# codeonwort/Software-Raytracing

Measured on AMD Instinct MI355X. Metric: Mrays/sec (primary+secondary) + frame time, Cornell Box 1080p 64spp, higher is better.
Workload: dtype f32

## Files before the change

### include/raylib_amd.h

```cpp
#ifndef RAYLIB_AMD_H
#define RAYLIB_AMD_H

#include "raylib_types.h"

#ifdef __cplusplus
extern "C" {
#endif

typedef struct RaylibAMDStats {
	uint64_t rays;
	uint64_t nodesVisited;
	uint64_t trisTested;
	uint64_t shadedHits;
	uint64_t texFetches;
	uint64_t cameraSamples;
	uint64_t pixels;
	double   kernelMs;
	double   traceKernelMs;
	double   wallMs;
	uint32_t traceLaunches;
	uint32_t numNodes;
	uint32_t numTriangles;
	uint32_t bvhDepth;
	uint64_t waveTrips;
// ... 203 lines not shown
typedef struct RaylibAMDLightmapParams {
	int32_t width, height;
	int32_t triFirst, triCount;
	int32_t dilate;
	float   time;
	RaylibAMDGatherParams gather;
} RaylibAMDLightmapParams;
RAYLIB_API int64_t RaylibAMD_LightmapPoints(SceneHandle scene, const RaylibAMDLightmapParams* params, const float* uv, RaylibAMDGatherPoint* outPoints, uint32_t* outTexel,
        int64_t capacity);
RAYLIB_API int64_t RaylibAMD_LightmapPointsHost(SceneHandle scene, const RaylibAMDLightmapParams* params, const float* uv, RaylibAMDGatherPoint* outPoints, uint32_t* outTexel,
        int64_t capacity);
RAYLIB_API int32_t RaylibAMD_BakeLightmap(SceneHandle scene, const RaylibAMDLightmapParams* params, const float* uv, float* out, uint8_t* outCoverage);
RAYLIB_API int32_t RaylibAMD_BakeLightmapDevice(SceneHandle scene, const RaylibAMDLightmapParams* params, const float* uv, float* out, uint8_t* outCoverage, void* stream);
RAYLIB_API int32_t RaylibAMD_BakeLightmapAdaptive(SceneHandle scene, const RaylibAMDLightmapParams* params, const RaylibAMDGatherAdaptiveParams* adaptive, const float* uv,
        float* out, uint8_t* outCoverage, uint32_t* outSamples);
RAYLIB_API int32_t RaylibAMD_BakeLightmapAdaptiveDevice(SceneHandle scene, const RaylibAMDLightmapParams* params, const RaylibAMDGatherAdaptiveParams* adaptive,
        const float* uv, float* out, uint8_t* outCoverage, uint32_t* outSamples, void* stream);

typedef struct RaylibAMDLightmapFilterParams {
	int32_t iterations;
	float   sigmaColor;
	float   sigmaNormal;
	float   sigmaPosition;
} RaylibAMDLightmapFilterParams;
RAYLIB_API int32_t RaylibAMD_BakeLightmapFiltered(SceneHandle scene, const RaylibAMDLightmapParams* params, const RaylibAMDLightmapFilterParams* filter, const float* uv,
        float* out, uint8_t* outCoverage);
RAYLIB_API int32_t RaylibAMD_BakeLightmapFilteredDevice(SceneHandle scene, const RaylibAMDLightmapParams* params, const RaylibAMDLightmapFilterParams* filter, const float* uv,
        float* out, uint8_t* outCoverage, void* stream);
RAYLIB_API int32_t RaylibAMD_FilterLightmap(SceneHandle scene, const RaylibAMDLightmapParams* params, const RaylibAMDLightmapFilterParams* filter, const float* uv,
        const float* in, float* out, uint8_t* outCoverage);
RAYLIB_API int32_t RaylibAMD_FilterLightmapDevice(SceneHandle scene, const RaylibAMDLightmapParams* params, const RaylibAMDLightmapFilterParams* filter, const float* uv,
        const float* in, float* out, uint8_t* outCoverage, void* stream);
RAYLIB_API int32_t RaylibAMD_FilterLightmapHost(int32_t width, int32_t height, int32_t kind, const RaylibAMDLightmapFilterParams* filter, const RaylibAMDGatherPoint* points,
        const uint32_t* texel, int64_t count, const float* values, float* outValues);

typedef uintptr_t MaterialHandle;
RAYLIB_API MaterialHandle RaylibAMD_CreateMaterial(int32_t type, const float albedo[3], float roughness, float metallic,
	const float emissive[3], float ior, const float transmission[3], float fuzziness);
RAYLIB_API int32_t RaylibAMD_DestroyMaterial(MaterialHandle material);
RAYLIB_API SceneElementHandle RaylibAMD_CreateSphere(float cx, float cy, float cz, float radius, MaterialHandle material);
RAYLIB_API SceneElementHandle RaylibAMD_CreateCube(const float minBounds[3], const float maxBounds[3], float timeStartMove,
	const float velocity[3], MaterialHandle material);
RAYLIB_API SceneElementHandle RaylibAMD_CreateTriangle(const float v0[3], const float v1[3], const float v2[3],
	const float n0[3], const float n1[3], const float n2[3], const float uv[6], MaterialHandle material);
RAYLIB_API int32_t RaylibAMD_DestroySceneElement(SceneElementHandle element);

RAYLIB_API int32_t RaylibAMD_EvalScatter(SceneHandle scene, int32_t material, const float* records, int32_t n, uint64_t seed, float* out);
RAYLIB_API int32_t RaylibAMD_EvalCameraRays(CameraHandle camera, const float* uv, int32_t n, uint64_t seed, float* out);
RAYLIB_API int32_t RaylibAMD_EvalTexture(SceneHandle scene, int32_t texture, int32_t bSRGB, const float* uv, int32_t n, float* out);
RAYLIB_API int32_t RaylibAMD_EvalDeviceMath(int32_t fn, const float* x, const float* y, int32_t n, float* out);

RAYLIB_API int32_t RaylibAMD_CullCells(CameraHandle camera, const float* bounds, const float* sunIlluminance, const float* sunDirection,
                                       int32_t width, int32_t height, uint8_t* outEmpty, float* outConstant);

RAYLIB_API int32_t RaylibAMD_VerifyExactMath(int32_t which, uint64_t* outMismatches, uint64_t* outFirstBits);
RAYLIB_API int32_t RaylibAMD_VerifyLazyRefl(uint32_t n, uint64_t seed, uint64_t* outEvents, uint64_t* outUnsafe, uint64_t* outGuardFailed);
RAYLIB_API int32_t RaylibAMD_VerifyLazyPdf(uint32_t n, uint64_t seed, uint64_t* outEvents, uint64_t* outWrong, uint64_t* outRefused);
RAYLIB_API int32_t RaylibAMD_VerifySamplerRanged(int32_t mode, uint64_t* outMismatches, uint64_t* outFirstBits, uint32_t* outInterval, uint64_t* outOutside);

RAYLIB_API int32_t RaylibAMD_SceneMoveTriangles(SceneHandle scene, int32_t first, int32_t count, const float* positions, const float* normals);
RAYLIB_API int32_t RaylibAMD_SceneMoveTrianglesDevice(SceneHandle scene, int32_t first, int32_t count, const float* positions, const float* normals, void* stream);
RAYLIB_API int32_t RaylibAMD_SceneRebuild(SceneHandle scene);
RAYLIB_API int32_t RaylibAMD_SceneCheckTrees(SceneHandle scene, uint32_t* outFailedTree);
RAYLIB_API int32_t RaylibAMD_SceneCompareTrees(SceneHandle scene, uint32_t* outDiffMask);

RAYLIB_API int32_t RaylibAMD_SceneNumTriangles(SceneHandle scene);
RAYLIB_API int32_t RaylibAMD_SceneNumMaterials(SceneHandle scene);
RAYLIB_API int32_t RaylibAMD_SceneNumTextures(SceneHandle scene);
RAYLIB_API void    RaylibAMD_SceneExportTriangles(SceneHandle scene, void* outTriangles);
RAYLIB_API void    RaylibAMD_SceneExportMaterials(SceneHandle scene, void* outMaterials);
RAYLIB_API int32_t RaylibAMD_SceneExportTriOrder(SceneHandle scene, uint32_t* outOrder);
RAYLIB_API void    RaylibAMD_SceneTextureSize(SceneHandle scene, int32_t index, int32_t* outW, int32_t* outH);
RAYLIB_API void    RaylibAMD_SceneExportTexture(SceneHandle scene, int32_t index, float* outRGBA);
RAYLIB_API void    RaylibAMD_SceneGetSun(SceneHandle scene, float outIlluminance[3], float outDirection[3]);
RAYLIB_API int32_t RaylibAMD_SceneBVHInfo(SceneHandle scene, uint32_t* outNodes, uint32_t* outDepth, float* outSahCost);
RAYLIB_API int32_t RaylibAMD_SceneBVH4Info(SceneHandle scene, uint32_t* outNodes4, uint32_t* outWorstCaseStack);
RAYLIB_API int32_t RaylibAMD_SceneBVH8Info(SceneHandle scene, uint32_t* outNodes8, uint32_t* outLevels, float* outSteps4, float* outSteps8);
RAYLIB_API int32_t RaylibAMD_SceneWalk8Host(SceneHandle scene, const float* rays, int32_t count, float tMin, const float* tMax, float* outT, uint32_t* outSteps);
RAYLIB_API int32_t RaylibAMD_SceneWalkStackHost(SceneHandle scene, int32_t tree, const float* rays, int32_t count, float tMin, int32_t capacity, float* outT, uint32_t* outHighWater);
RAYLIB_API int32_t RaylibAMD_SceneLeafListInfo(SceneHandle scene, uint32_t* outMaxTrianglesPerLeaf);
RAYLIB_API int32_t RaylibAMD_ScenePlain(SceneHandle scene);
RAYLIB_API int32_t RaylibAMD_LastTracePlain(void);
RAYLIB_API int32_t RaylibAMD_SceneLazyRefl(SceneHandle scene);
RAYLIB_API int32_t RaylibAMD_LastTraceLazy(void);
RAYLIB_API int32_t RaylibAMD_LastHitQueue(void);
RAYLIB_API int32_t RaylibAMD_LastLitMask(void);
typedef struct RaylibAMDRenderPlan {
	int32_t pathTrace;
	int32_t stack, prims;
	int32_t poolK;
	int32_t tree;
	int32_t lstack;
	int32_t lds;
	int32_t plain;
	uint32_t pathsPerWave, treeWidth, nodeBytes;
	int32_t keepNodes4, keepNodes4f;
	int32_t eagerTree;
	uint32_t batch, sampleCount, blocks, stackStride, jobChunk, heads, jobsPerHead, guideShift;
	uint64_t jobs;
	int32_t lazy;
	int32_t hitQueue;
} RaylibAMDRenderPlan;
RAYLIB_API int32_t RaylibAMD_PlanRender(SceneHandle scene, const RendererSettings* settings, int32_t hasSky, int32_t numCUs, int32_t workgroupsPerCU, RaylibAMDRenderPlan* out);
#define RAYLIB_AMD_MAX_VIEWS 64
RAYLIB_API int32_t RaylibAMD_RenderViews(const RendererSettings* settings, SceneHandle scene,
        const CameraHandle* cameras, int32_t count, const ImageHandle* outImages);
RAYLIB_API int32_t RaylibAMD_RenderViewsDevice(const RendererSettings* settings, SceneHandle scene,
        const CameraHandle* cameras, int32_t count, void* outDevice);
RAYLIB_API int32_t RaylibAMD_PlanViews(SceneHandle scene, const RendererSettings* settings, const CameraHandle* cameras, int32_t count, int32_t hasSky,
        int32_t numCUs, int32_t workgroupsPerCU, RaylibAMDRenderPlan* outPlan, uint8_t* outCellEmpty);
RAYLIB_API uint64_t RaylibAMD_SceneBVHHash(SceneHandle scene);
RAYLIB_API uint64_t RaylibAMD_SceneTopologyHash(SceneHandle scene);
RAYLIB_API int32_t RaylibAMD_SceneExportBVHNodes(SceneHandle scene, void* out);
RAYLIB_API void    RaylibAMD_CameraExport(CameraHandle camera, float out[19]);
RAYLIB_API ImageHandle RaylibAMD_CreateImageFromData(uint32_t width, uint32_t height, const float* rgba);
RAYLIB_API void    RaylibAMD_DumpImageRGBA(ImageHandle image, float* outRGBA);
RAYLIB_API float   RaylibAMD_ParseFloat(const char* token);
RAYLIB_API int32_t RaylibAMD_ImageSize(ImageHandle image, uint32_t* outWidth, uint32_t* outHeight);
RAYLIB_API int32_t RaylibAMD_OBJModelSetTexture(OBJModelHandle obj, const char* materialName, int32_t slot, ImageHandle image);

typedef struct RaylibAMDDenoiseParams {
	int32_t iterations;
	float   sigmaColor;
	float   sigmaNormal;
	float   sigmaAlbedo;
} RaylibAMDDenoiseParams;
RAYLIB_API int32_t RaylibAMD_Denoise(ImageHandle main, int32_t bHDR, ImageHandle albedo, ImageHandle normal,
                                     ImageHandle out, const RaylibAMDDenoiseParams* params);
RAYLIB_API int32_t RaylibAMD_DenoiseHost(uint32_t width, uint32_t height, const float* colorRGBA, int32_t bHDR,
                                         const float* albedoRGBA, const float* normalRGBA,
                                         const RaylibAMDDenoiseParams* params, float* outRGBA);
RAYLIB_API void    RaylibAMD_EnableDenoiser(int32_t enable);

typedef uintptr_t RaylibAMDProgressiveHandle;
typedef struct RaylibAMDProgressiveParams {
	float    threshold;
	uint32_t minSamples;
} RaylibAMDProgressiveParams;

RAYLIB_API RaylibAMDProgressiveHandle RaylibAMD_BeginProgressive(const RendererSettings* settings, SceneHandle scene, CameraHandle camera,
                                                                 ImageHandle out, const RaylibAMDProgressiveParams* params);
RAYLIB_API int32_t RaylibAMD_ProgressiveStep(RaylibAMDProgressiveHandle h, uint32_t samples);
RAYLIB_API int32_t RaylibAMD_ProgressiveExport(RaylibAMDProgressiveHandle h, uint32_t* cellSamples, uint8_t* cellStopped, float* sumY, float* sumY2);
RAYLIB_API int32_t RaylibAMD_EndProgressive(RaylibAMDProgressiveHandle h);
RAYLIB_API int32_t RaylibAMD_ProgressiveDecideHost(uint32_t width, uint32_t height, const uint32_t* cellSamples, const float* sumY,
                                                   const float* sumY2, const RaylibAMDProgressiveParams* params, uint8_t* outStop);
RAYLIB_API int32_t RaylibAMD_ProgressiveCompactTest(const uint32_t* live, uint32_t numLive, const uint8_t* stopped, const uint8_t* emptyOrNull, uint32_t numCells,
                                                    uint32_t width, uint32_t height, uint32_t* outLive, uint32_t* outTrace, uint32_t outCounts[4]);

#ifdef __cplusplus
}
#endif
#endif
```

### software-raytracing_amd/csrc/rl_abi.cc

```cpp
#include "raylib.h"
#include "raylib_amd.h"
#include "rl_host.h"
#include "rl_plan.h"
#include "rl_progressive.h"
#include "rl_lightmap.h"
#include "rl_nearest.h"
#include "rl_sdf.h"
#include "rl_overlap.h"
#include "rl_contact.h"
#include "raylib_amd_rng.h"

#include <float.h>
#include <math.h>
#include <stddef.h>
#include <stdio.h>
#include <stdlib.h>
#include <string.h>
#include <algorithm>

using namespace rl;

namespace {

template <typename T>
// ... 646 lines not shown
SceneElementHandle RaylibAMD_CreateTriangle(const float v0[3], const float v1[3], const float v2[3],
                                            const float n0[3], const float n1[3], const float n2[3], const float uv[6], MaterialHandle material)
{
	if (!v0 || !v1 || !v2 || !n0 || !n1 || !n2) return 0;
	SceneElement* e = NewElement(PRIM_TRIANGLE, material);
	if (!e) return 0;
	HostTriangle& t = e->tri;
	t.v0 = F3(v0[0], v0[1], v0[2]); t.v1 = F3(v1[0], v1[1], v1[2]); t.v2 = F3(v2[0], v2[1], v2[2]);
	t.n0 = F3(n0[0], n0[1], n0[2]); t.n1 = F3(n1[0], n1[1], n1[2]); t.n2 = F3(n2[0], n2[1], n2[2]);
	if (uv) { t.s0 = uv[0]; t.t0 = uv[1]; t.s1 = uv[2]; t.t1 = uv[3]; t.s2 = uv[4]; t.t2 = uv[5]; }
	return (SceneElementHandle)e;
}
int32_t RaylibAMD_DestroySceneElement(SceneElementHandle h)
{
	SceneElement* e = (SceneElement*)h;
	if (g_elements.eraseFirst(e)) { delete e; return 1; }
	return 0;
}

int32_t RaylibAMD_EvalScatter(SceneHandle sh, int32_t material, const float* records, int32_t n, uint64_t seed, float* out)
{
	Scene* s = (Scene*)sh;
	if (!s || !s->finalized || !records || !out || material < 0 || material >= (int32_t)s->materials.size()) return 0;
	return DeviceEvalHook(0, s, nullptr, material, 0, records, n, seed, out) ? 1 : 0;
}
int32_t RaylibAMD_EvalCameraRays(CameraHandle ch, const float* uv, int32_t n, uint64_t seed, float* out)
{
	Camera* c = (Camera*)ch;
	if (!c || !uv || !out) return 0;
	const DCamera d = c->ToDevice();
	return DeviceEvalHook(1, nullptr, &d, 0, 0, uv, n, seed, out) ? 1 : 0;
}
int32_t RaylibAMD_CullCells(CameraHandle ch, const float* bounds, const float* sunIlluminance, const float* sunDirection, int32_t width, int32_t height,
                            uint8_t* outEmpty, float* outConstant)
{
	Camera* c = (Camera*)ch;
	if (!c || !bounds || width <= 0 || height <= 0) return -1;
	CullScene cs;
	for (int k = 0; k < 3; ++k) { cs.boundsMin[k] = bounds[k]; cs.boundsMax[k] = bounds[3 + k]; }
	cs.boundsValid = true;
	if (sunIlluminance && sunDirection) {
		for (int k = 0; k < 3; ++k) { cs.sunIlluminance[k] = sunIlluminance[k]; cs.sunDirection[k] = sunDirection[k]; }
		cs.hasSun = !(sunIlluminance[0] == 0.0f && sunIlluminance[1] == 0.0f && sunIlluminance[2] == 0.0f);
	}
	const uint32_t W = (uint32_t)width, H = (uint32_t)height, cellsX = (W + 7) / 8, cellsY = (H + 7) / 8;
	CullResult r;
	if (!CullCells(cs, c->ToDevice(), 1, 0.0f, W, H, cellsX, 0, 1, cellsX * cellsY, r)) {
		if (outEmpty) memset(outEmpty, 0, (size_t)cellsX * cellsY);
		return r.empty.empty() ? -1 : 0;
	}
	if (outEmpty) memcpy(outEmpty, r.empty.data(), (size_t)cellsX * cellsY);
	if (outConstant) { outConstant[0] = r.L[0]; outConstant[1] = r.L[1]; outConstant[2] = r.L[2]; }
	return (int32_t)(cellsX * cellsY - (uint32_t)r.active.size());
}
int32_t RaylibAMD_EvalTexture(SceneHandle sh, int32_t texture, int32_t bSRGB, const float* uv, int32_t n, float* out)
{
	Scene* s = (Scene*)sh;
	if (!s || !s->finalized || !uv || !out || texture < 0 || texture >= (int32_t)s->textures.size()) return 0;
	return DeviceEvalHook(2, s, nullptr, texture, bSRGB, uv, n, 0, out) ? 1 : 0;
}

int32_t RaylibAMD_EvalDeviceMath(int32_t fn, const float* x, const float* y, int32_t n, float* out)
{
	if (!x || !out) return 0;
	return DeviceEvalMath(fn, x, y, n, out) ? 1 : 0;
}

int32_t RaylibAMD_VerifyExactMath(int32_t which, uint64_t* outMismatches, uint64_t* outFirstBits)
{
	if (which < 0 || which > 4) return 0;
	return DeviceVerifyExactMath(which, outMismatches, outFirstBits) ? 1 : 0;
}

int32_t RaylibAMD_VerifySamplerRanged(int32_t mode, uint64_t* outMismatches, uint64_t* outFirstBits, uint32_t* outInterval, uint64_t* outOutside)
{
	if (mode < 0 || mode > 3) return 0;
	uint64_t out[6] = { 0, 0, 0, 0, 0, 0 };
	if (!DeviceVerifySamplerRanged(mode, out)) return 0;
	if (outMismatches) *outMismatches = out[0];
	if (outFirstBits) *outFirstBits = out[1];
	if (outInterval) { outInterval[0] = (uint32_t)out[2] + 1u; outInterval[1] = (uint32_t)out[5] - 1u; outInterval[2] = (uint32_t)out[4]; }
	if (outOutside) *outOutside = out[3];
	return 1;
}

int32_t RaylibAMD_VerifyLazyRefl(uint32_t n, uint64_t seed, uint64_t* outEvents, uint64_t* outUnsafe, uint64_t* outGuardFailed)
{
	uint64_t out[3] = { 0, 0, 0 };
	if (!DeviceVerifyLazyRefl(n, seed, out)) return 0;
	if (outEvents) *outEvents = out[0];
	if (outUnsafe) *outUnsafe = out[1];
	if (outGuardFailed) *outGuardFailed = out[2];
	return 1;
}

int32_t RaylibAMD_VerifyLazyPdf(uint32_t n, uint64_t seed, uint64_t* outEvents, uint64_t* outWrong, uint64_t* outRefused)
{
	uint64_t out[3] = { 0, 0, 0 };
	if (!DeviceVerifyLazyPdf(n, seed, out)) return 0;
	if (outEvents) *outEvents = out[0];
	if (outWrong) *outWrong = out[1];
	if (outRefused) *outRefused = out[2];
	return 1;
}

int32_t RaylibAMD_ClosestHit(SceneHandle sh, const float* rays, int32_t n, float tMin, void* outHits)
// ... 892 lines not shown
	ill[0] = s->sunIlluminance.x; ill[1] = s->sunIlluminance.y; ill[2] = s->sunIlluminance.z;
	dir[0] = s->sunDirection.x; dir[1] = s->sunDirection.y; dir[2] = s->sunDirection.z;
}
int32_t RaylibAMD_SceneBVHInfo(SceneHandle sh, uint32_t* nodes, uint32_t* depth, float* sah)
{
	Scene* s = (Scene*)sh;
	if (!s || !s->finalized || !DeviceSyncMovedScene(*s)) return 0;
	if (nodes) *nodes = (uint32_t)s->bvh.nodes.size();
	if (depth) *depth = s->bvh.depth;
	if (sah) *sah = s->bvh.sahCost;
	return ValidateBVH(s->bvh, s->triangles) ? 1 : 0;
}
int32_t RaylibAMD_SceneBVH4Info(SceneHandle sh, uint32_t* nodes4, uint32_t* stackNeed)
{
	Scene* s = (Scene*)sh;
	if (!s || !s->finalized || s->bvh.nodes4.empty() || !DeviceSyncMovedScene(*s)) return 0;
	if (nodes4) *nodes4 = (uint32_t)s->bvh.nodes4.size();
	if (stackNeed) *stackNeed = s->bvh.stackNeed4;
	return (ValidateBVH4(s->bvh, s->triangles) && ValidateBVH8(s->bvh, s->triangles)) ? 1 : -1;
}
int32_t RaylibAMD_SceneBVH8Info(SceneHandle sh, uint32_t* nodes8, uint32_t* levels, float* steps4, float* steps8)
{
	Scene* s = (Scene*)sh;
	if (!s || !s->finalized || s->bvh.nodes8.empty() || !DeviceSyncMovedScene(*s)) return 0;
	if (nodes8) *nodes8 = (uint32_t)s->bvh.nodes8.size();
	if (levels) *levels = s->bvh.depth8;
	if (steps4) *steps4 = s->bvh.sahNodes4;
	if (steps8) *steps8 = s->bvh.sahNodes8;
	return ValidateBVH8(s->bvh, s->triangles) ? 1 : -1;
}
int32_t RaylibAMD_SceneWalk8Host(SceneHandle sh, const float* rays, int32_t count, float tMin, const float* tMax, float* outT, uint32_t* outSteps)
{
	Scene* s = (Scene*)sh;
	if (!s || !s->finalized || s->bvh.nodes8.empty() || !rays || !tMax || !outT || count < 0 || !DeviceSyncMovedScene(*s)) return 0;
	return Walk8Host(s->bvh, s->triangles, rays, count, tMin, tMax, outT, outSteps) ? 1 : -1;
}
int32_t RaylibAMD_SceneWalkStackHost(SceneHandle sh, int32_t tree, const float* rays, int32_t count, float tMin, int32_t capacity, float* outT, uint32_t* outHighWater)
{
	Scene* s = (Scene*)sh;
	if (!s || !s->finalized || !rays || !outT || count < 0 || capacity < 0 || (tree != 2 && tree != 3 && tree != 4 && tree != 8)) return 0;
	if (tree == 2 ? s->bvh.nodes.empty() : tree == 3 ? s->bvh.nodes4.empty() : tree == 4 ? s->bvh.nodes4q.empty() : s->bvh.nodes8.empty()) return 0;
	if (!DeviceSyncMovedScene(*s)) return 0;
	return WalkStackHost(s->bvh, s->triangles, s->spheres, s->cubes, tree, rays, count, tMin, capacity, outT, outHighWater) ? 1 : -1;
}
int32_t RaylibAMD_SceneLeafListInfo(SceneHandle sh, uint32_t* maxPerLeaf)
{
	Scene* s = (Scene*)sh;
	if (!s || !s->finalized) return 0;
	int32_t leaves = 0; uint32_t most = 0;
	for (const DNode4& n : s->bvh.leafList) for (int k = 0; k < 4; ++k) if (n.child[k] != DNODE_EMPTY) { ++leaves; most = std::max(most, (((uint32_t)~n.child[k]) & LEAF_COUNT_MASK) + 1u); }
	if (maxPerLeaf) *maxPerLeaf = most;
	return leaves;
}
int32_t RaylibAMD_ScenePlain(SceneHandle sh)
{
	Scene* s = (Scene*)sh;
	return (s && s->finalized && ScenePlain(*s)) ? 1 : 0;
}
int32_t RaylibAMD_LastTracePlain(void) { return DeviceLastTracePlain(); }
int32_t RaylibAMD_SceneLazyRefl(SceneHandle sh)
{
	Scene* s = (Scene*)sh;
	return (s && s->finalized && SceneLazyRefl(*s)) ? 1 : 0;
}
int32_t RaylibAMD_LastTraceLazy(void) { return DeviceLastTraceLazy(); }
int32_t RaylibAMD_LastHitQueue(void) { return DeviceLastHitQueue(); }
int32_t RaylibAMD_LastLitMask(void) { return DeviceLastLitMask(); }
int32_t RaylibAMD_PlanRender(SceneHandle sh, const RendererSettings* settings, int32_t hasSky, int32_t numCUs, int32_t workgroupsPerCU, RaylibAMDRenderPlan* out)
{
	Scene* s = (Scene*)sh;
	if (!s || !s->finalized || !settings || !out || numCUs < 1) return 0;
	memset(out, 0, sizeof(*out));
	const RenderKnobs knobs = ReadRenderKnobs();
	const TracePlan t = PlanTrace(*s, *settings, hasSky != 0, knobs);
	if (!t.ok) return -1;
	out->pathTrace = t.pathTrace; out->stack = t.stack; out->prims = t.prims; out->poolK = t.poolK; out->tree = t.tree; out->lstack = t.lstack; out->lds = t.lds; out->plain = t.plain; out->lazy = t.lazy ? 1 : 0; out->hitQueue = t.hitQueue ? 1 : 0;
	out->pathsPerWave = t.pathsPerWave; out->treeWidth = t.treeWidth; out->nodeBytes = t.nodeBytes;
	out->keepNodes4 = t.keepNodes4; out->keepNodes4f = t.keepNodes4f; out->eagerTree = t.eagerTree;
	const uint32_t cells = ((settings->viewportWidth + 7) / 8) * ((settings->viewportHeight + 7) / 8);
	const uint32_t spp = (uint32_t)(settings->samplesPerPixel > 1 ? settings->samplesPerPixel : 1);
	const LaunchPlan L = PlanLaunch(cells, cells, spp, 0, numCUs, workgroupsPerCU, t, knobs);
	out->batch = L.batch; out->sampleCount = L.sampleCount; out->blocks = L.blocks; out->stackStride = L.stackStride; out->jobChunk = L.jobChunk;
	out->heads = L.heads; out->jobsPerHead = L.jobsPerHead; out->guideShift = L.guideShift; out->jobs = L.jobs;
	return 1;
}
int32_t RaylibAMD_PlanViews(SceneHandle sh, const RendererSettings* settings, const CameraHandle* cameras, int32_t count, int32_t hasSky,
                           int32_t numCUs, int32_t workgroupsPerCU, RaylibAMDRenderPlan* out, uint8_t* outCellEmpty)
{
	Scene* s = (Scene*)sh;
	if (!out || numCUs < 1 || !ViewsArgsValid("RaylibAMD_PlanViews", settings, s, cameras, count, nullptr)) return 0;
	memset(out, 0, sizeof(*out));
	const RenderKnobs knobs = ReadRenderKnobs();
	const TracePlan t = PlanTrace(*s, *settings, hasSky != 0, knobs);
	if (!t.ok) return -1;
	out->pathTrace = t.pathTrace; out->stack = t.stack; out->prims = t.prims; out->poolK = t.poolK; out->tree = t.tree; out->lstack = t.lstack; out->lds = t.lds; out->plain = t.plain; out->lazy = 0;
	out->pathsPerWave = t.pathsPerWave; out->treeWidth = t.treeWidth; out->nodeBytes = t.nodeBytes;
	out->keepNodes4 = t.keepNodes4; out->keepNodes4f = t.keepNodes4f; out->eagerTree = t.eagerTree;
	std::vector<DCamera> cams((size_t)count);
	for (int32_t v = 0; v < count; ++v) cams[(size_t)v] = ((Camera*)cameras[v])->ToDevice();
	if (!DeviceSyncMovedScene(*s)) return 0;
	const ViewsPlan V = PlanViews(SceneCullScene(*s, hasSky != 0), *settings, cams.data(), (uint32_t)count, t, numCUs, workgroupsPerCU, knobs);
	if (!V.ok) return 0;
	if (outCellEmpty) memcpy(outCellEmpty, V.empty.data(), V.empty.size());
	const LaunchPlan& L = V.launch;
	out->batch = L.batch; out->sampleCount = L.sampleCount; out->blocks = L.blocks; out->stackStride = L.stackStride; out->jobChunk = L.jobChunk;
	out->heads = L.heads; out->jobsPerHead = L.jobsPerHead; out->guideShift = L.guideShift; out->jobs = L.jobs;
	return 1;
}
uint64_t RaylibAMD_SceneBVHHash(SceneHandle sh)
{
	Scene* s = (Scene*)sh;
	if (!s || !s->finalized || !DeviceSyncMovedScene(*s)) return 0;
	uint64_t h = 1469598103934665603ull;
	auto feed = [&h](const void* p, size_t n) { const unsigned char* b = (const unsigned char*)p; for (size_t i = 0; i < n; ++i) { h ^= b[i]; h *= 1099511628211ull; } };
	feed(s->bvh.nodes.data(), s->bvh.nodes.size() * sizeof(DNode));
	feed(s->bvh.triOrder.data(), s->bvh.triOrder.size() * sizeof(uint32_t));
	feed(s->bvh.nodes4.data(), s->bvh.nodes4.size() * sizeof(DNode4));
	feed(s->bvh.nodes4q.data(), s->bvh.nodes4q.size() * sizeof(DNode4Q));
	feed(s->bvh.leafList.data(), s->bvh.leafList.size() * sizeof(DNode4));
	feed(s->bvh.nodes8.data(), s->bvh.nodes8.size() * sizeof(DNode8));
	return h;
}
static int32_t MoveTrianglesInternal(const char* who, SceneHandle sh, int32_t first, int32_t count, const float* positions, const float* normals, bool hostMem, void* stream)
{
	Scene* s = (Scene*)sh;
	if (!s || !g_scenes.contains(s)) { Log("%s: unknown scene", who); return 0; }
	if (!s->finalized) { Log("%s: scene was not finalized (Raylib_FinalizeScene)", who); return 0; }
	if (first < 0 || count < 0 || (int64_t)first + (int64_t)count > (int64_t)s->triangles.size()) { Log("%s: triangles [%d, %d + %d) are not the scene's", who, first, first, count); return 0; }
	if (count == 0) return 1;
// ... 109 lines not shown
```

### software-raytracing_amd/csrc/rl_cull.cc

```cpp
#include "rl_host.h"

#include <algorithm>
#include <cmath>
#include <stdlib.h>

namespace rl {

bool CullCells(const CullScene& DS, const DCamera& cam, int32_t maxPathLength, float rayTMin, uint32_t W, uint32_t H,
               uint32_t cellsX, uint32_t cellFirst, uint32_t stride, uint32_t numLocalCells, CullResult& out)
{
	if (const char* e = getenv("RAYLIB_CULL_CELLS")) if (atoi(e) == 0) return false;
	if (DS.prims || !DS.boundsValid || maxPathLength <= 0 || numLocalCells == 0) return false;
	const double lensR = std::fabs((double)cam.lensRadius);
	if (!std::isfinite(lensR)) return false;
	if (!(rayTMin >= 0.0f)) return false;
	auto sub3 = [](const double* a, const double* b, double* r) { r[0] = a[0] - b[0]; r[1] = a[1] - b[1]; r[2] = a[2] - b[2]; };
	auto dot3 = [](const double* a, const double* b) { return a[0] * b[0] + a[1] * b[1] + a[2] * b[2]; };
	const double O[3] = { cam.origin[0], cam.origin[1], cam.origin[2] }, TL[3] = { cam.top_left[0], cam.top_left[1], cam.top_left[2] };
	const double Hh[3] = { cam.horizontal[0], cam.horizontal[1], cam.horizontal[2] }, Vv[3] = { cam.vertical[0], cam.vertical[1], cam.vertical[2] };
	for (int k = 0; k < 3; ++k) if (!std::isfinite(O[k]) || !std::isfinite(TL[k]) || !std::isfinite(Hh[k]) || !std::isfinite(Vv[k])) return false;
	double E[3]; sub3(TL, O, E); for (int k = 0; k < 3; ++k) E[k] += Vv[k];
	double N[3] = { Hh[1] * Vv[2] - Hh[2] * Vv[1], Hh[2] * Vv[0] - Hh[0] * Vv[2], Hh[0] * Vv[1] - Hh[1] * Vv[0] };
	const double hh = dot3(Hh, Hh), vv = dot3(Vv, Vv), nn = dot3(N, N);
	if (!(hh > 0.0) || !(vv > 0.0) || !(nn > 0.0) || std::fabs(dot3(Hh, Vv)) > 1e-6 * std::sqrt(hh * vv)) return false;
	double planeDist = dot3(E, N);
	if (planeDist < 0.0) { planeDist = -planeDist; for (int k = 0; k < 3; ++k) N[k] = -N[k]; }
	if (!(planeDist > 1e-12 * std::sqrt(nn) * std::sqrt(dot3(E, E)))) return false;
	const double ext = std::max({ DS.boundsMax[0] - DS.boundsMin[0], DS.boundsMax[1] - DS.boundsMin[1], DS.boundsMax[2] - DS.boundsMin[2], 1e-30 });
	double uLo = 1e300, uHi = -1e300, vLo = 1e300, vHi = -1e300;
	double lensFac = 0.0;
	for (int c = 0; c < 8; ++c) {
		double X[3], Q[3];
		for (int k = 0; k < 3; ++k) X[k] = (c >> k & 1) ? DS.boundsMax[k] + 1e-6 * ext : DS.boundsMin[k] - 1e-6 * ext;
		sub3(X, O, Q);
		const double depth = dot3(Q, N);
		if (!(depth > 1e-9 * std::sqrt(nn) * (std::sqrt(dot3(Q, Q)) + ext))) return false;
		const double sc = planeDist / depth;
		lensFac = std::max(lensFac, std::fabs(1.0 - sc));
		double R3[3]; for (int k = 0; k < 3; ++k) R3[k] = Q[k] * sc - E[k];
		const double u = dot3(R3, Hh) / hh, v = -dot3(R3, Vv) / vv;
		if (!std::isfinite(u) || !std::isfinite(v)) return false;
		uLo = std::min(uLo, u); uHi = std::max(uHi, u); vLo = std::min(vLo, v); vHi = std::max(vHi, v);
	}
	const double margin = 2.0;
	const double cocU = lensR * lensFac / std::sqrt(hh) * 1.0001, cocV = lensR * lensFac / std::sqrt(vv) * 1.0001;
	if (!std::isfinite(cocU) || !std::isfinite(cocV)) return false;
	const double xLo = (uLo - cocU) * W - margin, xHi = (uHi + cocU) * W + margin, yLo = (vLo - cocV) * H - margin, yHi = (vHi + cocV) * H + margin;
	out.raysPerSample = 1;
	out.L[0] = out.L[1] = out.L[2] = 0.0f;
	if (DS.hasSun) {
		const double D[3] = { -(double)DS.sunDirection[0], -(double)DS.sunDirection[1], -(double)DS.sunDirection[2] };
		double t0 = 0.0, t1 = 1e300;
		bool miss = false;
		for (int k = 0; k < 3 && !miss; ++k) {
			const double lo = DS.boundsMin[k] - 0.01 * ext - lensR, hi = DS.boundsMax[k] + 0.01 * ext + lensR;
			if (D[k] == 0.0) { if (O[k] < lo || O[k] > hi) miss = true; continue; }
			double a = (lo - O[k]) / D[k], b = (hi - O[k]) / D[k]; if (a > b) std::swap(a, b);
			t0 = std::max(t0, a); t1 = std::min(t1, b);
			if (t0 > t1) miss = true;
		}
		if (!miss || !std::isfinite(D[0]) || !std::isfinite(D[1]) || !std::isfinite(D[2])) return false;
		out.raysPerSample = 2;
		for (int k = 0; k < 3; ++k) out.L[k] = 0.0f + DS.sunIlluminance[k];
	}
	const uint32_t numCells = cellsX * ((H + 7) / 8);
	out.active.clear(); out.active.reserve(numLocalCells);
	out.empty.assign(numLocalCells, 0);
	out.emptyPixels = 0;
	for (uint32_t k = 0; k < numLocalCells; ++k) {
		const uint32_t cell = cellFirst + k * stride;
		if (cell >= numCells) { out.active.push_back(k); continue; }
		const uint32_t cx = cell % cellsX, cy = cell / cellsX;
		const double px0 = 8.0 * cx - 1.0, px1 = 8.0 * cx + 8.0, py0 = 8.0 * cy - 1.0, py1 = 8.0 * cy + 8.0;
		const bool outside = px1 < xLo || px0 > xHi || py1 < yLo || py0 > yHi;
		if (outside) {
			out.empty[k] = 1;
			out.emptyPixels += (uint64_t)std::min(8u, W - cx * 8) * std::min(8u, H - cy * 8);
		} else out.active.push_back(k);
	}
	return out.active.size() < numLocalCells;
}


}
```

### software-raytracing_amd/csrc/rl_dev_jobs.h

```cpp
#pragma once

#include "rl_dev_shade.h"

namespace rl {

__device__ __forceinline__ void CameraRay(const DCamera& k, float s, float t, Rng& g, V3& o, V3& d, float& rayTime)
{
	V3 rd;
	if (k.lensRadius == 0.0f) {
		(void)Next(g);
		const float u2 = Next(g);
		const float theta = 2.0f * 3.14159265358979323846f * u2;
		bool sn, cn; rtm::sincos_signs_(theta, &sn, &cn);
		rd = k.lensRadius * v3(cn ? -1.0f : 1.0f, sn ? -1.0f : 1.0f, 0.0f);
	} else {
		rd = k.lensRadius * RandomInUnitDisk(g);
	}
	V3 cu = ld3(k.u), cv = ld3(k.v);
	V3 offset = (cu * rd.x) + (cv * rd.y);
	float captureTime = k.beginTime + k.timePeriod * Next(g);
	rayTime = captureTime;
	V3 origin = ld3(k.origin);
	o = origin + offset;
	d = normalize(ld3(k.top_left) + s * ld3(k.horizontal) + (1.0f - t) * ld3(k.vertical) - origin - offset);
// ... 6 lines not shown
	v = rtm::div_by_((float)y, imageHeight, P.invHeight);
	if (sampleIndex != 0) {
		u += rtm::div_by_((Next(g) - 0.5f) * 2.0f, imageWidth, P.invWidth);
		v += rtm::div_by_((Next(g) - 0.5f) * 2.0f, imageHeight, P.invHeight);
	}
}

__device__ __forceinline__ SampleRGB make_sample(float x, float y, float z) { SampleRGB s; s.x = x; s.y = y; s.z = z; return s; }

struct JobPixel { uint32_t x, y, slot, sample; bool valid; };
__device__ __forceinline__ JobPixel DecodeJob(const DRenderParams& P, uint32_t job)
{
	JobPixel j;
	const uint32_t p = job & 63u;
	const uint32_t rest = job >> 6;
	uint32_t cellLocal = __umulhi(rest, P.magicSamples);
	uint32_t sLocal = rest - cellLocal * P.sampleCount;
	while (sLocal >= P.sampleCount) { sLocal -= P.sampleCount; ++cellLocal; }
#ifdef RL_EXP_STRIPS
	{
		const uint32_t cph = P.jobsPerHead / (P.sampleCount * 64u), hh = cellLocal / cph, ii = cellLocal % cph, sw = P.cellsX / P.numHeads;
		cellLocal = (ii / sw) * P.cellsX + hh * sw + ii % sw;
	}
#endif
	if (P.activeCells) cellLocal = P.activeCells[cellLocal];
	const uint32_t cell = P.cellFirst + cellLocal * P.cellStride;
	uint32_t cy = __umulhi(cell, P.magicCellsX);
	uint32_t cx = cell - cy * P.cellsX;
	while (cx >= P.cellsX) { cx -= P.cellsX; ++cy; }
	j.x = cx * 8u + (p & 7u); j.y = cy * 8u + (p >> 3);
	j.slot = cellLocal * 64u + p;
	j.sample = sLocal;
	j.valid = (j.x < P.width) && (j.y < P.height);
	return j;
}

__device__ __forceinline__ JobPixel DecodeJobBatch(const DRenderParams& P, uint32_t base, uint32_t lane)
{
	JobPixel j;
	const uint32_t rest = (uint32_t)__builtin_amdgcn_readfirstlane((int)base) >> 6;
	uint32_t cellLocal = __umulhi(rest, P.magicSamples);
	uint32_t sLocal = rest - cellLocal * P.sampleCount;
	while (sLocal >= P.sampleCount) { sLocal -= P.sampleCount; ++cellLocal; }
	if (P.activeCells) cellLocal = *(const __attribute__((address_space(4))) uint32_t*)(P.activeCells + cellLocal);
	const uint32_t cell = P.cellFirst + cellLocal * P.cellStride;
	uint32_t cy = __umulhi(cell, P.magicCellsX);
	uint32_t cx = cell - cy * P.cellsX;
	while (cx >= P.cellsX) { cx -= P.cellsX; ++cy; }
	j.x = cx * 8u + (lane & 7u); j.y = cy * 8u + (lane >> 3);
	j.slot = cellLocal * 64u + lane;
	j.sample = sLocal;
	j.valid = (j.x < P.width) && (j.y < P.height);
	return j;
}

__device__ __forceinline__ uint32_t DecodeView(const DViews& V, uint32_t batchCell, uint32_t& cellInView)
{
	uint32_t view = __umulhi(batchCell, V.magicCellsPerView);
	uint32_t c = batchCell - view * V.cellsPerView;
	while (c >= V.cellsPerView) { c -= V.cellsPerView; ++view; }
	cellInView = c;
	return view;
}
__device__ __forceinline__ JobPixel DecodeJobViews(const DRenderParams& P, const DViews& V, uint32_t job, uint32_t& view)
{
	JobPixel j;
	const uint32_t p = job & 63u;
	const uint32_t rest = job >> 6;
	uint32_t cellLocal = __umulhi(rest, P.magicSamples);
	uint32_t sLocal = rest - cellLocal * P.sampleCount;
	while (sLocal >= P.sampleCount) { sLocal -= P.sampleCount; ++cellLocal; }
	if (P.activeCells) cellLocal = P.activeCells[cellLocal];
	uint32_t cell;
	view = DecodeView(V, cellLocal, cell);
	uint32_t cy = __umulhi(cell, P.magicCellsX);
	uint32_t cx = cell - cy * P.cellsX;
	while (cx >= P.cellsX) { cx -= P.cellsX; ++cy; }
	j.x = cx * 8u + (p & 7u); j.y = cy * 8u + (p >> 3);
	j.slot = cellLocal * 64u + p;
	j.sample = sLocal;
	j.valid = (j.x < P.width) && (j.y < P.height);
	return j;
}
__device__ __forceinline__ JobPixel DecodeJobBatchViews(const DRenderParams& P, const DViews& V, uint32_t base, uint32_t lane, uint32_t& view)
{
	JobPixel j;
	const uint32_t rest = (uint32_t)__builtin_amdgcn_readfirstlane((int)base) >> 6;
	uint32_t cellLocal = __umulhi(rest, P.magicSamples);
	uint32_t sLocal = rest - cellLocal * P.sampleCount;
	while (sLocal >= P.sampleCount) { sLocal -= P.sampleCount; ++cellLocal; }
	if (P.activeCells) cellLocal = *(const __attribute__((address_space(4))) uint32_t*)(P.activeCells + cellLocal);
	uint32_t cell;
	view = DecodeView(V, cellLocal, cell);
	uint32_t cy = __umulhi(cell, P.magicCellsX);
	uint32_t cx = cell - cy * P.cellsX;
	while (cx >= P.cellsX) { cx -= P.cellsX; ++cy; }
	j.x = cx * 8u + (lane & 7u); j.y = cy * 8u + (lane >> 3);
	j.slot = cellLocal * 64u + lane;
	j.sample = sLocal;
	j.valid = (j.x < P.width) && (j.y < P.height);
	return j;
}
__device__ __forceinline__ DCamera LoadViewCamera(const DViews& V, uint32_t view) { return V.cameras[view]; }
__device__ __forceinline__ DCamera LoadViewCameraUniform(const DViews& V, uint32_t view)
{
	DCamera k;
// ... 43 lines not shown
		key = max(key, (uint32_t)__shfl_xor((int)key, 2));
		key = max(key, (uint32_t)__shfl_xor((int)key, 4));
		key = (uint32_t)__builtin_amdgcn_readfirstlane((int)key);
		if (key < 64u) return false;
		js.cur = key & 7u; js.left = key & ~63u;
	}
}

__device__ __forceinline__ void WaveLdsSync()
{
	__builtin_amdgcn_fence(__ATOMIC_ACQ_REL, "wavefront");
	__builtin_amdgcn_wave_barrier();
}

#ifndef RL_KARG_RELOAD
#define RL_KARG_RELOAD 1
#endif
struct KTraceArgs { DRenderParams P; DSceneView S; SkyRot R; SampleRGB* samples; float* pathStack; unsigned long long* counters; unsigned int* jobCounter; };
template <class T> __device__ __forceinline__ T KArg(uint32_t offset)
{
	uint32_t z = 0u;
	asm volatile("" : "+s"(z));
	T v;
	__builtin_memcpy(&v, (const __attribute__((address_space(4))) char*)__builtin_amdgcn_kernarg_segment_ptr() + offset + (z << 2), sizeof(T));
	return v;
}
#if RL_KARG_RELOAD
#define RL_ARGS() \
	const DRenderParams P = KArg<DRenderParams>((uint32_t)offsetof(KTraceArgs, P)); const DSceneView S = KArg<DSceneView>((uint32_t)offsetof(KTraceArgs, S)); \
	const SkyRot R = KArg<SkyRot>((uint32_t)offsetof(KTraceArgs, R)); SampleRGB* const samples = KArg<SampleRGB*>((uint32_t)offsetof(KTraceArgs, samples)); \
	float* const pathStack = KArg<float*>((uint32_t)offsetof(KTraceArgs, pathStack)); unsigned long long* const counters = KArg<unsigned long long*>((uint32_t)offsetof(KTraceArgs, counters)); \
	unsigned int* const jobCounter = KArg<unsigned int*>((uint32_t)offsetof(KTraceArgs, jobCounter)); \
	(void)P; (void)S; (void)R; (void)samples; (void)pathStack; (void)counters; (void)jobCounter
#else
#define RL_ARGS() \
	const DRenderParams& P = Pk; const DSceneView& S = Sk; const SkyRot& R = Rk; SampleRGB* const samples = samplesK; float* const pathStack = pathStackK; \
	unsigned long long* const counters = countersK; unsigned int* const jobCounter = jobCounterK; \
	(void)P; (void)S; (void)R; (void)samples; (void)pathStack; (void)counters; (void)jobCounter
#endif
struct KTraceViewsArgs { KTraceArgs A; DViews V; };
#if RL_KARG_RELOAD
#define RL_VIEWS() const DViews VW = KArg<DViews>((uint32_t)offsetof(KTraceViewsArgs, V)); (void)VW
#else
#define RL_VIEWS() const DViews& VW = Vk; (void)VW
#endif

struct KTraceLazyArgs { KTraceArgs A; DLitList LL; };
#if RL_KARG_RELOAD
#define RL_LIT_ARGS() const DLitList LL = KArg<DLitList>((uint32_t)offsetof(KTraceLazyArgs, LL)); (void)LL
#else
#define RL_LIT_ARGS() const DLitList& LL = LLk; (void)LL
#endif

template <class EACH>
__device__ __forceinline__ float4 SumSlotBatch(const DRenderParams& P, const DSceneView& S, const SkyRot& R, const SampleRGB* samples,
                                               uint32_t numSlots, uint32_t slot, uint32_t cellLocal, uint32_t x, uint32_t y, float4 a, EACH&& each)
{
	if (P.cellEmpty && P.cellEmpty[cellLocal]) {
		if (P.emptySky) {
			Counters c; c.rays = c.nodes = c.tris = c.shaded = c.texels = c.samples = c.trips = 0; RL_DIAG_BIND(c);
			for (uint32_t s = 0; s < P.sampleCount; ++s) {
				const uint32_t sidx = P.sampleBegin + s;
				Rng g; g.s = raylib_rng_begin_mixed(P.seedMixed, y * P.width + x, sidx);
				float u, v;
				PixelUV(P, x, y, sidx, g, u, v);
				V3 o, d; float rayTime;
				CameraRay(P.camera, u, v, g, o, d, rayTime);
				V3 L = MissSky(S, R, d, c);
				if (S.hasSun) L = L + ld3(S.sunIlluminance);
				a.x += L.x; a.y += L.y; a.z += L.z;
				each(L.x, L.y, L.z);
			}
		} else
		for (uint32_t s = 0; s < P.sampleCount; ++s) { a.x += P.emptyL[0]; a.y += P.emptyL[1]; a.z += P.emptyL[2]; each(P.emptyL[0], P.emptyL[1], P.emptyL[2]); }
	} else
	for (uint32_t s = 0; s < P.sampleCount; ++s) {
		const SampleRGB v = samples[(size_t)s * numSlots + slot];
		a.x += v.x; a.y += v.y; a.z += v.z;
		each(v.x, v.y, v.z);
	}
	return a;
}

}
```

### software-raytracing_amd/csrc/rl_dev_walk.h

```cpp
#pragma once

#include "rl_dev_scene.h"

namespace rl {

#define RL_BOX_WIDEN 1.00001f
#define RL_CANDIDATE_SLACK 1.000009f

#ifndef RL_OWN_BOX_WIDEN_TMIN
#define RL_OWN_BOX_WIDEN_TMIN 0
#endif
__device__ __forceinline__ bool OwnBoxPassBox(V3 mn, V3 mx, V3 o, V3 inv , float tMin, float t);
__device__ __forceinline__ bool OwnBoxPass(V3 a, V3 b, V3 c, V3 o, V3 inv , float tMin, float t)
{
	const V3 mn = v3(fminf(fminf(a.x, b.x), c.x), fminf(fminf(a.y, b.y), c.y), fminf(fminf(a.z, b.z), c.z));
	const V3 mx = v3(fmaxf(fmaxf(a.x, b.x), c.x), fmaxf(fmaxf(a.y, b.y), c.y), fmaxf(fmaxf(a.z, b.z), c.z));
	return OwnBoxPassBox(mn, mx, o, inv, tMin, t);
}
__device__ __forceinline__ bool OwnBoxPassMnMx(const float4* rec, V3 o, V3 inv, float tMin, float t)
{
	const float4 q4 = rec[4], q5 = rec[5];
	return OwnBoxPassBox(v3(q4.x, q4.y, q4.z), v3(q4.w, q5.x, q5.y), o, inv, tMin, t);
}
__device__ __forceinline__ bool OwnBoxPassBox(V3 mn, V3 mx, V3 o, V3 inv , float tMin, float t)
// ... 215 lines not shown
		cur = stk[sp * RL_BLOCK];
	}
	return best.tri >= 0;
}

__device__ __forceinline__ V3 ClampInv(V3 inv)
{
	return v3(isinf(inv.x) ? copysignf(1e30f, inv.x) : inv.x, isinf(inv.y) ? copysignf(1e30f, inv.y) : inv.y, isinf(inv.z) ? copysignf(1e30f, inv.z) : inv.z);
}
typedef float rl_v4f __attribute__((ext_vector_type(4)));
typedef uint32_t rl_v4u __attribute__((ext_vector_type(4)));
__device__ __forceinline__ float4 GLoadF4(const void* p, int i) { const rl_v4f v = ((const __attribute__((address_space(1))) rl_v4f*)p)[i]; return make_float4(v.x, v.y, v.z, v.w); }
__device__ __forceinline__ uint4 GLoadU4(const void* p, int i) { const rl_v4u v = ((const __attribute__((address_space(1))) rl_v4u*)p)[i]; return make_uint4(v.x, v.y, v.z, v.w); }
#define RL_GRID_ERR(A_, B_) (fabsf((A_) * 1.21593475e-4f) + fabsf((B_) * 4.76837158e-7f))
#define RL_SORT4_STEP(ta, ra, tb, rb) { const bool sw = tb < ta; const float tt = sw ? tb : ta; tb = sw ? ta : tb; ta = tt; const int rr = sw ? rb : ra; rb = sw ? ra : rb; ra = rr; }
#define RL_SORT4(t0, r0, t1, r1, t2, r2, t3, r3) RL_SORT4_STEP(t0, r0, t1, r1) RL_SORT4_STEP(t2, r2, t3, r3) RL_SORT4_STEP(t0, r0, t2, r2) RL_SORT4_STEP(t1, r1, t3, r3) RL_SORT4_STEP(t1, r1, t2, r2)
#define RL_WIDE_STEP_Q(S_, cur_, o_, inv_, nx_, ny_, nz_, tMin_, tmx_, widen_, t0, t1, t2, t3, ch) \
	 \
	 \
	const DNode4Q* np_ = (S_).nodes4 + (cur_); \
	const float4 h0_ = GLoadF4(np_, 0); const uint4 l_ = GLoadU4(np_, 1); const uint4 u_ = GLoadU4(np_, 2); \
	const uint4 chu_ = GLoadU4(np_, 3); const int4 ch = make_int4((int)chu_.x, (int)chu_.y, (int)chu_.z, (int)chu_.w); \
	const float Ax_ = h0_.w * (inv_).x, Ay_ = __uint_as_float(l_.w) * (inv_).y, Az_ = __uint_as_float(u_.w) * (inv_).z; \
	const float Bx_ = (h0_.x - (o_).x) * (inv_).x, By_ = (h0_.y - (o_).y) * (inv_).y, Bz_ = (h0_.z - (o_).z) * (inv_).z; \
	const float Ex_ = RL_GRID_ERR(Ax_, Bx_), Ey_ = RL_GRID_ERR(Ay_, By_), Ez_ = RL_GRID_ERR(Az_, Bz_); \
	const float Bnx_ = Bx_ - Ex_, Bfx_ = Bx_ + Ex_, Bny_ = By_ - Ey_, Bfy_ = By_ + Ey_, Bnz_ = Bz_ - Ez_, Bfz_ = Bz_ + Ez_; \
	const uint32_t nX_ = (nx_) ? u_.x : l_.x, fX_ = (nx_) ? l_.x : u_.x, nY_ = (ny_) ? u_.y : l_.y, fY_ = (ny_) ? l_.y : u_.y, nZ_ = (nz_) ? u_.z : l_.z, fZ_ = (nz_) ? l_.z : u_.z; \
	const float tMinL_ = (tMin_), tmxL_ = (tmx_), widenL_ = (widen_); \
	float t0, t1, t2, t3; \
	RL_QSLAB(0, t0) RL_QSLAB(8, t1) RL_QSLAB(16, t2) RL_QSLAB(24, t3)
#define RL_QSLAB(sh, tk) { \
	float tn = tMinL_, tf = tmxL_; \
	tn = fmaxf(tn, __builtin_fmaf((float)((nX_ >> sh) & 0xffu), Ax_, Bnx_)); tf = fminf(tf, __builtin_fmaf((float)((fX_ >> sh) & 0xffu), Ax_, Bfx_)); \
	tn = fmaxf(tn, __builtin_fmaf((float)((nY_ >> sh) & 0xffu), Ay_, Bny_)); tf = fminf(tf, __builtin_fmaf((float)((fY_ >> sh) & 0xffu), Ay_, Bfy_)); \
	tn = fmaxf(tn, __builtin_fmaf((float)((nZ_ >> sh) & 0xffu), Az_, Bnz_)); tf = fminf(tf, __builtin_fmaf((float)((fZ_ >> sh) & 0xffu), Az_, Bfz_)); \
	tk = (tf * widenL_ < tn) ? INFINITY : tn; }
#define RL_WIDE_STEP_F(np_expr, o_, inv_, nx_, ny_, nz_, tMin_, tmx_, widen_, t0, t1, t2, t3, ch) \
	const float4* np_ = (np_expr); \
	const float4 lox_ = np_[0], loy_ = np_[1], loz_ = np_[2], hix_ = np_[3], hiy_ = np_[4], hiz_ = np_[5]; \
	const int4 ch = ((const int4*)np_)[6]; \
	const float4 nX_ = (nx_) ? hix_ : lox_, fX_ = (nx_) ? lox_ : hix_; \
	const float4 nY_ = (ny_) ? hiy_ : loy_, fY_ = (ny_) ? loy_ : hiy_; \
	const float4 nZ_ = (nz_) ? hiz_ : loz_, fZ_ = (nz_) ? loz_ : hiz_; \
	const float tMinL_ = (tMin_), tmxL_ = (tmx_), widenL_ = (widen_); const V3 oL_ = (o_), invL_ = (inv_); \
	float t0, t1, t2, t3; \
	RL_FSLAB(x, t0) RL_FSLAB(y, t1) RL_FSLAB(z, t2) RL_FSLAB(w, t3)
#define RL_FSLAB(k, tk) { \
	float tn = tMinL_, tf = tmxL_; \
	tn = fmaxf(tn, (nX_.k - oL_.x) * invL_.x); tf = fminf(tf, (fX_.k - oL_.x) * invL_.x); \
	tn = fmaxf(tn, (nY_.k - oL_.y) * invL_.y); tf = fminf(tf, (fY_.k - oL_.y) * invL_.y); \
	tn = fmaxf(tn, (nZ_.k - oL_.z) * invL_.z); tf = fminf(tf, (fZ_.k - oL_.z) * invL_.z); \
	tk = (tf * widenL_ < tn) ? INFINITY : tn; }

template <bool ANYHIT, bool PLAIN = false>
__device__ __forceinline__ bool TraverseLeafList(const DSceneView& S, V3 o, V3 d, float tMin, HitRec& best, Counters& c, const float4* sm)
{
	c.rays++;
	const V3 invb = ExactInv(d);
	const bool nx = invb.x < 0.0f, ny = invb.y < 0.0f, nz = invb.z < 0.0f;
	best.t = INFINITY; best.tri = -1; best.a = 0.0f; best.b = 0.0f;
	uint32_t key[4 * RL_LEAFLIST_RECORDS];
	const V3 cc = v3(-(o.x * invb.x), -(o.y * invb.y), -(o.z * invb.z));
	const V3 ce = v3(fabsf(cc.x) * 2.3841858e-7f, fabsf(cc.y) * 2.3841858e-7f, fabsf(cc.z) * 2.3841858e-7f);
	const V3 cn = cc - ce, cf = cc + ce;
	const char* recs = (const char*)(sm + LdsAt<2>::NODES);
	const uint32_t oNX = nx ? 48u : 0u, oFX = 48u - oNX, oNY = ny ? 64u : 16u, oFY = 80u - oNY, oNZ = nz ? 80u : 32u, oFZ = 112u - oNZ;
	#pragma unroll
	for (int g = 0; g < RL_LEAFLIST_RECORDS; ++g) {
		key[4 * g] = key[4 * g + 1] = key[4 * g + 2] = key[4 * g + 3] = 0xffffffffu;
		if (g < S.numLeafRecords) {
			c.nodes += 2;
			RL_WSTEP(4);
			const char* rec = recs + g * (RL_LDS_NSTRIDE * 16);
			const float4 nX = *(const float4*)(rec + oNX), fX = *(const float4*)(rec + oFX);
			const float4 nY = *(const float4*)(rec + oNY), fY = *(const float4*)(rec + oFY);
			const float4 nZ = *(const float4*)(rec + oNZ), fZ = *(const float4*)(rec + oFZ);
			#ifndef RL_LL_SMEAR
			#define RL_LL_SMEAR 1
			#endif
			#define RL_LSLAB(k, slot) { \
				float tn = tMin, tf; \
				if (RL_LL_SMEAR) { \
					float ntn = -tMin; \
					ntn = fminf(ntn, -__builtin_fmaf(nX.k, invb.x, cn.x)); tf = __builtin_fmaf(fX.k, invb.x, cf.x); \
					ntn = fminf(ntn, -__builtin_fmaf(nY.k, invb.y, cn.y)); tf = fminf(tf, __builtin_fmaf(fY.k, invb.y, cf.y)); \
					ntn = fminf(ntn, -__builtin_fmaf(nZ.k, invb.z, cn.z)); tf = fminf(tf, __builtin_fmaf(fZ.k, invb.z, cf.z)); \
					key[slot] = ((__float_as_uint(ntn) & 0x7fffffe0u) | (uint32_t)(slot)) | (uint32_t)((int32_t)__float_as_uint(__builtin_fmaf(tf, RL_BOX_WIDEN, ntn)) >> 31); \
				} else { \
					tn = fmaxf(tn, __builtin_fmaf(nX.k, invb.x, cn.x)); tf = __builtin_fmaf(fX.k, invb.x, cf.x); \
					tn = fmaxf(tn, __builtin_fmaf(nY.k, invb.y, cn.y)); tf = fminf(tf, __builtin_fmaf(fY.k, invb.y, cf.y)); \
					tn = fmaxf(tn, __builtin_fmaf(nZ.k, invb.z, cn.z)); tf = fminf(tf, __builtin_fmaf(fZ.k, invb.z, cf.z)); \
					if (!(tf * RL_BOX_WIDEN < tn)) key[slot] = (__float_as_uint(tn) & ~31u) | (uint32_t)(slot); } }
			RL_LSLAB(x, 4 * g) RL_LSLAB(y, 4 * g + 1) RL_LSLAB(z, 4 * g + 2) RL_LSLAB(w, 4 * g + 3)
			#undef RL_LSLAB
		}
	}
	uint32_t from = 0u;
#ifdef RL_WATCHDOG
	int guardSel = 0;
#endif
	uint32_t m = 0xffffffffu;
	#pragma unroll
	for (int j = 0; j < 4 * RL_LEAFLIST_RECORDS; ++j) m = min(m, key[j]);
	for (;;) {
#ifdef RL_WATCHDOG
		if (++guardSel > 200) { printf("leaf-list pick stuck: lane %u from %u tMin %g best %g keys %u %u %u %u\n", threadIdx.x, from, tMin, best.t, key[0], key[1], key[2], key[3]); break; }
#endif
		if (m >= 0xffffffffu - from) break;
		m += from;
		if (best.t * RL_BOX_WIDEN < __uint_as_float(m & ~31u)) break;
		from = m + 1u;
		RL_WSTEP(6);
		const uint32_t j = m & 31u;
		const LeafRef L = DecodeLeaf(((const int*)(sm + LdsAt<2>::NODES + (j >> 2) * RL_LDS_NSTRIDE + 6))[j & 3u]);
#if defined(RL_DIAG_STAMPS) && RL_DIAG_STAMPS >= 2
		{
			uint32_t pairs = 0;
			for (int cc = 1; cc <= 8; ++cc) pairs += (uint32_t)cc * (uint32_t)__popcll(Ballot(L.count == cc));
			const unsigned long long em_ = Ballot(true);
			if (c.diag && (threadIdx.x & 63u) == (uint32_t)__ffsll((long long)em_) - 1u) atomicAdd(&c.diag[CNT_COUNT + 7], (unsigned long long)((pairs + 63u) / 64u));
		}
#endif
		for (int i = 0; i < L.count; ++i) {
			const float4* tr = sm + LdsAt<2>::ISECT + (L.first + i) * 6;
			const float4 q0 = tr[0], q1 = tr[1], q2 = tr[2], q3 = tr[3];
			struct { V3 v0, n, u, v; float uv, uu, vv, denom, rden; } T;
			T.v0 = v3(q0.x, q0.y, q0.z); T.n = v3(q0.w, q1.x, q1.y); T.u = v3(q1.z, q1.w, q2.x); T.v = v3(q2.y, q2.z, q2.w);
			T.uv = q3.x; T.uu = q3.y; T.vv = q3.z; T.denom = q3.w; T.rden = tr[5].z;
			c.tris++;
			RL_WSTEP(5);
			RL_TRIANGLE_TEST(S, T, L.first + i, o, d, tMin, best, !PLAIN && L.alpha, OwnBoxPassMnMx(tr, o, invb, tMin, t), ANYHIT, c, RL_ELSE_CONTINUE)
		}
		m = 0xffffffffu;
		#pragma unroll
		for (int j = 0; j < 4 * RL_LEAFLIST_RECORDS; ++j) m = min(m, key[j] - from);
	}
	return best.tri >= 0;
}

template <int STACK, bool ANYHIT, bool PRIMS, bool FULL, int LDS = 0, bool PLAIN = false>
__device__ __forceinline__ bool Traverse4(const DSceneView& S, V3 o, V3 d, float rayTime, float tMin, HitRec& best, int* stk, Counters& c, const float4* sm = nullptr,
                                          const float tBound = INFINITY)
{
	if constexpr (LDS == 2) return TraverseLeafList<ANYHIT, PLAIN>(S, o, d, tMin, best, c, sm);
	c.rays++;
	V3 invb = ExactInv(d);
	if (!FULL) invb = ClampInv(invb);
	const bool nx = invb.x < 0.0f, ny = invb.y < 0.0f, nz = invb.z < 0.0f;
	best.t = tBound; best.tri = -1; best.a = 0.0f; best.b = 0.0f;
	int sp = 0, cur = 0;
	const int DONE = 0x7fffffff;
	for (;;) {
		while (cur >= 0 && cur != DONE) {
			c.nodes += FULL ? 2 : 1;
			RL_WSTEP(4);
			const float tmx = fminf(best.t, FLT_MAX);
			float t0, t1, t2, t3; int r0, r1, r2, r3;
			if (FULL) { RL_WIDE_STEP_F((LDS ? sm + RL_LDS_NODES + cur * RL_LDS_NSTRIDE : (const float4*)(S.nodes4f + cur)), o, invb, nx, ny, nz, tMin, tmx, RL_BOX_WIDEN, a0, a1, a2, a3, ch) t0 = a0; t1 = a1; t2 = a2; t3 = a3; r0 = ch.x; r1 = ch.y; r2 = ch.z; r3 = ch.w; }
			else { RL_WIDE_STEP_Q(S, cur, o, invb, nx, ny, nz, tMin, tmx, RL_BOX_WIDEN, a0, a1, a2, a3, ch) t0 = a0; t1 = a1; t2 = a2; t3 = a3; r0 = ch.x; r1 = ch.y; r2 = ch.z; r3 = ch.w; }
			if (r0 == DNODE_EMPTY) t0 = INFINITY;
			if (r1 == DNODE_EMPTY) t1 = INFINITY;
			if (r2 == DNODE_EMPTY) t2 = INFINITY;
			if (r3 == DNODE_EMPTY) t3 = INFINITY;
			RL_SORT4(t0, r0, t1, r1, t2, r2, t3, r3)
			if (!(t0 < INFINITY)) { if (sp == 0) cur = DONE; else { --sp; cur = stk[sp * RL_BLOCK]; } continue; }
			if (t3 < INFINITY && sp < STACK) { stk[sp * RL_BLOCK] = r3; ++sp; }
			if (t2 < INFINITY && sp < STACK) { stk[sp * RL_BLOCK] = r2; ++sp; }
			if (t1 < INFINITY && sp < STACK) { stk[sp * RL_BLOCK] = r1; ++sp; }
			cur = r0;
		}
		if (cur == DONE) break;
		{
			const LeafRef L = DecodeLeaf(cur);
			RL_WSTEP(6);
			for (int i = 0; i < L.count; ++i) {
				const Tri T = LDS ? TriFrom(sm + RL_LDS_ISECT + (L.first + i) * RL_LDS_TSTRIDE) : LoadTri(S, L.first + i);
				c.tris++;
				RL_WSTEP(5);
				RL_TRIANGLE_TEST(S, T, L.first + i, o, d, tMin, best, L.alpha, OwnBoxPass(T.v0, T.v1, T.v2, o, ExactInv(d), tMin, t), ANYHIT, c, RL_ELSE_CONTINUE)
			}
		}
		if (sp == 0) break;
		--sp;
		cur = stk[sp * RL_BLOCK];
	}
	(void)rayTime;
	return best.tri >= 0;
}

}
```

### software-raytracing_amd/csrc/rl_host.h

```cpp
#pragma once

#include "raylib_types.h"
#include "raylib_amd.h"
#include "rl_device.h"

#include <math.h>
#include <stdint.h>
#include <memory>
#include <mutex>
#include <string>
#include <vector>

namespace rl {

struct f3 { float x, y, z; };
inline f3 F3(float x, float y, float z) { f3 r; r.x = x; r.y = y; r.z = z; return r; }
inline f3 operator+(f3 a, f3 b) { return F3(a.x + b.x, a.y + b.y, a.z + b.z); }
inline f3 operator-(f3 a, f3 b) { return F3(a.x - b.x, a.y - b.y, a.z - b.z); }
inline f3 operator*(f3 a, f3 b) { return F3(a.x * b.x, a.y * b.y, a.z * b.z); }
inline f3 operator*(f3 a, float t) { return F3(a.x * t, a.y * t, a.z * t); }
inline f3 operator*(float t, f3 a) { return F3(a.x * t, a.y * t, a.z * t); }
inline f3 operator-(f3 a) { return F3(-a.x, -a.y, -a.z); }
inline float dot(f3 a, f3 b) { return a.x * b.x + a.y * b.y + a.z * b.z; }
inline f3 cross(f3 a, f3 b) { return F3(a.y * b.z - a.z * b.y, -(a.x * b.z - a.z * b.x), a.x * b.y - a.y * b.x); }
// ... 129 lines not shown
	void Finalize();
	bool BuildAccel(float t0, float t1);
};
bool ScenePlain(const Scene& sc);
bool SceneLazyRefl(const Scene& sc);

struct FlatScene {
	std::vector<DTriIsect> isect; std::vector<DTriShade> shade; std::vector<int32_t> alphaTex;
	std::vector<DMaterial> materials; std::vector<DTexture> textures; std::vector<float> texels;
	std::vector<DSphere> spheres; std::vector<DCube> cubes;
	int32_t fastBary = 1;
	SkyRot skyRot;
};
FlatScene FlattenScene(const Scene& sc);

bool LoadOBJ(const char* path, OBJModel& out);
void TransformOBJ(OBJModel& m, float tx, float ty, float tz, float yaw, float pitch, float roll, float sx, float sy, float sz);
Image* LoadImageFile(const char* path);
bool WriteImageFile(const Image& img, const char* path, uint32_t fileType);
void PostProcessHost(Image& img);

void Log(const char* fmt, ...);
void LogStart();
void LogFlush();
void LogStop();

struct RenderRequest {
	RendererSettings settings;
	DCamera camera;
	uint64_t seed;
	uint32_t cellFirst, cellStride;
	bool cellMajor = false;
	int slot = 0;
	void* outDevice;
	bool callerOwnsOut = false;
	float* outHostRGBA;
};
bool DeviceAvailable();
int DeviceNumRanks();
float ParseDecimalFloat(const char* token);
constexpr uint64_t kMaxImagePixels = 1ull << 28;
inline bool PlausibleImageSize(uint64_t w, uint64_t h, uint64_t fileBytes, uint64_t maxPixelsPerByte)
{
	return w > 0 && h > 0 && w <= 65535 && h <= 65535 && w * h <= kMaxImagePixels && w * h <= (fileBytes + 64) * maxPixelsPerByte;
}
bool DecodeJPEG(const std::vector<uint8_t>& data, uint32_t& w, uint32_t& h, std::vector<uint8_t>& rgba);
bool DecodeTGA(const std::vector<uint8_t>& data, uint32_t& w, uint32_t& h, std::vector<uint8_t>& rgba);
bool EncodeJPEG(uint32_t w, uint32_t h, const uint8_t* rgbTopDown, std::vector<uint8_t>& out);
bool DeviceRender(Scene& scene, const RenderRequest& req, RaylibAMDStats& stats);
bool DeviceRenderViews(Scene& scene, const RenderRequest& req, const DCamera* cameras, uint32_t count, void* outDevice, void* const* imagePixels, RaylibAMDStats& stats);
int32_t DeviceLastTraceLazy();
int32_t DeviceLastHitQueue();
int32_t DeviceLastLitMask();
int32_t DeviceLastTracePlain();
bool DeviceDrain(RaylibAMDStats* outLastStats);
void DeviceOwnStats();
bool DeviceClosestHit(Scene& scene, const float* rays, int32_t n, float tMin, void* outHits);
bool DeviceTraceRays(Scene& scene, int32_t kind, const void* rays, int32_t n, float rayTime, void* out, int32_t* outPrim, bool hostMem, void* stream,
                     RaylibAMDStats& stats);
bool DeviceRenderGBuffer(Scene& scene, const RendererSettings& settings, const DCamera& camera, uint64_t seed, const RaylibAMDGBufferPlanes& planes, bool hostMem, void* stream,
                         RaylibAMDStats& stats);
bool DeviceTraceRaysAll(Scene& scene, const void* rays, int32_t n, int32_t maxHits, void* outHits, uint32_t* outCount, bool hostMem, void* stream, RaylibAMDStats& stats);
bool DeviceNearestPoints(Scene& scene, int32_t kind, const void* points, int32_t n, void* out, bool hostMem, void* stream, RaylibAMDStats& stats);
bool DeviceNearestPointsAll(Scene& scene, const void* points, int32_t n, int32_t maxHits, void* outHits, uint32_t* outCount, bool hostMem, void* stream, RaylibAMDStats& stats);
bool DeviceBakeDistanceField(Scene& scene, const RaylibAMDDistanceFieldParams& grid, float* outDist, int32_t* outPrim, bool hostMem, void* stream, RaylibAMDStats& stats);
bool DeviceOverlapTriangles(Scene& scene, int32_t kind, uint32_t flags, const void* queries, int32_t n, int32_t maxHits, void* out, uint32_t* outCount, bool hostMem, void* stream,
                            RaylibAMDStats& stats, void* outContact = nullptr, bool contacts = false);
constexpr uint64_t RL_RADIANCE_STACK_BUDGET = 256ull << 20;
constexpr int32_t RL_RADIANCE_MAX_PATH = 32768;
bool DeviceTraceRadiance(Scene& scene, const RaylibAMDRadianceParams& prm, uint64_t seed, const void* rays, int32_t n, float* out, bool hostMem, void* stream,
                         RaylibAMDStats& stats);
constexpr uint64_t RL_GATHER_SAMPLE_BUDGET = 256ull << 20;
constexpr uint64_t RL_GATHER_MAX_SLOTS = 1ull << 28;
constexpr uint64_t RL_GATHER_TIMED = 4096;
constexpr uint32_t RL_GATHER_ADAPTIVE_MAX_PASSES = 4096;
bool DeviceGather(Scene& scene, int32_t kind, const RaylibAMDRadianceParams& prm, uint64_t seed, const void* points, int32_t n, float* out, bool hostMem, void* stream,
                  RaylibAMDStats& stats, const RaylibAMDGatherAdaptiveParams* A = nullptr, uint32_t* outSamples = nullptr);
bool DeviceGatherCompactTest(const uint32_t* live, uint32_t numLive, const uint8_t* stopped, const RaylibAMDGatherPoint* points, uint32_t numPoints,
                             uint32_t* outLive, RaylibAMDGatherPoint* outPoints, uint32_t* outCount);
int64_t LightmapPointsHost(const Scene& scene, const RaylibAMDLightmapParams& P, int32_t triFirst, int32_t triCount, const float* uv,
                           RaylibAMDGatherPoint* outPoints, uint32_t* outTexel, int64_t capacity);
int64_t DeviceLightmapPoints(Scene& scene, const RaylibAMDLightmapParams& P, int32_t triFirst, int32_t triCount, const float* uv,
                             RaylibAMDGatherPoint* outPoints, uint32_t* outTexel, int64_t capacity);
bool DeviceBakeLightmap(const char* who, Scene& scene, const RaylibAMDLightmapParams& P, int32_t triFirst, int32_t triCount, const RaylibAMDRadianceParams& prm, uint64_t seed,
                        const float* uv, float* out, uint8_t* outCoverage, bool hostMem, void* stream, RaylibAMDStats& stats,
                        const RaylibAMDLightmapFilterParams* filter = nullptr, const float* in = nullptr,
                        const RaylibAMDGatherAdaptiveParams* adaptive = nullptr, uint32_t* outSamples = nullptr);
struct LmFilterInv { float invC[8], invN, invP[8]; };
LmFilterInv MakeLmFilterInv(const RaylibAMDLightmapFilterParams& F);
bool FilterLightmapHost(int32_t width, int32_t height, int32_t kind, const RaylibAMDLightmapFilterParams& F, const RaylibAMDGatherPoint* points, const uint32_t* texel,
                        int64_t count, const float* values, float* outValues);
bool DevicePostProcess(Image& img);
bool DeviceDumpRGB(Image& img, float* outRGB);
bool DeviceReadback(Image& img);
void* DeviceImagePixels(Image& img);
void DeviceFreePixels(void* p);
struct CullScene { double boundsMin[3] = { 0, 0, 0 }, boundsMax[3] = { 0, 0, 0 }; bool boundsValid = false, prims = false, hasSky = false, hasSun = false; float sunDirection[3] = { 0, 0, 0 }, sunIlluminance[3] = { 0, 0, 0 }; };
struct CullResult { std::vector<uint32_t> active; std::vector<unsigned char> empty; uint64_t emptyPixels = 0; float L[3] = { 0, 0, 0 }; uint32_t raysPerSample = 1; };
bool CullCells(const CullScene& DS, const DCamera& cam, int32_t maxPathLength, float rayTMin, uint32_t W, uint32_t H,
               uint32_t cellsX, uint32_t cellFirst, uint32_t stride, uint32_t numLocalCells, CullResult& out);
bool DeviceEvalMath(int fn, const float* x, const float* y, int n, float* out);
bool DeviceVerifyLazyRefl(uint32_t n, uint64_t seed, uint64_t out[3]);
bool DeviceVerifyLazyPdf(uint32_t n, uint64_t seed, uint64_t out[3]);
bool DeviceVerifySamplerRanged(int mode, uint64_t out[6]);
bool DeviceVerifyExactMath(int which, uint64_t* outMismatches, uint64_t* outFirst);
bool DeviceEvalHook(int kind, Scene* sc, const DCamera* cam, int a, int b, const float* in, int n, uint64_t seed, float* out);
void DeviceReleaseScene(DeviceScene* dev);
bool DeviceMoveTriangles(Scene& scene, int32_t first, int32_t count, const float* positions, const float* normals, bool hostMem, void* stream);
bool DeviceSyncMovedScene(Scene& scene);
bool DeviceCheckTrees(Scene& scene, uint32_t* outFailedTree);
bool DeviceCompareTrees(Scene& scene, uint32_t* outDiffMask);

struct ProgressiveSession;
ProgressiveSession* DeviceProgressiveBegin(Scene& sc, const RenderRequest& req, float threshold, uint32_t minSamples);
int32_t DeviceProgressiveStep(ProgressiveSession& S, uint32_t samples, void* outDevice, RaylibAMDStats& stats, bool& rendered);
bool DeviceProgressiveExport(ProgressiveSession& S, uint32_t* cellSamples, uint8_t* cellStopped, float* sumY, float* sumY2);
void DeviceProgressiveEnd(ProgressiveSession* S);
bool DeviceProgressiveCompactTest(const uint32_t* live, uint32_t numLive, const uint8_t* stopped, const uint8_t* emptyOrNull, uint32_t numCells,
                                  uint32_t width, uint32_t height, uint32_t* outLive, uint32_t* outTrace, uint32_t outCounts[4]);

void DenoiseHost(uint32_t width, uint32_t height, const float* color, bool hdr, const float* albedo, const float* normal,
                 const RaylibAMDDenoiseParams& params, float* out);
bool DeviceDenoise(Image& main, bool hdr, Image* albedo, Image* normal, Image& out, const RaylibAMDDenoiseParams& params);

}
```

### software-raytracing_amd/csrc/rl_kernels.h

```cpp
#pragma once

#include "rl_dev_jobs.h"
#include "rl_dev_pool.h"

namespace rl {

#ifndef RL_QUEUE_SPIN_LIMIT
#define RL_QUEUE_SPIN_LIMIT 0
#endif
#ifndef RL_TRACE_MIN_WAVES
#define RL_TRACE_MIN_WAVES 4
#endif
#define RL_TRACE_ARGS const DRenderParams, const DSceneView, const SkyRot, SampleRGB* __restrict__, float* __restrict__, unsigned long long* __restrict__, unsigned int* __restrict__
template <int STACK, bool PRIMS, bool FULL, int LDS = 0, bool PLAIN = false>
__global__ void __launch_bounds__(RL_BLOCK, (STACK <= 32 ? RL_TRACE_MIN_WAVES : 2)) k_trace(RL_TRACE_ARGS);
template <int STACK, bool PRIMS, bool FULL, int LDS = 0, bool PLAIN = false>
__global__ void __launch_bounds__(RL_BLOCK, (STACK <= 32 ? RL_TRACE_MIN_WAVES : 2)) k_trace_views(RL_TRACE_ARGS, const DViews);
#define RL_TRACE_INSTANCES(X) \
	X(16, false, false, 0, false) X(16, false, true, 0, false) X(16, false, true, 1, false) X(16, false, true, 2, false) X(16, false, true, 2, true) \
	X(32, false, false, 0, false) X(32, false, true, 0, false) X(32, true, false, 0, false) X(32, true, true, 0, false) \
	X(64, false, false, 0, false) X(64, false, true, 0, false) X(64, true, false, 0, false) X(64, true, true, 0, false)
#define RL_K_TRACE(a, b, c, d, e) template __global__ void k_trace<a, b, c, d, e>(RL_TRACE_ARGS);
#define RL_K_TRACE_VIEWS(a, b, c, d, e) template __global__ void k_trace_views<a, b, c, d, e>(RL_TRACE_ARGS, const DViews);
RL_TRACE_INSTANCES(extern RL_K_TRACE)
RL_TRACE_INSTANCES(extern RL_K_TRACE_VIEWS)
template <int STACK, bool PRIMS, bool FULL, int LDS, bool PLAIN>
__global__ void __launch_bounds__(RL_BLOCK, (STACK <= 32 ? RL_TRACE_MIN_WAVES : 2)) k_trace_lazy(RL_TRACE_ARGS, const DLitList);
#define RL_TRACE_LAZY_INSTANCES(X) X(16, false, true, 2, true)
#define RL_K_TRACE_LAZY(a, b, c, d, e) template __global__ void k_trace_lazy<a, b, c, d, e>(RL_TRACE_ARGS, const DLitList);
RL_TRACE_LAZY_INSTANCES(extern RL_K_TRACE_LAZY)
template <int STACK, bool PRIMS, bool FULL, int LDS, bool PLAIN>
__global__ void __launch_bounds__(RL_BLOCK, (STACK <= 32 ? RL_TRACE_MIN_WAVES : 2)) k_trace_lazy_hitq(RL_TRACE_ARGS, const DLitList);
#define RL_K_TRACE_LAZY_HITQ(a, b, c, d, e) template __global__ void k_trace_lazy_hitq<a, b, c, d, e>(RL_TRACE_ARGS, const DLitList);
RL_TRACE_LAZY_INSTANCES(extern RL_K_TRACE_LAZY_HITQ)
__global__ void __launch_bounds__(RL_BLOCK) k_fold_lit(const DSceneView S, const DLitList LL, SampleRGB* __restrict__ samples, uint32_t numSlots);
__global__ void __launch_bounds__(RL_BLOCK)
k_resolve_lit(const DRenderParams P, const DSceneView S, const SkyRot R, const SampleRGB* __restrict__ samples, float4* __restrict__ accum, float4* __restrict__ out,
              int firstBatch, int lastBatch, const DLitList LL);

template <int STACK, bool PRIMS, int K, int LSTACK = STACK, int WIDE = 0>
__global__ void __launch_bounds__(RL_BLOCK, (PoolOcc<LSTACK, PRIMS, K>::kBlocks)) k_trace_pool(RL_TRACE_ARGS);
template <int STACK, bool PRIMS, int K, int LSTACK = STACK, int WIDE = 0>
__global__ void __launch_bounds__(RL_BLOCK, (PoolOcc<LSTACK, PRIMS, K>::kBlocks)) k_trace_pool_views(RL_TRACE_ARGS, const DViews);
#define RL_POOL_INSTANCES(X) \
	X(16, false, 2, 16, 0) X(16, false, 3, 16, 0) X(16, false, 4, 16, 0) X(32, false, 2, 32, 0) X(32, false, 3, 32, 0) X(32, false, 4, 32, 0) \
	X(32, false, 2, 4, 0) X(32, false, 2, RL_POOL_SHORT_LSTACK, 0) \
	X(32, false, 2, 32, 1) X(64, false, 2, 32, 1) X(32, false, 2, RL_POOL_SHORT_LSTACK, 1) X(64, false, 2, RL_POOL_SHORT_LSTACK, 1) \
	X(2 * RL_POOL8_MAXLEVELS, false, 2, RL_POOL8_LSTACK, 3)
#define RL_K_TRACE_POOL(a, b, c, d, e) template __global__ void k_trace_pool<a, b, c, d, e>(RL_TRACE_ARGS);
#define RL_K_TRACE_POOL_VIEWS(a, b, c, d, e) template __global__ void k_trace_pool_views<a, b, c, d, e>(RL_TRACE_ARGS, const DViews);
RL_POOL_INSTANCES(extern RL_K_TRACE_POOL_VIEWS)
RL_POOL_INSTANCES(extern RL_K_TRACE_POOL)

__global__ void __launch_bounds__(RL_BLOCK)
k_resolve(const DRenderParams P, const DSceneView S, const SkyRot R, const SampleRGB* __restrict__ samples, float4* __restrict__ accum, float4* __restrict__ out, int firstBatch, int lastBatch);
__global__ void __launch_bounds__(RL_BLOCK)
k_resolve_views(const DRenderParams Pb, const DSceneView S, const SkyRot R, const SampleRGB* __restrict__ samples, float4* __restrict__ accum, float4* __restrict__ out,
                int firstBatch, int lastBatch, const DViews V);
#define RL_AOV_ARGS const DRenderParams, const DSceneView, float4* __restrict__, unsigned long long* __restrict__
template <int STACK, bool PRIMS> __global__ void __launch_bounds__(RL_BLOCK) k_aov(RL_AOV_ARGS);
template <int STACK, bool PRIMS> __global__ void __launch_bounds__(RL_BLOCK) k_aov_views(RL_AOV_ARGS, const DViews);
#define RL_AOV_INSTANCES(X) X(16, false) X(32, false) X(32, true) X(64, false) X(64, true)
#define RL_K_AOV(a, b) template __global__ void k_aov<a, b>(RL_AOV_ARGS);
#define RL_K_AOV_VIEWS(a, b) template __global__ void k_aov_views<a, b>(RL_AOV_ARGS, const DViews);
RL_AOV_INSTANCES(extern RL_K_AOV)
RL_AOV_INSTANCES(extern RL_K_AOV_VIEWS)

struct ProgressiveState {
	float4* sum;
	float* s1;
	float* s2;
	uint32_t* cellSamples;
	uint8_t* stopped;
	float threshold;
	uint32_t minSamples;
};
__global__ void __launch_bounds__(RL_BLOCK)
k_progressive_resolve(const DRenderParams P, const DSceneView S, const SkyRot R, const SampleRGB* __restrict__ samples, const ProgressiveState st,
                      float4* __restrict__ out, int lastBatch);
#define RL_COMPACT_BLOCK 1024
#define RL_COMPACT_PER 8
__global__ void __launch_bounds__(RL_COMPACT_BLOCK)
k_progressive_compact(uint32_t* __restrict__ live, uint32_t* __restrict__ trace, const uint8_t* __restrict__ stopped, const uint8_t* __restrict__ empty,
                      uint32_t numLive, uint32_t width, uint32_t height, uint32_t cellsX, uint32_t* __restrict__ counts);

__global__ void __launch_bounds__(RL_BLOCK) k_pp_max(const float4* __restrict__ px, size_t n, unsigned int* __restrict__ whiteBits);
// ... 208 lines not shown
```

### software-raytracing_amd/csrc/rl_plan.cc

```cpp
#include "rl_plan.h"

#include <algorithm>
#include <atomic>
#include <cmath>
#include <cstring>
#include <stdlib.h>

namespace rl {

RenderKnobs ReadRenderKnobs()
{
	RenderKnobs k;
	auto flag = [](const char* name) { const char* e = getenv(name); return e ? (atoi(e) != 0 ? 1 : 0) : -1; };
	if (const char* e = getenv("RAYLIB_POOL")) { const int v = atoi(e); k.pool = (v == 2 || v == 3 || v == 4) ? v : 0; }
	if (const char* e = getenv("RAYLIB_POOL_MIN_TRIS")) k.poolMinTris = (uint32_t)atoi(e);
	if (const char* e = getenv("RAYLIB_POOL_SHORT_STACK")) { const int v = atoi(e); k.poolShortStack = (v == 0 || v == 4) ? v : 1; }
	k.bvh4 = flag("RAYLIB_BVH4"); k.bvh8 = flag("RAYLIB_BVH8");
	k.ldsScene = flag("RAYLIB_LDS_SCENE"); k.leafList = flag("RAYLIB_LEAF_LIST"); k.plainKernel = flag("RAYLIB_PLAIN_KERNEL");
	if (const char* e = getenv("RAYLIB_SAMPLE_BATCH")) k.sampleBatch = std::max(0, atoi(e));
	if (const char* e = getenv("RAYLIB_SAMPLE_BUFFER_GIB")) k.sampleBufferGiB = std::max(0, atoi(e));
	if (const char* e = getenv("RAYLIB_JOB_CHUNK")) k.jobChunk = std::max(0, atoi(e));
	if (const char* e = getenv("RAYLIB_JOB_HEADS")) k.jobHeads = std::max(1, atoi(e));
	if (const char* e = getenv("RAYLIB_GUIDED")) k.guided = atoi(e);
	if (const char* e = getenv("RAYLIB_BLOCKS_PER_CU")) k.blocksPerCU = std::max(0, atoi(e));
	if (const char* e = getenv("RAYLIB_CULL_CELLS")) k.cullCells = atoi(e);
	k.lazyRefl = flag("RAYLIB_LAZY_REFL"); k.hitQueue = flag("RAYLIB_HIT_QUEUE");
	if (const char* e = getenv("RAYLIB_LIT_LIST")) k.litList = std::max(0ll, atoll(e));
	k.litMask = flag("RAYLIB_LIT_MASK");
	if (const char* e = getenv("RAYLIB_QUERY_TREE")) { const int v = atoi(e); k.queryTree = (v == 2 || v == 4 || v == 8) ? v : 0; }
	if (const char* e = getenv("RAYLIB_GATHER_BATCH")) k.gatherBatch = std::max(0, atoi(e));
	return k;
}

namespace {

TracePlan Pick(const Scene& sc, const RendererSettings& st, bool hasSky, const RenderKnobs& k, bool say)
{
	TracePlan p;
	const BVH& b = sc.bvh;
	const size_t ntri = sc.triangles.size();
	p.prims = !sc.spheres.empty() || !sc.cubes.empty();
	if (b.depth > 64) {
		if (say) Log("Raylib_Render: BVH depth %u exceeds the traversal stack (64)", b.depth);
		p.ok = false;
		return p;
	}
	p.stack = (b.depth <= 16 && !p.prims) ? 16 : b.depth <= 32 ? 32 : 64;
	p.pathTrace = st.renderMode == RAYLIB_RENDERMODE_Default;
	if (!p.pathTrace) return p;
	const bool hasNodes4 = !b.nodes4.empty(), hasNodes8 = !b.nodes8.empty();

	const bool poolable = p.stack <= 32 && !p.prims;
	const int poolK = k.pool >= 0 ? k.pool : (poolable && ntri >= k.poolMinTris ? 2 : 0);
	if (poolable && poolK > 0) {
		p.poolK = poolK; p.pathsPerWave = 64u * (uint32_t)poolK;
		if (poolK == 2 && hasNodes4 && b.stackNeed4 <= 64 && k.bvh4 != 0) {
			p.tree = TREE_GRID4; p.treeWidth = 4;
			p.stack = b.stackNeed4 <= 32 ? 32 : 64;
			if (k.poolShortStack == 0) { p.lstack = 32; return p; }
			const bool want8 = hasNodes8 && (k.bvh8 >= 0 ? k.bvh8 != 0 : b.sahNodes4 >= RL_BVH8_MIN_STEPS);
			if (want8 && b.depth8 <= RL_POOL8_MAXLEVELS) {
				p.tree = TREE_WIDE8; p.treeWidth = 8; p.nodeBytes = (uint32_t)sizeof(DNode8);
				p.stack = 2 * RL_POOL8_MAXLEVELS; p.lstack = RL_POOL8_LSTACK;
				return p;
			}
			if (want8 && say) {
				static std::atomic<const Scene*> told{ nullptr };
				if (told.exchange(&sc) != &sc) Log("Raylib_Render: the scene's 8-wide tree has %u levels, the pool kernel's stack holds %d: walking the 4-wide tree", b.depth8, (int)RL_POOL8_MAXLEVELS);
			}
			p.lstack = RL_POOL_SHORT_LSTACK;
			return p;
		}
		p.lstack = p.stack;
		if (p.stack == 32 && poolK == 2) {
			if (k.poolShortStack == 4) p.lstack = 4;
			else if (k.poolShortStack >= 0 ? k.poolShortStack != 0 : b.depth <= RL_POOL_SHORT_MAXDEPTH) p.lstack = RL_POOL_SHORT_LSTACK;
		}
		return p;
	}

	const bool floatBoxes = hasNodes4 && ntri < RL_FLOAT_BOX_MAX_TRIS;
	const bool wide = !p.prims && hasNodes4 && b.stackNeed4 <= (uint32_t)p.stack && k.bvh4 != 0;
	p.tree = !wide ? TREE_BVH2 : floatBoxes ? TREE_BOX4 : TREE_GRID4;
	p.treeWidth = wide ? 4 : 2;
	p.keepNodes4 = p.tree == TREE_GRID4;
	p.keepNodes4f = p.tree == TREE_BOX4;
	if (p.stack == 16 && p.tree == TREE_BOX4 && k.ldsScene != 0 && b.nodes4.size() <= RL_LDS_MAXNODES && ntri <= RL_LDS_MAXTRIS && sc.materials.size() <= RL_LDS_MAXMATS) {
		p.lds = 1;
		if (!b.leafList.empty() && b.leafList.size() <= RL_LEAFLIST_RECORDS && ntri <= RL_LEAFLIST_MAXTRIS && k.leafList != 0 && st.rayTMin >= 0.0f) {
			p.lds = 2; p.tree = TREE_NONE; p.treeWidth = 0;
			p.plain = !hasSky && k.plainKernel != 0 && ScenePlain(sc);
			p.lazy = p.plain && k.lazyRefl != 0 && st.maxPathLength <= RL_LAZY_MAX_PATH && SceneLazyRefl(sc);
			p.hitQueue = p.lazy && st.maxPathLength >= 1 && (k.hitQueue >= 0 ? k.hitQueue != 0 : RL_HIT_QUEUE_DEFAULT != 0);
		}
	}
	return p;
}

}

int32_t EagerTree(const Scene& sc)
{
	RendererSettings st = {};
	st.renderMode = RAYLIB_RENDERMODE_Default;
	const TracePlan d = Pick(sc, st, false, RenderKnobs(), false);
	return (d.tree == TREE_GRID4 || d.tree == TREE_WIDE8) ? d.tree : TREE_NONE;
}

TracePlan PlanTrace(const Scene& sc, const RendererSettings& st, bool hasSky, const RenderKnobs& knobs)
{
	TracePlan p = Pick(sc, st, hasSky, knobs, true);
	p.eagerTree = EagerTree(sc);
	return p;
}

QueryPlan PlanQuery(const Scene& sc, int32_t kind, const RenderKnobs& k)
{
	QueryPlan p;
	const BVH& b = sc.bvh;
	p.prims = !sc.spheres.empty() || !sc.cubes.empty();
	if (b.depth > 64) { p.ok = false; return p; }
	const int want = k.queryTree ? k.queryTree : 8;
	if (want >= 8 && !p.prims && !b.nodes8.empty() && b.depth8 <= RL_POOL8_MAXLEVELS) {
		p.tree = TREE_WIDE8; p.treeWidth = 8; p.nodeBytes = (uint32_t)sizeof(DNode8); p.stack = 2 * RL_POOL8_MAXLEVELS;
	} else if (want >= 4 && !p.prims && !b.nodes4q.empty() && b.stackNeed4 <= 64) {
		p.tree = TREE_GRID4; p.treeWidth = 4; p.stack = b.stackNeed4 <= 32 ? 32 : 64;
	} else {
		p.stack = b.depth <= 32 ? 32 : 64;
	}
	p.early = kind == RAYLIB_AMD_QUERY_ANY && !p.prims;
	return p;
}

QueryPlan PlanGBuffer(const Scene& sc, const RenderKnobs& k)
{
	return PlanQuery(sc, RAYLIB_AMD_QUERY_SURFACE, k);
}

QueryPlan PlanQueryAll(const Scene& sc, const RenderKnobs& k)
{
	QueryPlan p;
	const BVH& b = sc.bvh;
	p.prims = !sc.spheres.empty() || !sc.cubes.empty();
	if (b.depth > 64) { p.ok = false; return p; }
	const int want = k.queryTree ? k.queryTree : 8;
	if (want >= 8 && !p.prims && !b.nodes8.empty() && b.depth8 <= RL_POOL8_MAXLEVELS) {
// ... 179 lines not shown
```

### software-raytracing_amd/csrc/rl_plan.h

```cpp
#pragma once

#include "rl_host.h"

namespace rl {

#define RL_POOL_DEFAULT_MIN_TRIS 256u
#define RL_HIT_QUEUE_DEFAULT 1
#define RL_FLOAT_BOX_MAX_TRIS 4096u

struct RenderKnobs {
	int pool = -1;
	uint32_t poolMinTris = RL_POOL_DEFAULT_MIN_TRIS;
	int poolShortStack = -1;
	int bvh4 = -1, bvh8 = -1;
	int ldsScene = -1, leafList = -1, plainKernel = -1;
	int sampleBatch = 0, sampleBufferGiB = 0;
	int jobChunk = -1;
	int jobHeads = 0;
	int guided = 0;
	int blocksPerCU = 0;
	int cullCells = 1;
	int queryTree = 0;
	int gatherBatch = 0;
	int lazyRefl = -1;
	int hitQueue = -1;
	long long litList = -1;
	int litMask = -1;
};
RenderKnobs ReadRenderKnobs();

enum PlanTree : int32_t { TREE_NONE = 0, TREE_BVH2 = 1, TREE_BOX4 = 2, TREE_GRID4 = 3, TREE_WIDE8 = 4 };

struct TracePlan {
	bool ok = true;
	bool pathTrace = true;
	int stack = 16;
	bool prims = false;
	int poolK = 0;
	int32_t tree = TREE_BVH2;
	int lstack = 0;
	int lds = 0;
	bool plain = false;
	bool lazy = false;
	bool hitQueue = false;
	uint32_t pathsPerWave = 64, treeWidth = 2, nodeBytes = 64;
	bool keepNodes4 = true, keepNodes4f = true;
	int32_t eagerTree = TREE_NONE;
};
TracePlan PlanTrace(const Scene& sc, const RendererSettings& st, bool hasSky, const RenderKnobs& knobs);
int32_t EagerTree(const Scene& sc);

struct LaunchPlan {
	uint32_t batch = 1;
	uint32_t sampleCount = 0;
	uint64_t jobs = 0;
	uint32_t blocks = 1, stackStride = 0, jobChunk = 64, heads = 1, jobsPerHead = 0, guideShift = 0;
};
LaunchPlan PlanLaunch(uint32_t numLocalCells, uint32_t numActive, uint32_t spp, uint32_t sampleBegin, int numCUs, int workgroupsPerCU,
                      const TracePlan& trace, const RenderKnobs& knobs);

struct QueryPlan {
	bool ok = true;
	int32_t tree = TREE_BVH2;
	uint32_t treeWidth = 2, nodeBytes = 64;
	int stack = 32;
	bool prims = false;
	bool early = false;
};
QueryPlan PlanQuery(const Scene& sc, int32_t kind, const RenderKnobs& knobs);
QueryPlan PlanGBuffer(const Scene& sc, const RenderKnobs& knobs);
QueryPlan PlanQueryAll(const Scene& sc, const RenderKnobs& knobs);
QueryPlan PlanRadiance(const Scene& sc, const RenderKnobs& knobs);
QueryPlan PlanNearest(const Scene& sc, int32_t kind, const RenderKnobs& knobs);
QueryPlan PlanNearestAll(const Scene& sc, const RenderKnobs& knobs);
struct DistanceFieldPlan { QueryPlan nearest, rows; };
DistanceFieldPlan PlanDistanceField(const Scene& sc, const RenderKnobs& knobs);
QueryPlan PlanOverlap(const Scene& sc, int32_t kind, const RenderKnobs& knobs);

struct GatherCut { uint32_t pointsPer = 0, samplesPer = 0; uint64_t pointRanges = 0, sampleRanges = 0, launches = 0; };
struct GatherLaunch { uint32_t pointFirst, numPoints, sampleBase, numSamples; bool first, last; };
GatherCut PlanGatherCut(uint32_t n, uint32_t sampleCount, bool sphere, const RenderKnobs& knobs);
GatherLaunch GatherLaunchAt(const GatherCut& c, uint32_t n, uint32_t sampleCount, uint64_t k);

struct ViewsPlan {
	bool ok = false;
	uint32_t cellsPerView = 0, numCells = 0, numActive = 0;
	std::vector<uint32_t> active;
	std::vector<unsigned char> empty;
	std::vector<uint32_t> culledPerView;
	uint64_t emptyPixels = 0;
	float emptyL[3] = { 0, 0, 0 };
	uint32_t raysPerSample = 1;
	RenderKnobs knobs;
	LaunchPlan launch;
};
ViewsPlan PlanViews(const CullScene& cs, const RendererSettings& st, const DCamera* cameras, uint32_t count, const TracePlan& trace,
                    int numCUs, int workgroupsPerCU, const RenderKnobs& knobs);
// ... 4 lines not shown
```

### software-raytracing_amd/csrc/rl_rt.h

```cpp
#pragma once

#include "rl_kernels.h"
#include "rl_plan.h"

#include <algorithm>
#include <chrono>
#include <condition_variable>
#include <functional>
#include <map>
#include <mutex>
#include <thread>

namespace rl {

#define HIP_OK(expr) do { hipError_t e_ = (expr); if (e_ != hipSuccess) { \
	Log("HIP error %s at %s:%d: %s", hipGetErrorName(e_), __FILE__, __LINE__, #expr); return false; } } while (0)
#define HIP_TRY(expr) do { hipError_t e_ = (expr); if (e_ != hipSuccess) { \
	Log("HIP error %s at %s:%d: %s", hipGetErrorName(e_), __FILE__, __LINE__, #expr); ok = false; } } while (0)

template <typename T, bool PINNED = false>
struct DevBuf {
	T* ptr = nullptr;
	size_t bytes = 0;
	DevBuf() = default;
// ... 72 lines not shown
struct RcclApi {
	bool tried = false, ok = false;
	void* lib = nullptr;
	int (*CommInitAll)(void** comms, int ndev, const int* devlist) = nullptr;
	int (*CommDestroy)(void* comm) = nullptr;
	int (*Send)(const void* buf, size_t count, int dtype, int peer, void* comm, hipStream_t stream) = nullptr;
	int (*Recv)(void* buf, size_t count, int dtype, int peer, void* comm, hipStream_t stream) = nullptr;
	int (*GroupStart)() = nullptr;
	int (*GroupEnd)() = nullptr;
	const char* (*GetErrorString)(int) = nullptr;
	std::vector<void*> comms;
};
constexpr int kRcclFloat = 7;

struct Worker {
	std::mutex m;
	std::condition_variable cv;
	std::function<bool()> job;
	bool pending = false, result = true;
	void Start(int device)
	{
		std::thread([this, device]() {
			(void)hipSetDevice(device);
			for (;;) {
				std::function<bool()> f;
				{ std::unique_lock<std::mutex> lk(m); cv.wait(lk, [&] { return pending; }); f = job; }
				const bool r = f();
				{ std::lock_guard<std::mutex> lk(m); result = r; pending = false; }
				cv.notify_all();
			}
		}).detach();
	}
	void Post(std::function<bool()> f) { { std::lock_guard<std::mutex> lk(m); job = std::move(f); pending = true; } cv.notify_all(); }
	bool Wait() { std::unique_lock<std::mutex> lk(m); cv.wait(lk, [&] { return !pending; }); return result; }
};

#define RL_QUERY_RING 64
struct RankCtx {
	int rank = 0, device = 0, devSlot = 0, numCUs = 0;
	hipStream_t stream = nullptr;
	hipEvent_t ev[2][8] = {};
	PinBuf<unsigned long long> cntHost[2];
	DevBuf<SampleRGB> samples;
	DevBuf<float4> accum, image;
	DevBuf<float> pathStack;
	DevBuf<float4> cells;
	DevBuf<unsigned long long> counters;
	DevBuf<unsigned int> jobCounter;
	DevBuf<float4> litList; DevBuf<uint32_t> litCtl;
	DevBuf<uint32_t> litMask;
	PinBuf<uint32_t> cellListHost[2]; DevBuf<uint32_t> cellList[2]; size_t cellListCells[2] = { 0, 0 };
	std::vector<unsigned char> cullKey[2];
	uint32_t cullActive[2] = { 0, 0 }; uint64_t cullEmptyPixels[2] = { 0, 0 }; float cullL[2][3] = { { 0, 0, 0 }, { 0, 0, 0 } }; uint32_t cullRays[2] = { 1, 1 };
	std::map<const void*, int> occupancy;
	Worker* worker = nullptr;
	DevBuf<float4> qRays;
	DevBuf<void> qOut, qPrim;
	DevBuf<void> qContact;
	DevBuf<void> qPlane3, qPlane4, qPlane5, qPlane6;
	DevBuf<uint32_t> sdfBits;
	hipEvent_t sdfEv = nullptr; bool sdfEvUsed = false;
	DevBuf<unsigned int> qRing; hipEvent_t qRingEv[RL_QUERY_RING] = {}; bool qRingUsed[RL_QUERY_RING] = {}; uint32_t qRingNext = 0;
	DevBuf<unsigned long long> qStats; PinBuf<unsigned long long> qStatsHost;
	hipEvent_t qEv[2] = { nullptr, nullptr };
	DevBuf<unsigned int> radCounter;
	DevBuf<float> radStack;
	hipEvent_t radEv = nullptr; bool radEvUsed = false;
	DevBuf<float4> gSamples;
	DevBuf<float> gAcc;
	std::vector<hipEvent_t> gEv;
	DevBuf<float> gaState;
	DevBuf<uint8_t> gaStopped;
	DevBuf<uint32_t> gaCounts, gaLive[2], gaTiles;
	DevBuf<float4> gaPoints[2];
	PinBuf<uint32_t> gaHost;
	DevBuf<DLmTri> lmRec; DevBuf<unsigned long long> lmCounts, lmSums; DevBuf<float> lmUv;
	DevBuf<uint32_t> lmOwner, lmRank, lmTexel; DevBuf<float4> lmPoints; DevBuf<float> lmValues, lmFilt, lmAtlas[2]; DevBuf<uint8_t> lmCov[2];
	PinBuf<unsigned long long> lmHost;
	hipEvent_t lmEv[6] = {};
	DevBuf<uint32_t> lmSamples, lmSampleAtlas;
	hipEvent_t lmInEv = nullptr;
};

struct Runtime {
	bool probed = false, ok = false;
	std::vector<RankCtx*> ranks;
	std::vector<int> devices;
	DevBuf<float4> gather[2];
	hipStream_t gatherStream = nullptr;
	bool gatherSelf = false, wantRccl = true, pipeline = true;
	uint64_t frameNo = 0;
	struct Inflight;
	Inflight* inflight[2] = { nullptr, nullptr };
	RaylibAMDStats deferredStats = {};
	bool deferredUnreported = false;
	uint64_t statsSerial = 0;
	RcclApi rccl;
	std::mutex lock;
};
Runtime& Rt();
inline RankCtx& Rank0() { return *Rt().ranks[0]; }

struct PendingRender {
	bool pathTrace = false, lastBatchPending = false;
	float traceMs = 0.0f;
	uint32_t launches = 0, jobHeads = 0, pathsPerWave = 64, treeWidth = 2, nodeBytes = 64;
	uint64_t pixels = 0;
	uint64_t culledSamples = 0; uint32_t culledRaysPerSample = 0, culledSkyTexels = 0;
	uint32_t culledCells = 0, listedCells = 0;
	bool lazy = false;
	bool enqueuedToEnd = false;
	float4* out = nullptr; size_t outBytes = 0;
	int slot = 0;
	const unsigned long long* cnt = nullptr;
};

bool EnsureRuntime();
bool EnsureRccl();
int OccupancyOf(RankCtx& R, const void* kernel, const TracePlan* megakernel = nullptr);
bool UploadScene(Scene& sc);
bool SyncSky(Scene& sc);
bool EnsureWideTree(DeviceSceneCopy* C, Scene& sc, int32_t tree);
bool SettleMove(Scene& sc);
bool SyncMovedLocked(Scene& sc);
bool ReadbackLocked(Image& img);
bool EnqueueRender(RankCtx& R, Scene& sc, const RenderRequest& req, PendingRender& pend, ProgressiveSession* prog = nullptr);
bool FinishRender(RankCtx& R, PendingRender& pend, RaylibAMDStats& stats);
bool OnDevice(const void* p, int device);
bool GatherLocked(Scene& sc, RankCtx& R, int32_t kind, const RaylibAMDRadianceParams& prm, uint64_t seed, const void* points, int32_t n, float* out, bool hostMem, void* stream,
                  std::chrono::steady_clock::time_point t0, RaylibAMDStats& stats, const RaylibAMDGatherAdaptiveParams* A = nullptr, uint32_t* outSamples = nullptr);
bool EnqueueGatherCompact(const uint32_t* live, uint32_t numLive, const uint8_t* stopped, const float4* points, uint32_t* outLive, float4* outPoints, uint32_t* tiles,
                          uint32_t* countHost, hipStream_t st);
bool DrainLocked();

inline void SceneStats(RaylibAMDStats& stats, const Scene& sc)
{
	stats.numNodes = (uint32_t)sc.bvh.nodes.size(); stats.numTriangles = (uint32_t)sc.triangles.size(); stats.bvhDepth = sc.bvh.depth;
}
inline void OneRankStats(RaylibAMDStats& stats, const Scene& sc) { stats.ranks = 1; stats.devices = 1; SceneStats(stats, sc); }
inline double MsSince(std::chrono::steady_clock::time_point t0) { return std::chrono::duration<double, std::milli>(std::chrono::steady_clock::now() - t0).count(); }

}
```

### software-raytracing_amd/csrc/rl_rt_frame.hip

```cpp
#include "rl_rt.h"

#include <atomic>

namespace rl {

typedef void (*TraceKernel)(const DRenderParams, const DSceneView, const SkyRot, SampleRGB*, float*, unsigned long long*, unsigned int*);
typedef void (*TraceViewsKernel)(const DRenderParams, const DSceneView, const SkyRot, SampleRGB*, float*, unsigned long long*, unsigned int*, const DViews);
typedef void (*TraceLazyKernel)(const DRenderParams, const DSceneView, const SkyRot, SampleRGB*, float*, unsigned long long*, unsigned int*, const DLitList);
typedef void (*AovKernel)(const DRenderParams, const DSceneView, float4*, unsigned long long*);
typedef void (*AovViewsKernel)(const DRenderParams, const DSceneView, float4*, unsigned long long*, const DViews);

template <int STACK, bool PRIMS, bool FULL, int LDS = 0, bool PLAIN = false>
static const void* Trace(bool views)
{
	return views ? (const void*)(TraceViewsKernel)k_trace_views<STACK, PRIMS, FULL, LDS, PLAIN> : (const void*)(TraceKernel)k_trace<STACK, PRIMS, FULL, LDS, PLAIN>;
}
template <int STACK, bool PRIMS>
static const void* TraceFor(bool floatBoxes, bool views) { return floatBoxes ? Trace<STACK, PRIMS, true>(views) : Trace<STACK, PRIMS, false>(views); }
template <int STACK, bool PRIMS>
static const void* Aov(bool views) { return views ? (const void*)(AovViewsKernel)k_aov_views<STACK, PRIMS> : (const void*)(AovKernel)k_aov<STACK, PRIMS>; }
static const void* KernelFor(const TracePlan& p, bool views)
{
	if (p.poolK > 0) {
		const int wide = p.tree == TREE_WIDE8 ? 3 : p.tree == TREE_GRID4 ? 1 : 0;
#define RL_POOL_PICK(a, b, c, d, e) if (p.stack == a && p.prims == b && p.poolK == c && p.lstack == d && wide == e) \
			return views ? (const void*)(TraceViewsKernel)k_trace_pool_views<a, b, c, d, e> : (const void*)(TraceKernel)k_trace_pool<a, b, c, d, e>;
		RL_POOL_INSTANCES(RL_POOL_PICK)
#undef RL_POOL_PICK
		return nullptr;
	}
	if (p.lds == 2 && p.lazy && p.hitQueue && !views) return (const void*)(TraceLazyKernel)k_trace_lazy_hitq<16, false, true, 2, true>;
	if (p.lds == 2 && p.lazy && !views) return (const void*)(TraceLazyKernel)k_trace_lazy<16, false, true, 2, true>;
	if (p.lds == 2) return p.plain ? Trace<16, false, true, 2, true>(views) : Trace<16, false, true, 2>(views);
	if (p.lds == 1) return Trace<16, false, true, 1>(views);
	const bool full = p.tree == TREE_BOX4;
	if (p.stack == 16) return TraceFor<16, false>(full, views);
	if (p.stack == 32) return p.prims ? TraceFor<32, true>(full, views) : TraceFor<32, false>(full, views);
	return p.prims ? TraceFor<64, true>(full, views) : TraceFor<64, false>(full, views);
}
static const void* AovKernelFor(const TracePlan& p, bool views)
{
	if (p.stack == 16) return Aov<16, false>(views);
	if (p.stack == 32) return p.prims ? Aov<32, true>(views) : Aov<32, false>(views);
	return p.prims ? Aov<64, true>(views) : Aov<64, false>(views);
}
static std::atomic<int32_t> g_lastTracePlain{0};
int32_t DeviceLastTracePlain() { return g_lastTracePlain.load(std::memory_order_relaxed); }
static std::atomic<int32_t> g_lastTraceLazy{0};
int32_t DeviceLastTraceLazy() { return g_lastTraceLazy.load(std::memory_order_relaxed); }
static std::atomic<int32_t> g_lastHitQueue{0};
int32_t DeviceLastHitQueue() { return g_lastHitQueue.load(std::memory_order_relaxed); }
static std::atomic<int32_t> g_lastLitMask{0};
int32_t DeviceLastLitMask() { return g_lastLitMask.load(std::memory_order_relaxed); }

struct Frame {
	RenderKnobs knobs;
	TracePlan plan;
	DSceneView view;
	DRenderParams P;
	uint32_t numLive = 0, numActive = 0;
	uint32_t sBegin = 0, sEnd = 1;
	float4* out = nullptr;
	const DViews* views = nullptr;
	const void* resolve = nullptr;
	void* resolveArgs[5] = {};
	int firstBatch = 0, lastBatch = 0;
	bool accum = true;
	ProgressiveSession* compact = nullptr;
};

static DRenderParams BaseParams(const RendererSettings& st, uint64_t seed, const DCamera& camera, uint32_t cellFirst, uint32_t stride, uint32_t numLocalCells, bool rowMajor)
{
	DRenderParams P; memset(&P, 0, sizeof(P));
	const uint32_t W = st.viewportWidth, H = st.viewportHeight, cellsX = (W + 7) / 8;
	P.width = W; P.height = H; P.spp = (uint32_t)(st.samplesPerPixel > 1 ? st.samplesPerPixel : 1); P.maxPathLength = st.maxPathLength; P.rayTMin = st.rayTMin;
	P.invWidth = 1.0f / (float)W; P.invHeight = 1.0f / (float)H;
	P.renderMode = st.renderMode; P.seed = seed; P.cellsX = cellsX; P.cellsY = (H + 7) / 8;
	P.cellFirst = cellFirst; P.cellStride = stride; P.numLocalCells = numLocalCells;
	P.rowMajorOutput = rowMajor ? 1u : 0u; P.camera = camera;
	P.seedMixed = raylib_rng_mix64(seed);
	P.magicCellsX = cellsX > 1 ? (uint32_t)(0x100000000ull / cellsX) : 0xFFFFFFFFu;
	return P;
}

static uint64_t CoveredPixels(uint32_t W, uint32_t H, uint32_t cellFirst, uint32_t stride, uint32_t count)
{
	const uint32_t cellsX = (W + 7) / 8;
	uint64_t px = 0;
	for (uint32_t k = 0; k < count; ++k) {
		const uint32_t cell = cellFirst + k * stride, cx = cell % cellsX, cy = cell / cellsX;
		px += (uint64_t)std::min(8u, W - cx * 8) * std::min(8u, H - cy * 8);
	}
	return px;
}

static bool TraceView(DeviceSceneCopy* D, Scene& sc, const TracePlan& plan, DSceneView& view)
{
	if (!EnsureWideTree(D, sc, plan.tree)) return false;
	view = D->view;
	if (!plan.keepNodes4) view.nodes4 = nullptr;
	if (!plan.keepNodes4f) view.nodes4f = nullptr;
	return true;
}

static void ListCells(Frame& F, PendingRender& pend, const uint32_t* list, const uint8_t* empty, uint32_t numListed, uint32_t numLive, const float* L, uint64_t emptyPixels, uint32_t raysPerSample)
{
	DRenderParams& P = F.P;
	F.numLive = numLive; F.numActive = numListed;
	P.activeCells = list; P.cellEmpty = empty; P.numActiveCells = numListed;
	P.emptyL[0] = L[0]; P.emptyL[1] = L[1]; P.emptyL[2] = L[2];
	P.emptySky = F.view.sky ? 1u : 0u;
	pend.culledSamples = emptyPixels * (uint64_t)(F.sEnd - F.sBegin); pend.culledRaysPerSample = raysPerSample; pend.culledSkyTexels = F.view.sky ? 1u : 0u;
}

static bool BeginFrame(RankCtx& R, int q, const Frame& F, size_t outBytes, PendingRender& pend)
{
	pend.pathTrace = F.plan.pathTrace; pend.slot = q; pend.cnt = R.cntHost[q].ptr;
	pend.out = F.out; pend.outBytes = outBytes;
	HIP_OK(hipMemsetAsync(R.counters.ptr, 0, RL_CNT_BLOCK * sizeof(unsigned long long), R.stream));
	HIP_OK(hipEventRecord(R.ev[q][0], R.stream));
	return true;
}

static bool EnqueueFrame(RankCtx& R, int q, const DeviceScene& DS, Frame& F, PendingRender& pend)
{
	const TracePlan& plan = F.plan;
	DRenderParams& P = F.P;
	const uint32_t numCells = P.numLocalCells, numSlots = numCells * 64u;
	const uint32_t rblocks = (numSlots + RL_BLOCK - 1) / RL_BLOCK;
	SkyRot skyRot = DS.skyRot;
	if (numSlots == 0) {
	} else if (!plan.pathTrace) {
		void* args[] = { &P, &F.view, &F.out, &R.counters.ptr, (void*)F.views };
		HIP_OK(hipLaunchKernel(AovKernelFor(plan, F.views != nullptr), dim3(rblocks), dim3(RL_BLOCK), args, 0, R.stream));
	} else {
		const void* traceKernel = KernelFor(plan, F.views != nullptr);
		if (!traceKernel) { Log("Raylib_Render: no megakernel instance for STACK %d, K %d, stack in LDS %d", plan.stack, plan.poolK, plan.lstack); return false; }
		const int blocksPerCU = OccupancyOf(R, traceKernel, &plan);
		if (blocksPerCU < 0) return false;
		g_lastTracePlain.store(plan.plain ? 1 : 0, std::memory_order_relaxed);
		const bool lazy = plan.lazy && !F.views;
		g_lastTraceLazy.store(lazy ? 1 : 0, std::memory_order_relaxed);
		g_lastHitQueue.store(lazy && plan.hitQueue ? 1 : 0, std::memory_order_relaxed);
		pend.lazy = lazy;
		DLitList LL = {};
		pend.pathsPerWave = plan.pathsPerWave; pend.treeWidth = plan.treeWidth; pend.nodeBytes = plan.nodeBytes;
		pend.culledCells = F.numLive - F.numActive; pend.listedCells = F.numActive;
		const uint32_t batch = PlanLaunch(numCells, F.numActive, F.sEnd, F.sBegin, R.numCUs, blocksPerCU, plan, F.knobs).batch;
		if (!R.samples.Grow((size_t)numSlots * sizeof(SampleRGB) * std::min(batch, F.sEnd - F.sBegin))) return false;
		if (F.accum && batch < P.spp && !R.accum.Grow((size_t)numSlots * sizeof(float4))) return false;
		const bool masked = lazy && F.resolve == (const void*)k_resolve && F.knobs.litMask != 0 && (F.knobs.litMask > 0 || !F.view.hasSun) &&
		                    (std::min(batch, F.sEnd - F.sBegin) + 31u) / 32u <= RL_LIT_MASK_MAX_WORDS;
		g_lastLitMask.store(masked ? 1 : 0, std::memory_order_relaxed);
		const void* resolveKernel = masked ? (const void*)k_resolve_lit : F.resolve;
		const int depthSlots = P.maxPathLength > 1 ? P.maxPathLength : 1;
		void* traceArgs[] = { &P, &F.view, &skyRot, &R.samples.ptr, &R.pathStack.ptr, &R.counters.ptr, &R.jobCounter.ptr, lazy ? (void*)&LL : (void*)F.views };
		void* foldArgs[] = { &F.view, &LL, &R.samples.ptr, (void*)&numSlots };
		void* resolveArgs[] = { &P, &F.view, &skyRot, &R.samples.ptr, F.resolveArgs[0], F.resolveArgs[1], F.resolveArgs[2], F.resolveArgs[3], masked ? (void*)&LL : F.resolveArgs[4] };
		for (uint32_t s0 = F.sBegin; s0 < F.sEnd; s0 += batch) {
			const LaunchPlan L = PlanLaunch(numCells, F.numActive, F.sEnd, s0, R.numCUs, blocksPerCU, plan, F.knobs);
			const uint32_t cnt = L.sampleCount;
			P.sampleBegin = s0; P.sampleCount = cnt;
			P.magicSamples = cnt > 1 ? (uint32_t)(0x100000000ull / cnt) : 0xFFFFFFFFu;
			if (L.jobs > 0xF0000000ull) { Log("Raylib_Render: job count overflow"); return false; }
			P.numJobs = (uint32_t)L.jobs;
			P.stackStride = L.stackStride; P.jobChunk = L.jobChunk;
			P.numHeads = L.heads; P.jobsPerHead = L.jobsPerHead; P.guideShift = L.guideShift;
			if (!R.pathStack.Grow((size_t)depthSlots * 8 * P.stackStride * sizeof(float))) return false;
			if (lazy) {
				const uint64_t want = F.knobs.litList >= 0 ? (uint64_t)F.knobs.litList
				                                           : std::max<uint64_t>(4096, L.jobs / 32) + (uint64_t)L.blocks * (RL_BLOCK / 64) * RL_LIT_CHUNK;
				const uint32_t chunks = (uint32_t)std::min<uint64_t>(want / RL_LIT_CHUNK, 0x7FFFFFFFu / RL_LIT_CHUNK);
				if (!R.litList.Grow(std::max<size_t>(1, chunks) * RL_LIT_CHUNK * RL_LIT_STRIDE * sizeof(float4))) return false;
				if (!R.litCtl.Grow((RL_LIT_CTL + (size_t)chunks) * sizeof(uint32_t))) return false;
				LL.entries = (float*)R.litList.ptr; LL.ctl = R.litCtl.ptr; LL.numChunks = chunks;
				HIP_OK(hipMemsetAsync(R.litCtl.ptr, 0, (RL_LIT_CTL + (size_t)chunks) * sizeof(uint32_t), R.stream));
				if (masked) {
					const uint32_t words = (cnt + 31u) / 32u;
					const size_t bytes = (size_t)words * numSlots * sizeof(uint32_t);
					if (!R.litMask.Grow(bytes)) return false;
					LL.mask = R.litMask.ptr; LL.maskWords = words;
					HIP_OK(hipMemsetAsync(R.litMask.ptr, 0, bytes, R.stream));
				}
			}
			pend.jobHeads = L.heads;
			F.firstBatch = s0 == F.sBegin; F.lastBatch = s0 + cnt >= F.sEnd;
			HIP_OK(hipMemsetAsync(R.jobCounter.ptr, 0, RL_MAX_HEADS * RL_HEAD_STRIDE * sizeof(unsigned int), R.stream));
			HIP_OK(hipEventRecord(R.ev[q][2], R.stream));
			if (L.jobs > 0)
				HIP_OK(hipLaunchKernel(traceKernel, dim3(L.blocks), dim3(RL_BLOCK), traceArgs, 0, R.stream));
			if (L.jobs > 0 && lazy && LL.numChunks > 0)
				HIP_OK(hipLaunchKernel((const void*)k_fold_lit, dim3(std::min<uint32_t>((LL.numChunks + 3u) / 4u, (uint32_t)R.numCUs * 8u)), dim3(RL_BLOCK), foldArgs, 0, R.stream));
			HIP_OK(hipEventRecord(R.ev[q][3], R.stream));
			HIP_OK(hipLaunchKernel(resolveKernel, dim3(rblocks), dim3(RL_BLOCK), resolveArgs, 0, R.stream));
			++pend.launches;
			if (!F.lastBatch) {
				HIP_OK(hipEventSynchronize(R.ev[q][3]));
				float ms = 0.0f;
				HIP_OK(hipEventElapsedTime(&ms, R.ev[q][2], R.ev[q][3]));
				pend.traceMs += ms;
			} else pend.lastBatchPending = true;
		}
		if (ProgressiveSession* S = F.compact) {
			hipLaunchKernelGGL(k_progressive_compact, dim3(1), dim3(RL_COMPACT_BLOCK), 0, R.stream,
			                   S->live.ptr, S->trace.ptr, (const uint8_t*)S->st.stopped, (const uint8_t*)S->empty.ptr, S->numLive, P.width, P.height, P.cellsX, S->counts.ptr);
			HIP_OK(hipGetLastError());
			HIP_OK(hipMemcpyAsync(S->countsHost.ptr, S->counts.ptr, 4 * sizeof(uint32_t), hipMemcpyDeviceToHost, R.stream));
		}
	}
// ... 19 lines not shown
	const uint32_t stride = req.cellStride ? req.cellStride : 1;
	const uint32_t numLocalCells = req.cellFirst < numCells ? (numCells - req.cellFirst + stride - 1) / stride : 0;
	const bool rowMajor = (stride == 1 && req.cellFirst == 0 && !req.cellMajor);
	const int q = req.slot & 1;
	F.P = BaseParams(st, req.seed, req.camera, req.cellFirst, stride, numLocalCells, rowMajor);
	F.numLive = F.numActive = numLocalCells;
	F.sBegin = prog ? prog->samples : 0u; F.sEnd = prog ? prog->passEnd : F.P.spp;
	const size_t outBytes = rowMajor ? (size_t)W * H * sizeof(float4) : (size_t)numLocalCells * 64u * sizeof(float4);
	F.out = (float4*)req.outDevice;
	if (!F.out) { if (!R.image.Grow(outBytes ? outBytes : 16)) return false; F.out = R.image.ptr; }
	if (!BeginFrame(R, q, F, outBytes, pend)) return false;
	if (F.plan.pathTrace && numLocalCells && (!prog || !prog->seeded)) {
		const CullScene cs = SceneCullScene(sc, F.view.sky != nullptr);
		std::vector<unsigned char> key;
		auto put = [&](const void* ptr, size_t n) { const unsigned char* b = (const unsigned char*)ptr; key.insert(key.end(), b, b + n); };
		const uint32_t geo[7] = { W, H, req.cellFirst, stride, numLocalCells, (uint32_t)st.maxPathLength, __builtin_bit_cast(uint32_t, st.rayTMin) };
		const int flags[3] = { cs.hasSky ? 1 : 0, cs.hasSun ? 1 : 0, F.knobs.cullCells };
		put(&req.camera, sizeof(req.camera)); put(geo, sizeof(geo)); put(flags, sizeof(flags)); put(cs.sunDirection, sizeof(cs.sunDirection));
		put(cs.sunIlluminance, sizeof(cs.sunIlluminance)); put(cs.boundsMin, sizeof(cs.boundsMin)); put(cs.boundsMax, sizeof(cs.boundsMax));
		const void* sceneId = sc.device; put(&sceneId, sizeof(sceneId));
		if (key != R.cullKey[q]) {
			CullResult cr;
			const bool culled = CullCells(cs, req.camera, st.maxPathLength, st.rayTMin, W, H, cellsX, req.cellFirst, stride, numLocalCells, cr);
			R.cullKey[q].clear();
			R.cullActive[q] = numLocalCells; R.cullEmptyPixels[q] = 0;
			if (culled) {
				if (R.cellListCells[q] < numLocalCells) {
					R.cellListCells[q] = 0;
					if (!R.cellListHost[q].Grow((size_t)numLocalCells * 5 + 16) || !R.cellList[q].Grow((size_t)numLocalCells * 5 + 16)) return false;
					R.cellListCells[q] = numLocalCells;
				}
				memcpy(R.cellListHost[q].ptr, cr.active.data(), cr.active.size() * sizeof(uint32_t));
				memcpy((unsigned char*)(R.cellListHost[q].ptr + R.cellListCells[q]), cr.empty.data(), numLocalCells);
				HIP_OK(hipMemcpyAsync(R.cellList[q].ptr, R.cellListHost[q].ptr, (size_t)R.cellListCells[q] * 5, hipMemcpyHostToDevice, R.stream));
				R.cullActive[q] = (uint32_t)cr.active.size(); R.cullEmptyPixels[q] = cr.emptyPixels;
				R.cullL[q][0] = cr.L[0]; R.cullL[q][1] = cr.L[1]; R.cullL[q][2] = cr.L[2]; R.cullRays[q] = cr.raysPerSample;
			}
			R.cullKey[q] = key;
		}
		const uint32_t* list = R.cellList[q].ptr; const uint8_t* empty = (const uint8_t*)(R.cellList[q].ptr + R.cellListCells[q]);
		if (!prog) {
			if (R.cullActive[q] < numLocalCells) ListCells(F, pend, list, empty, R.cullActive[q], numLocalCells, R.cullL[q], R.cullEmptyPixels[q], R.cullRays[q]);
		} else {
			if (R.cullActive[q] < numLocalCells) {
				HIP_OK(hipMemcpyAsync(prog->trace.ptr, list, (size_t)R.cullActive[q] * sizeof(uint32_t), hipMemcpyDeviceToDevice, R.stream));
				HIP_OK(hipMemcpyAsync(prog->empty.ptr, empty, numLocalCells, hipMemcpyDeviceToDevice, R.stream));
				prog->emptyLivePixels = R.cullEmptyPixels[q]; prog->culledRays = R.cullRays[q];
				for (int k = 0; k < 3; ++k) prog->emptyL[k] = R.cullL[q][k];
			}
			prog->numLive = numLocalCells; prog->numTrace = R.cullActive[q];
			prog->seeded = true;
		}
	}
	if (prog) {
		if (F.plan.pathTrace && numLocalCells) ListCells(F, pend, prog->trace.ptr, prog->empty.ptr, prog->numTrace, prog->numLive, prog->emptyL, prog->emptyLivePixels, prog->culledRays);
		F.resolve = (const void*)k_progressive_resolve; F.resolveArgs[0] = &prog->st; F.resolveArgs[1] = &F.out; F.resolveArgs[2] = &F.lastBatch;
		F.accum = false; F.compact = prog;
	} else {
		F.resolve = (const void*)k_resolve; F.resolveArgs[0] = &R.accum.ptr; F.resolveArgs[1] = &F.out; F.resolveArgs[2] = &F.firstBatch; F.resolveArgs[3] = &F.lastBatch;
	}
	if (!EnqueueFrame(R, q, *sc.device, F, pend)) return false;
	pend.pixels = CoveredPixels(W, H, req.cellFirst, stride, numLocalCells);
	return true;
}

static bool PrintStamps(RankCtx& R, const unsigned long long* cnt)
{
	(void)R;
#ifdef RL_DIAG_TIMELINE
	if (getenv("RAYLIB_PRINT_STAMPS")) {
		std::vector<unsigned long long> tl(RL_TIMELINE_SLOTS);
		HIP_OK(hipMemcpy(tl.data(), R.counters.ptr + CNT_COUNT + 24, tl.size() * sizeof(unsigned long long), hipMemcpyDeviceToHost));
		std::vector<double> st, ex, en;
		unsigned long long t0 = ~0ull;
		for (int w = 0; w < 8192; ++w) if (tl[w] && tl[w] < t0) t0 = tl[w];
		for (int w = 0; w < 8192; ++w) if (tl[w]) { st.push_back((tl[w] - t0) * 0.01); if (tl[8192 + w]) ex.push_back((tl[8192 + w] - t0) * 0.01); en.push_back((tl[16384 + w] - t0) * 0.01); }
		auto pct = [](std::vector<double>& v, double q) { if (v.empty()) return 0.0; std::sort(v.begin(), v.end()); return v[(size_t)(q * (v.size() - 1))]; };
		Log("timeline (us from the first wave's start; last launch, %d waves): start p50 %.1f max %.1f | queue seen empty min %.1f p50 %.1f max %.1f | end min %.1f p10 %.1f p50 %.1f p90 %.1f max %.1f",
			(int)st.size(), pct(st, 0.5), pct(st, 1.0), pct(ex, 0.0), pct(ex, 0.5), pct(ex, 1.0), pct(en, 0.0), pct(en, 0.1), pct(en, 0.5), pct(en, 0.9), pct(en, 1.0));
		for (unsigned x = 0; x < 8; ++x) {
			std::vector<double> xe, xn;
			for (int w = 0; w < 8192; ++w) if (tl[w] && tl[24576 + w] == x) { if (tl[8192 + w]) xe.push_back((tl[8192 + w] - t0) * 0.01); xn.push_back((tl[16384 + w] - t0) * 0.01); }
			if (!xn.empty()) Log("   XCC %u: %d waves | job list seen empty min %.1f p50 %.1f max %.1f | end min %.1f p50 %.1f max %.1f", x, (int)xn.size(), pct(xe, 0.0), pct(xe, 0.5), pct(xe, 1.0), pct(xn, 0.0), pct(xn, 0.5), pct(xn, 1.0));
		}
	}
#endif
#ifdef RL_DIAG_TOPN
	if (getenv("RAYLIB_PRINT_STAMPS")) {
		const double n = (double)cnt[CNT_NODES] + 1e-9;
		Log("node steps by node number (breadth first): < 9: %.3f  < 22: %.3f  < 53: %.3f  < 73: %.3f  < 128: %.3f  < 256: %.3f  < 1024: %.3f  beyond: %.3f (cumulative shares of %.0f steps)",
		    cnt[CNT_COUNT + 4] / n, (cnt[CNT_COUNT + 4] + cnt[CNT_COUNT + 5]) / n, (cnt[CNT_COUNT + 4] + cnt[CNT_COUNT + 5] + cnt[CNT_COUNT + 6]) / n,
		    (cnt[CNT_COUNT + 4] + cnt[CNT_COUNT + 5] + cnt[CNT_COUNT + 6] + cnt[CNT_COUNT + 7]) / n, (cnt[CNT_COUNT + 4] + cnt[CNT_COUNT + 5] + cnt[CNT_COUNT + 6] + cnt[CNT_COUNT + 7] + cnt[CNT_COUNT + 8]) / n,
		    (cnt[CNT_COUNT + 4] + cnt[CNT_COUNT + 5] + cnt[CNT_COUNT + 6] + cnt[CNT_COUNT + 7] + cnt[CNT_COUNT + 8] + cnt[CNT_COUNT + 9]) / n,
		    (cnt[CNT_COUNT + 4] + cnt[CNT_COUNT + 5] + cnt[CNT_COUNT + 6] + cnt[CNT_COUNT + 7] + cnt[CNT_COUNT + 8] + cnt[CNT_COUNT + 9] + cnt[CNT_COUNT + 10]) / n, cnt[CNT_COUNT + 11] / n, n);
		Log("groups on the stack at a node step: 0: %.3f  1: %.3f  2: %.3f  3: %.3f  4: %.3f  5: %.3f  6-7: %.3f  8+: %.3f", cnt[CNT_COUNT + 16] / n, cnt[CNT_COUNT + 17] / n, cnt[CNT_COUNT + 18] / n,
		    cnt[CNT_COUNT + 19] / n, cnt[CNT_COUNT + 20] / n, cnt[CNT_COUNT + 21] / n, cnt[CNT_COUNT + 22] / n, cnt[CNT_COUNT + 23] / n);
	}
#else
	if (getenv("RAYLIB_PRINT_STAMPS")) {
		const double tot = (double)(cnt[CNT_COUNT] + cnt[CNT_COUNT + 1] + cnt[CNT_COUNT + 2] + cnt[CNT_COUNT + 3]);
		Log("wave steps: node %llu (lane steps %llu, eff %.3f)  tri %llu (lane %llu, eff %.3f)  leaf rounds %llu  trips %llu", cnt[CNT_COUNT + 4], cnt[CNT_NODES], cnt[CNT_NODES] / (64.0 * cnt[CNT_COUNT + 4] + 1), cnt[CNT_COUNT + 5], cnt[CNT_TRIS], cnt[CNT_TRIS] / (64.0 * cnt[CNT_COUNT + 5] + 1), cnt[CNT_COUNT + 6], cnt[CNT_TRIPS]);
#if defined(RL_DIAG_STAMPS) && RL_DIAG_STAMPS >= 2
		if (cnt[CNT_COUNT + 7]) Log("leaf list: %llu triangle wave steps taken; %llu if every round's (ray, triangle) pairs were dealt evenly to the wave's 64 lanes (the bound of any regrouping: a round cannot take less than one step)", cnt[CNT_COUNT + 5], cnt[CNT_COUNT + 7]);
#endif
		Log("diagnostic slots (wave level): [4] %llu [5] %llu [6] %llu [7] %llu [16] %llu [17] %llu [18] %llu [19] %llu trips %llu", cnt[CNT_COUNT + 4], cnt[CNT_COUNT + 5], cnt[CNT_COUNT + 6], cnt[CNT_COUNT + 7],
		    cnt[CNT_COUNT + 16], cnt[CNT_COUNT + 17], cnt[CNT_COUNT + 18], cnt[CNT_COUNT + 19], cnt[CNT_TRIPS]);
		if (tot > 0) Log("shade split (of all): surface+material %.3f scatter %.3f emit+store %.3f", cnt[CNT_COUNT + 8] / tot, cnt[CNT_COUNT + 9] / tot, cnt[CNT_COUNT + 10] / tot);
		if (tot > 0) Log("microfacet split (of all): setup %.3f beckmann sample %.3f brdf+pdf %.3f | newton wave iters %llu lane iters %llu (eff %.3f) | microfacet wave calls %llu lanes %llu (eff %.3f)", cnt[CNT_COUNT + 12] / tot, cnt[CNT_COUNT + 13] / tot, cnt[CNT_COUNT + 14] / tot, cnt[CNT_COUNT + 16], cnt[CNT_COUNT + 17], cnt[CNT_COUNT + 17] / (64.0 * cnt[CNT_COUNT + 16] + 1), cnt[CNT_COUNT + 18], cnt[CNT_COUNT + 19], cnt[CNT_COUNT + 19] / (64.0 * cnt[CNT_COUNT + 18] + 1));
		{
			static const char* nm[4] = { "traverse", "shade a hit", "miss shader", "fold + store" };
			for (int k = 0; k < 4; ++k) if (cnt[CNT_COUNT + 4 + k] && cnt[CNT_COUNT + 20 + k])
				Log("  %-12s clock share %.3f, lanes taking part %.3f (level-1 diagnostic build)", nm[k], cnt[CNT_COUNT + 4 + k] / tot, cnt[CNT_COUNT + 20 + k] / (64.0 * cnt[CNT_COUNT + 4 + k]));
		}
		if (tot > 0) Log("phase shares (shader clock): refill %.3f traverse %.3f shade %.3f fold %.3f", cnt[CNT_COUNT] / tot, cnt[CNT_COUNT + 1] / tot, cnt[CNT_COUNT + 2] / tot, cnt[CNT_COUNT + 3] / tot);
	}
#endif
// ... 115 lines not shown
```

### software-raytracing_amd/csrc/rl_rt_render.hip

```cpp
#include "rl_rt.h"

namespace rl {

struct Runtime::Inflight {
	std::vector<PendingRender> pend;
	RaylibAMDStats stats;
	int slot = 0;
	uint64_t serial = 0;
	bool ok = true, timed = false;
	std::chrono::steady_clock::time_point t0;
};

static bool FinishInflight(int slot)
{
	Runtime& R = Rt();
	Runtime::Inflight* F = R.inflight[slot];
	if (!F) return true;
	R.inflight[slot] = nullptr;
	RankCtx& R0 = Rank0();
	bool ok = F->ok;
	for (int r = (int)F->pend.size() - 1; r >= 0; --r) {
		ok = FinishRender(*R.ranks[(size_t)r], F->pend[(size_t)r], F->stats) && ok;
	}
	(void)hipSetDevice(R0.device);
// ... 94 lines not shown
			RankCtx& C = *R.ranks[(size_t)r];
			const size_t floats = (size_t)local[(size_t)r] * 64 * 4;
			rc = A.Recv(gather + plan.offset[r], floats, kRcclFloat, C.devSlot, A.comms[(size_t)R0.devSlot], R.gatherStream);
			if (rc == 0) rc = A.Send(C.cells.ptr, floats, kRcclFloat, R0.devSlot, A.comms[(size_t)C.devSlot], sendStream(C));
		}
		const int rcEnd = A.GroupEnd();
		if (rc != 0 || rcEnd != 0) { Log("Raylib_Render: RCCL gather failed (%s)", A.GetErrorString ? A.GetErrorString(rc ? rc : rcEnd) : "?"); ok = false; }
		for (size_t sl = 0; sl < lead.size() && ok; ++sl) {
			if (lead[sl] < 0 || (int)sl == R0.devSlot) continue;
			RankCtx& L = *R.ranks[(size_t)lead[sl]];
			(void)hipSetDevice(L.device);
			HIP_TRY(hipEventRecord(L.ev[b][5], L.stream));
			for (int r = 0; r < N; ++r) if (r != lead[sl] && remote[(size_t)r] && R.ranks[(size_t)r]->devSlot == (int)sl) HIP_TRY(hipStreamWaitEvent(R.ranks[(size_t)r]->stream, L.ev[b][5], 0));
		}
		(void)hipSetDevice(R0.device);
	}
	if (ok) {
		for (int r = 0; r < N; ++r) HIP_TRY(hipStreamWaitEvent(R.gatherStream, R.ranks[(size_t)r]->ev[b][4], 0));
		HIP_TRY(hipEventRecord(R0.ev[b][5], R.gatherStream));
		const uint32_t blocks = (uint32_t)(((size_t)W * H + RL_BLOCK - 1) / RL_BLOCK);
		hipLaunchKernelGGL(k_scatter_cells, dim3(blocks), dim3(RL_BLOCK), 0, R.gatherStream, (const float4*)gather, out, W, H, cellsX, plan);
		HIP_TRY(hipGetLastError());
		if (req.outHostRGBA) HIP_TRY(hipMemcpyAsync(req.outHostRGBA, out, frameBytes, hipMemcpyDeviceToHost, R.gatherStream));
		HIP_TRY(hipEventRecord(R0.ev[b][6], R.gatherStream));
		if (remote[0] && useRccl) HIP_TRY(hipStreamWaitEvent(R0.stream, R0.ev[b][5], 0));
		F->timed = ok;
	}
	F->ok = ok;
	F->stats.ranks = (uint32_t)N; F->stats.devices = (uint32_t)R.devices.size();
	F->stats.gatherMode = !anyRemote ? 0u : (useRccl ? 1u : 2u);
	F->stats.rcclCommSize = R.rccl.ok ? (uint32_t)R.rccl.comms.size() : 0u;
	SceneStats(F->stats, sc);
	R.inflight[b] = F;
	++R.frameNo;
	if (!ok || !R.pipeline || req.outHostRGBA || req.callerOwnsOut) {
		ok = DrainLocked() && ok;
		stats = R.deferredStats; R.deferredUnreported = false;
		return ok;
	}
	stats = F->stats;
	deferred = true;
	return ok;
}

bool DeviceRender(Scene& sc, const RenderRequest& req, RaylibAMDStats& stats)
{
	Runtime& RT = Rt();
	std::lock_guard<std::mutex> lk(RT.lock);
	const auto t0 = std::chrono::steady_clock::now();
	if (!EnsureRuntime()) return false;
	HIP_OK(hipSetDevice(Rank0().device));
	if (!UploadScene(sc)) return false;
	if (!SyncSky(sc)) return false;
	bool ok;
	const bool whole = req.cellFirst == 0 && (req.cellStride == 0 || req.cellStride == 1);
	if (whole && (RT.ranks.size() > 1 || RT.gatherSelf)) {
		bool deferred = false;
		ok = RenderMulti(sc, req, stats, deferred);
		if (deferred) return ok;
	} else {
		(void)DrainLocked();
		RT.deferredUnreported = false;
		PendingRender pend;
		ok = EnqueueRender(Rank0(), sc, req, pend);
		if (ok && req.outHostRGBA) HIP_OK(hipMemcpyAsync(req.outHostRGBA, pend.out, pend.outBytes, hipMemcpyDeviceToHost, Rank0().stream));
		ok = FinishRender(Rank0(), pend, stats) && ok;
		stats.ranks = 1; stats.devices = 1;
	}
	SceneStats(stats, sc);
	if (!(whole && (RT.ranks.size() > 1 || RT.gatherSelf))) stats.wallMs = MsSince(t0);
	return ok;
}

static bool AllocProgressive(ProgressiveSession& S)
{
	const size_t slots = (size_t)S.numCells * 64u, cells = S.numCells;
	if (!S.sum.Grow(slots * sizeof(float4)) || !S.s1.Grow(slots * sizeof(float)) || !S.s2.Grow(slots * sizeof(float))) return false;
	if (!S.cellSamples.Grow(cells * sizeof(uint32_t)) || !S.stopped.Grow(cells)) return false;
	if (!S.live.Grow(cells * sizeof(uint32_t)) || !S.trace.Grow(cells * sizeof(uint32_t)) || !S.empty.Grow(cells)) return false;
	if (!S.counts.Grow(4 * sizeof(uint32_t)) || !S.countsHost.Grow(4 * sizeof(uint32_t))) return false;
	S.st.sum = S.sum.ptr; S.st.s1 = S.s1.ptr; S.st.s2 = S.s2.ptr; S.st.cellSamples = S.cellSamples.ptr; S.st.stopped = S.stopped.ptr;
	HIP_OK(hipMemset(S.st.sum, 0, slots * sizeof(float4)));
	HIP_OK(hipMemset(S.st.s1, 0, slots * sizeof(float)));
	HIP_OK(hipMemset(S.st.s2, 0, slots * sizeof(float)));
	HIP_OK(hipMemset(S.st.cellSamples, 0, cells * sizeof(uint32_t)));
	HIP_OK(hipMemset(S.st.stopped, 0, cells));
	HIP_OK(hipMemset(S.empty.ptr, 0, cells));
	std::vector<uint32_t> all(cells);
	for (size_t c = 0; c < cells; ++c) all[c] = (uint32_t)c;
	HIP_OK(hipMemcpy(S.live.ptr, all.data(), cells * sizeof(uint32_t), hipMemcpyHostToDevice));
	HIP_OK(hipMemcpy(S.trace.ptr, all.data(), cells * sizeof(uint32_t), hipMemcpyHostToDevice));
	return true;
}

ProgressiveSession* DeviceProgressiveBegin(Scene& sc, const RenderRequest& req, float threshold, uint32_t minSamples)
{
	std::lock_guard<std::mutex> lk(Rt().lock);
	if (!EnsureRuntime()) return nullptr;
	if (hipSetDevice(Rank0().device) != hipSuccess) return nullptr;
	if (!UploadScene(sc) || !SyncSky(sc)) return nullptr;
	(void)DrainLocked();
	ProgressiveSession* S = new ProgressiveSession;
	S->scene = &sc; S->sceneSerial = sc.device->serial;
	S->sky = sc.sky; S->skyVersion = sc.sky ? sc.sky->version : 0;
	S->accelT0 = sc.accelT0; S->accelT1 = sc.accelT1;
	S->req = req; S->req.cellFirst = 0; S->req.cellStride = 1; S->req.cellMajor = false; S->req.slot = 0;
	S->req.outDevice = nullptr; S->req.outHostRGBA = nullptr; S->req.callerOwnsOut = false;
	S->width = req.settings.viewportWidth; S->height = req.settings.viewportHeight;
	S->numCells = ((S->width + 7) / 8) * ((S->height + 7) / 8);
	S->cap = (uint32_t)(req.settings.samplesPerPixel > 1 ? req.settings.samplesPerPixel : 1);
	S->st.threshold = threshold; S->st.minSamples = minSamples;
	S->numLive = S->numTrace = S->numCells;
	if (!AllocProgressive(*S)) { Log("RaylibAMD_BeginProgressive: the session's buffers could not be allocated"); delete S; return nullptr; }
	return S;
}

int32_t DeviceProgressiveStep(ProgressiveSession& S, uint32_t samples, void* outDevice, RaylibAMDStats& stats, bool& rendered)
{
	std::lock_guard<std::mutex> lk(Rt().lock);
	const auto t0 = std::chrono::steady_clock::now();
	rendered = false;
	if (!Rt().ok) return -1;
	Scene& sc = *S.scene;
	if (!sc.device || sc.device->serial != S.sceneSerial || sc.accelT0 != S.accelT0 || sc.accelT1 != S.accelT1) {
		Log("RaylibAMD_ProgressiveStep: the scene changed since the session began (finalized, sun or shutter); the image is unchanged");
		return -1;
	}
	if (sc.sky != S.sky || (sc.sky && sc.sky->version != S.skyVersion)) {
		Log("RaylibAMD_ProgressiveStep: the scene's sky panorama changed since the session began; the image is unchanged");
		return -1;
	}
	if (S.samples >= S.cap || S.numLive == 0) return 0;
	const uint32_t cnt = std::min(samples, S.cap - S.samples);
	(void)DrainLocked();
	Rt().deferredUnreported = false;
	if (hipSetDevice(Rank0().device) != hipSuccess || !SyncSky(sc)) return -1;
	S.passEnd = S.samples + cnt;
	RenderRequest req = S.req;
	req.outDevice = outDevice;
	PendingRender pend;
	bool ok = EnqueueRender(Rank0(), sc, req, pend, &S);
	ok = FinishRender(Rank0(), pend, stats) && ok;
	if (!ok) return -1;
	rendered = true;
	S.samples += cnt; ++S.passes;
	S.numLive = S.countsHost.ptr[0]; S.numTrace = S.countsHost.ptr[1];
	S.emptyLivePixels = (uint64_t)S.countsHost.ptr[2] | ((uint64_t)S.countsHost.ptr[3] << 32);
	OneRankStats(stats, sc);
	stats.wallMs = MsSince(t0);
	return S.samples >= S.cap ? 0 : (int32_t)S.numLive;
}

bool DeviceProgressiveExport(ProgressiveSession& S, uint32_t* cellSamples, uint8_t* cellStopped, float* sumY, float* sumY2)
{
	std::lock_guard<std::mutex> lk(Rt().lock);
	if (!Rt().ok) return false;
	HIP_OK(hipSetDevice(Rank0().device));
	if (cellSamples) HIP_OK(hipMemcpy(cellSamples, S.st.cellSamples, (size_t)S.numCells * sizeof(uint32_t), hipMemcpyDeviceToHost));
	if (cellStopped) HIP_OK(hipMemcpy(cellStopped, S.st.stopped, S.numCells, hipMemcpyDeviceToHost));
	const uint32_t cellsX = (S.width + 7) / 8;
	std::vector<float> slots((size_t)S.numCells * 64u);
	for (int m = 0; m < 2; ++m) {
		float* dst = m ? sumY2 : sumY;
		if (!dst) continue;
		HIP_OK(hipMemcpy(slots.data(), m ? S.st.s2 : S.st.s1, slots.size() * sizeof(float), hipMemcpyDeviceToHost));
		for (uint32_t y = 0; y < S.height; ++y)
			for (uint32_t x = 0; x < S.width; ++x) dst[(size_t)y * S.width + x] = slots[((size_t)(y / 8) * cellsX + x / 8) * 64u + (y % 8) * 8u + x % 8];
	}
	return true;
}

void DeviceProgressiveEnd(ProgressiveSession* S)
{
	if (!S) return;
	std::lock_guard<std::mutex> lk(Rt().lock);
	if (Rt().ok) (void)hipSetDevice(Rank0().device);
	delete S;
}

}
```

### software-raytracing_amd/raylib_amd/binding.py

```python
import ctypes as C
import os
import numpy as np

HERE = os.path.dirname(os.path.abspath(__file__))
LIB_PATH = os.environ.get("RAYLIB_LIB") or os.path.join(os.path.dirname(HERE), "libraylib.so")

RENDERMODE_DEFAULT, RENDERMODE_ALBEDO, RENDERMODE_SURFACE_NORMAL, RENDERMODE_MICROSURFACE_NORMAL, \
    RENDERMODE_TEXCOORD, RENDERMODE_EMISSION, RENDERMODE_REFLECTANCE = range(7)


class RendererSettings(C.Structure):
    _fields_ = [("viewportWidth", C.c_uint32), ("viewportHeight", C.c_uint32),
                ("samplesPerPixel", C.c_int32), ("maxPathLength", C.c_int32),
                ("rayTMin", C.c_float), ("renderMode", C.c_uint32)]


class DenoiseParams(C.Structure):
    _fields_ = [("iterations", C.c_int32), ("sigmaColor", C.c_float), ("sigmaNormal", C.c_float), ("sigmaAlbedo", C.c_float)]


class ProgressiveParams(C.Structure):
    _fields_ = [("threshold", C.c_float), ("minSamples", C.c_uint32)]


class Stats(C.Structure):
    _fields_ = [("rays", C.c_uint64), ("nodesVisited", C.c_uint64), ("trisTested", C.c_uint64),
                ("shadedHits", C.c_uint64), ("texFetches", C.c_uint64), ("cameraSamples", C.c_uint64),
                ("pixels", C.c_uint64), ("kernelMs", C.c_double), ("traceKernelMs", C.c_double), ("wallMs", C.c_double),
                ("traceLaunches", C.c_uint32), ("numNodes", C.c_uint32), ("numTriangles", C.c_uint32), ("bvhDepth", C.c_uint32),
                ("waveTrips", C.c_uint64), ("pathsPerWave", C.c_uint32), ("ranks", C.c_uint32),
                ("gatherMode", C.c_uint32), ("rcclCommSize", C.c_uint32), ("devices", C.c_uint32), ("jobHeads", C.c_uint32),
                ("gatherMs", C.c_double), ("scatterMs", C.c_double), ("rankKernelMs", C.c_double * 16), ("rankTraceMs", C.c_double * 16),
                ("culledCells", C.c_uint32), ("listedCells", C.c_uint32), ("culledSamples", C.c_uint64), ("culledRays", C.c_uint64),
                ("treeWidth", C.c_uint32), ("nodeBytes", C.c_uint32), ("litPaths", C.c_uint64), ("litFoldedInPlace", C.c_uint64)]

    GATHER_MODES = {0: "none", 1: "rccl", 2: "peer"}

    def as_dict(self):
        d = {k: getattr(self, k) for k, _ in self._fields_}
        d["rankKernelMs"] = list(self.rankKernelMs)[: max(1, self.ranks)]
        d["rankTraceMs"] = list(self.rankTraceMs)[: max(1, self.ranks)]
        d["gatherMode"] = self.GATHER_MODES.get(self.gatherMode, "?")
        d["frameSamples"] = self.cameraSamples + self.culledSamples
        d["frameRays"] = self.rays + self.culledRays
        d["frameNodes"] = self.nodesVisited + self.culledRays
        return d


class RenderPlan(C.Structure):
    _fields_ = [(k, C.c_int32) for k in ("pathTrace", "stack", "prims", "poolK", "tree", "lstack", "lds", "plain")] + \
               [(k, C.c_uint32) for k in ("pathsPerWave", "treeWidth", "nodeBytes")] + \
               [(k, C.c_int32) for k in ("keepNodes4", "keepNodes4f", "eagerTree")] + \
               [(k, C.c_uint32) for k in ("batch", "sampleCount", "blocks", "stackStride", "jobChunk", "heads", "jobsPerHead", "guideShift")] + \
               [("jobs", C.c_uint64), ("lazy", C.c_int32), ("hitQueue", C.c_int32)]
    TREES = {0: "none", 1: "bvh2", 2: "box4", 3: "grid4", 4: "wide8"}

    def as_dict(self):
        return {k: getattr(self, k) for k, _ in self._fields_}


class Ray(C.Structure):
    _fields_ = [("org", C.c_float * 3), ("tMin", C.c_float), ("dir", C.c_float * 3), ("tMax", C.c_float)]


class HitT(C.Structure):
    _fields_ = [("t", C.c_float), ("prim", C.c_int32), ("b1", C.c_float), ("b2", C.c_float)]


class QueryPlan(C.Structure):
    _fields_ = [("tree", C.c_int32), ("treeWidth", C.c_uint32), ("nodeBytes", C.c_uint32), ("stack", C.c_int32), ("prims", C.c_int32), ("early", C.c_int32)]

    def as_dict(self):
        return {k: getattr(self, k) for k, _ in self._fields_}


QUERY_ANY, QUERY_CLOSEST, QUERY_SURFACE = 0, 1, 2
PRIM_SPHERE, PRIM_CUBE = 0x10000000, 0x20000000
HITT_DTYPE = np.dtype([("t", "f4"), ("prim", "i4"), ("b1", "f4"), ("b2", "f4")])
SURFACE_DTYPE = np.dtype([("hit", "i4"), ("t", "f4"), ("p", "f4", 3), ("n", "f4", 3), ("paramU", "f4"), ("paramV", "f4"), ("material", "i4")])
_QUERY_DTYPES = {QUERY_ANY: np.dtype("u4"), QUERY_CLOSEST: HITT_DTYPE, QUERY_SURFACE: SURFACE_DTYPE}
_TORCH_WORDS = {QUERY_ANY: 1, QUERY_CLOSEST: 4, QUERY_SURFACE: 11}


def _plan(lib, entry, scene, *args):
    p = QueryPlan()
    r = getattr(lib, entry)(scene, *args, C.byref(p))
    return r, p.as_dict()


def _ordered(stream):
    if stream.cuda_stream == 0:
        stream.synchronize()
    return C.c_void_p(stream.cuda_stream)


def _query(lib, scene, data, cols, entry, specs, pre=(), mid=(), host=False, device=False, records=None, type_error="", host_error=None):
    if isinstance(data, np.ndarray) and not device:
        d = np.ascontiguousarray(data)
        d = d.view(np.uint8).reshape(-1, records.itemsize) if records is not None and d.dtype == records else np.ascontiguousarray(d, np.float32).reshape(-1, cols)
        n = len(d)
        outs = [None if s is None else np.zeros(s[0], s[1]) for s in specs(n)]
        name = entry + "Host" if host else entry
        if getattr(lib, name)(scene, *pre, d.ctypes.data, n, *mid, *[None if o is None else o.ctypes.data for o in outs]) != 1:
            raise RuntimeError(name + " refused the query")
        return outs
    import torch
    if host:
# ... 722 lines not shown
    "RaylibAMD_OverlapContactsHost": (C.c_int32, [C.c_void_p, C.c_uint32, C.c_void_p, C.c_int32, C.c_int32, C.c_void_p, C.c_void_p, C.c_void_p]),
    "RaylibAMD_PlanOverlapContacts": (C.c_int32, [C.c_void_p, C.POINTER(QueryPlan)]),
    "RaylibAMD_Gather": (C.c_int32, [C.c_void_p, C.POINTER(GatherParams), C.POINTER(GatherPoint), C.c_int32, C.POINTER(C.c_float)]),
    "RaylibAMD_GatherDevice": (C.c_int32, [C.c_void_p, C.POINTER(GatherParams), C.POINTER(GatherPoint), C.c_int32, C.POINTER(C.c_float), C.c_void_p]),
    "RaylibAMD_GatherDirectionsHost": (C.c_int32, [C.POINTER(GatherParams), C.POINTER(GatherPoint), C.c_int32, C.c_uint64, C.c_uint32, C.POINTER(C.c_float)]),
    "RaylibAMD_PlanGatherCut": (C.c_int32, [C.POINTER(GatherParams), C.c_int32, C.c_uint64, C.POINTER(GatherCut)]),
    "RaylibAMD_GatherAdaptive": (C.c_int32, [C.c_void_p, C.POINTER(GatherParams), C.POINTER(GatherAdaptiveParams), C.POINTER(GatherPoint), C.c_int32, C.POINTER(C.c_float),
                                             C.POINTER(C.c_uint32)]),
    "RaylibAMD_GatherAdaptiveDevice": (C.c_int32, [C.c_void_p, C.POINTER(GatherParams), C.POINTER(GatherAdaptiveParams), C.POINTER(GatherPoint), C.c_int32, C.POINTER(C.c_float),
                                                   C.POINTER(C.c_uint32), C.c_void_p]),
    "RaylibAMD_GatherAdaptiveDecideHost": (C.c_int32, [C.POINTER(GatherAdaptiveParams), C.c_uint32, C.POINTER(C.c_float), C.c_int64, C.POINTER(C.c_uint32)]),
    "RaylibAMD_GatherCompactTest": (C.c_int32, [C.POINTER(C.c_uint32), C.c_uint32, C.POINTER(C.c_uint8), C.POINTER(GatherPoint), C.c_uint32, C.POINTER(C.c_uint32),
                                                C.POINTER(GatherPoint), C.POINTER(C.c_uint32)]),
    "RaylibAMD_BakeLightmapAdaptive": (C.c_int32, [C.c_void_p, C.POINTER(LightmapParams), C.POINTER(GatherAdaptiveParams), C.POINTER(C.c_float), C.POINTER(C.c_float),
                                                   C.POINTER(C.c_uint8), C.POINTER(C.c_uint32)]),
    "RaylibAMD_BakeLightmapAdaptiveDevice": (C.c_int32, [C.c_void_p, C.POINTER(LightmapParams), C.POINTER(GatherAdaptiveParams), C.POINTER(C.c_float), C.POINTER(C.c_float),
                                                         C.POINTER(C.c_uint8), C.POINTER(C.c_uint32), C.c_void_p]),
    "RaylibAMD_LightmapPoints": (C.c_int64, [C.c_void_p, C.POINTER(LightmapParams), C.POINTER(C.c_float), C.POINTER(GatherPoint), C.POINTER(C.c_uint32), C.c_int64]),
    "RaylibAMD_LightmapPointsHost": (C.c_int64, [C.c_void_p, C.POINTER(LightmapParams), C.POINTER(C.c_float), C.POINTER(GatherPoint), C.POINTER(C.c_uint32), C.c_int64]),
    "RaylibAMD_BakeLightmap": (C.c_int32, [C.c_void_p, C.POINTER(LightmapParams), C.POINTER(C.c_float), C.POINTER(C.c_float), C.POINTER(C.c_uint8)]),
    "RaylibAMD_BakeLightmapDevice": (C.c_int32, [C.c_void_p, C.POINTER(LightmapParams), C.POINTER(C.c_float), C.POINTER(C.c_float), C.POINTER(C.c_uint8), C.c_void_p]),
    "RaylibAMD_BakeLightmapFiltered": (C.c_int32, [C.c_void_p, C.POINTER(LightmapParams), C.POINTER(LightmapFilterParams), C.POINTER(C.c_float), C.POINTER(C.c_float), C.POINTER(C.c_uint8)]),
    "RaylibAMD_BakeLightmapFilteredDevice": (C.c_int32, [C.c_void_p, C.POINTER(LightmapParams), C.POINTER(LightmapFilterParams), C.POINTER(C.c_float), C.POINTER(C.c_float), C.POINTER(C.c_uint8),
                                                         C.c_void_p]),
    "RaylibAMD_FilterLightmap": (C.c_int32, [C.c_void_p, C.POINTER(LightmapParams), C.POINTER(LightmapFilterParams), C.POINTER(C.c_float), C.POINTER(C.c_float), C.POINTER(C.c_float),
                                             C.POINTER(C.c_uint8)]),
    "RaylibAMD_FilterLightmapDevice": (C.c_int32, [C.c_void_p, C.POINTER(LightmapParams), C.POINTER(LightmapFilterParams), C.POINTER(C.c_float), C.POINTER(C.c_float), C.POINTER(C.c_float),
                                                   C.POINTER(C.c_uint8), C.c_void_p]),
    "RaylibAMD_FilterLightmapHost": (C.c_int32, [C.c_int32, C.c_int32, C.c_int32, C.POINTER(LightmapFilterParams), C.POINTER(GatherPoint), C.POINTER(C.c_uint32), C.c_int64,
                                                 C.POINTER(C.c_float), C.POINTER(C.c_float)]),
    "RaylibAMD_VerifyExactMath": (C.c_int32, [C.c_int32, C.POINTER(C.c_uint64), C.POINTER(C.c_uint64)]),
    "RaylibAMD_CullCells": (C.c_int32, [C.c_void_p, C.POINTER(C.c_float), C.POINTER(C.c_float), C.POINTER(C.c_float), C.c_int32, C.c_int32, C.POINTER(C.c_uint8), C.POINTER(C.c_float)]),
    "RaylibAMD_SceneNumTriangles": (C.c_int32, [C.c_void_p]),
    "RaylibAMD_SceneNumMaterials": (C.c_int32, [C.c_void_p]),
    "RaylibAMD_SceneNumTextures": (C.c_int32, [C.c_void_p]),
    "RaylibAMD_SceneExportTriangles": (None, [C.c_void_p, C.c_void_p]),
    "RaylibAMD_SceneExportTriOrder": (C.c_int32, [C.c_void_p, C.POINTER(C.c_uint32)]),
    "RaylibAMD_SceneExportMaterials": (None, [C.c_void_p, C.c_void_p]),
    "RaylibAMD_SceneTextureSize": (None, [C.c_void_p, C.c_int32, C.POINTER(C.c_int32), C.POINTER(C.c_int32)]),
    "RaylibAMD_SceneExportTexture": (None, [C.c_void_p, C.c_int32, C.POINTER(C.c_float)]),
    "RaylibAMD_SceneGetSun": (None, [C.c_void_p, C.POINTER(C.c_float), C.POINTER(C.c_float)]),
    "RaylibAMD_SceneBVHInfo": (C.c_int32, [C.c_void_p, C.POINTER(C.c_uint32), C.POINTER(C.c_uint32), C.POINTER(C.c_float)]),
    "RaylibAMD_ParseFloat": (C.c_float, [C.c_char_p]),
    "RaylibAMD_ImageSize": (C.c_int32, [C.c_void_p, C.POINTER(C.c_uint32), C.POINTER(C.c_uint32)]),
    "RaylibAMD_SceneBVH4Info": (C.c_int32, [C.c_void_p, C.POINTER(C.c_uint32), C.POINTER(C.c_uint32)]),
    "RaylibAMD_SceneBVH8Info": (C.c_int32, [C.c_void_p, C.POINTER(C.c_uint32), C.POINTER(C.c_uint32), C.POINTER(C.c_float), C.POINTER(C.c_float)]),
    "RaylibAMD_SceneLeafListInfo": (C.c_int32, [C.c_void_p, C.POINTER(C.c_uint32)]),
    "RaylibAMD_ScenePlain": (C.c_int32, [C.c_void_p]),
    "RaylibAMD_LastTracePlain": (C.c_int32, []),
    "RaylibAMD_SceneLazyRefl": (C.c_int32, [C.c_void_p]),
    "RaylibAMD_LastTraceLazy": (C.c_int32, []),
    "RaylibAMD_LastHitQueue": (C.c_int32, []),
    "RaylibAMD_LastLitMask": (C.c_int32, []),
    "RaylibAMD_VerifyLazyRefl": (C.c_int32, [C.c_uint32, C.c_uint64, C.POINTER(C.c_uint64), C.POINTER(C.c_uint64), C.POINTER(C.c_uint64)]),
    "RaylibAMD_VerifyLazyPdf": (C.c_int32, [C.c_uint32, C.c_uint64, C.POINTER(C.c_uint64), C.POINTER(C.c_uint64), C.POINTER(C.c_uint64)]),
    "RaylibAMD_VerifySamplerRanged": (C.c_int32, [C.c_int32, C.POINTER(C.c_uint64), C.POINTER(C.c_uint64), C.POINTER(C.c_uint32), C.POINTER(C.c_uint64)]),
    "RaylibAMD_PlanRender": (C.c_int32, [C.c_void_p, C.POINTER(RendererSettings), C.c_int32, C.c_int32, C.c_int32, C.POINTER(RenderPlan)]),
    "RaylibAMD_SceneWalk8Host": (C.c_int32, [C.c_void_p, C.POINTER(C.c_float), C.c_int32, C.c_float, C.POINTER(C.c_float), C.POINTER(C.c_float), C.POINTER(C.c_uint32)]),
    "RaylibAMD_SceneWalkStackHost": (C.c_int32, [C.c_void_p, C.c_int32, C.POINTER(C.c_float), C.c_int32, C.c_float, C.c_int32, C.POINTER(C.c_float), C.POINTER(C.c_uint32)]),
    "RaylibAMD_SceneBVHHash": (C.c_uint64, [C.c_void_p]),
    "RaylibAMD_SceneTopologyHash": (C.c_uint64, [C.c_void_p]),
    "RaylibAMD_SceneExportBVHNodes": (C.c_int32, [C.c_void_p, C.c_void_p]),
    "RaylibAMD_SceneMoveTriangles": (C.c_int32, [C.c_void_p, C.c_int32, C.c_int32, C.POINTER(C.c_float), C.POINTER(C.c_float)]),
    "RaylibAMD_SceneMoveTrianglesDevice": (C.c_int32, [C.c_void_p, C.c_int32, C.c_int32, C.c_void_p, C.c_void_p, C.c_void_p]),
    "RaylibAMD_SceneRebuild": (C.c_int32, [C.c_void_p]),
    "RaylibAMD_SceneCheckTrees": (C.c_int32, [C.c_void_p, C.POINTER(C.c_uint32)]),
    "RaylibAMD_SceneCompareTrees": (C.c_int32, [C.c_void_p, C.POINTER(C.c_uint32)]),
    "RaylibAMD_CameraExport": (None, [C.c_void_p, C.POINTER(C.c_float)]),
    "RaylibAMD_CreateImageFromData": (C.c_void_p, [C.c_uint32, C.c_uint32, C.POINTER(C.c_float)]),
    "RaylibAMD_DumpImageRGBA": (None, [C.c_void_p, C.POINTER(C.c_float)]),
    "RaylibAMD_OBJModelSetTexture": (C.c_int32, [C.c_void_p, C.c_char_p, C.c_int32, C.c_void_p]),
    "RaylibAMD_Denoise": (C.c_int32, [C.c_void_p, C.c_int32, C.c_void_p, C.c_void_p, C.c_void_p, C.POINTER(DenoiseParams)]),
    "RaylibAMD_DenoiseHost": (C.c_int32, [C.c_uint32, C.c_uint32, C.POINTER(C.c_float), C.c_int32, C.POINTER(C.c_float), C.POINTER(C.c_float),
                                          C.POINTER(DenoiseParams), C.POINTER(C.c_float)]),
    "RaylibAMD_EnableDenoiser": (None, [C.c_int32]),
    "RaylibAMD_BeginProgressive": (C.c_size_t, [C.POINTER(RendererSettings), C.c_void_p, C.c_void_p, C.c_void_p, C.POINTER(ProgressiveParams)]),
    "RaylibAMD_ProgressiveStep": (C.c_int32, [C.c_size_t, C.c_uint32]),
    "RaylibAMD_ProgressiveExport": (C.c_int32, [C.c_size_t, C.POINTER(C.c_uint32), C.POINTER(C.c_uint8), C.POINTER(C.c_float), C.POINTER(C.c_float)]),
    "RaylibAMD_EndProgressive": (C.c_int32, [C.c_size_t]),
    "RaylibAMD_ProgressiveDecideHost": (C.c_int32, [C.c_uint32, C.c_uint32, C.POINTER(C.c_uint32), C.POINTER(C.c_float), C.POINTER(C.c_float),
                                                    C.POINTER(ProgressiveParams), C.POINTER(C.c_uint8)]),
    "RaylibAMD_ProgressiveCompactTest": (C.c_int32, [C.POINTER(C.c_uint32), C.c_uint32, C.POINTER(C.c_uint8), C.POINTER(C.c_uint8), C.c_uint32, C.c_uint32, C.c_uint32,
                                                     C.POINTER(C.c_uint32), C.POINTER(C.c_uint32), C.POINTER(C.c_uint32)]),
    "RaylibAMD_RenderViews": (C.c_int32, [C.POINTER(RendererSettings), C.c_void_p, C.POINTER(C.c_void_p), C.c_int32, C.POINTER(C.c_void_p)]),
    "RaylibAMD_RenderViewsDevice": (C.c_int32, [C.POINTER(RendererSettings), C.c_void_p, C.POINTER(C.c_void_p), C.c_int32, C.c_void_p]),
    "RaylibAMD_PlanViews": (C.c_int32, [C.c_void_p, C.POINTER(RendererSettings), C.POINTER(C.c_void_p), C.c_int32, C.c_int32, C.c_int32, C.c_int32,
                                        C.POINTER(RenderPlan), C.POINTER(C.c_uint8)]),
}
MAX_VIEWS = 64
RAYLIB_H_EXPORTS = [k for k in _EXPORTS if k.startswith("Raylib_")]
RAYLIB_AMD_H_EXPORTS = [k for k in _EXPORTS if k.startswith("RaylibAMD_")]


def load(path=LIB_PATH):
    if not os.path.exists(path):
        raise FileNotFoundError(path + " -- build it with `make -C software-raytracing_amd` (or __graft_entry__.build())")
    lib = C.CDLL(path)
    for name, (res, args) in _EXPORTS.items():
        if os.environ.get("RAYLIB_LIB") and name.startswith("RaylibAMD_") and not hasattr(lib, name):
            continue
        fn = getattr(lib, name)
        fn.restype, fn.argtypes = res, args
    return lib


def _fp(a):
# ... 238 lines not shown
```

Baseline: 23160.

## Add per-cell leaf-group masks to restrict primary-ray traversal in hit-queue kernel

Computes, on the host, a 32-bit mask per 8x8 screen cell giving which BVH leaf-list groups can be hit by primary rays. Each leaf box is projected onto the camera plane with conservative margins for lens blur and rounding. The mask is uploaded to the device, cached by a key over camera, viewport and leaf data, and passed to the lazy hit-queue trace kernel so it can skip leaf groups that cannot be reached. This adds host work and a transfer whenever the key changes, and correctness depends on the projection bounds being conservative.

```diff
diff --git a/include/raylib_amd.h b/include/raylib_amd.h
--- a/include/raylib_amd.h
+++ b/include/raylib_amd.h
@@ -279,6 +279,8 @@
 
 RAYLIB_API int32_t RaylibAMD_CullCells(CameraHandle camera, const float* bounds, const float* sunIlluminance, const float* sunDirection,
                                        int32_t width, int32_t height, uint8_t* outEmpty, float* outConstant);
+RAYLIB_API int32_t RaylibAMD_CellLeafMasks(SceneHandle scene, CameraHandle camera, const RendererSettings* settings, uint32_t cellFirst, uint32_t stride,
+                                           uint32_t numLocalCells, uint32_t* out);
 
 RAYLIB_API int32_t RaylibAMD_VerifyExactMath(int32_t which, uint64_t* outMismatches, uint64_t* outFirstBits);
 RAYLIB_API int32_t RaylibAMD_VerifyLazyRefl(uint32_t n, uint64_t seed, uint64_t* outEvents, uint64_t* outUnsafe, uint64_t* outGuardFailed);
@@ -306,12 +308,14 @@
 RAYLIB_API int32_t RaylibAMD_SceneWalk8Host(SceneHandle scene, const float* rays, int32_t count, float tMin, const float* tMax, float* outT, uint32_t* outSteps);
 RAYLIB_API int32_t RaylibAMD_SceneWalkStackHost(SceneHandle scene, int32_t tree, const float* rays, int32_t count, float tMin, int32_t capacity, float* outT, uint32_t* outHighWater);
 RAYLIB_API int32_t RaylibAMD_SceneLeafListInfo(SceneHandle scene, uint32_t* outMaxTrianglesPerLeaf);
+RAYLIB_API int32_t RaylibAMD_SceneLeafListBoxes(SceneHandle scene, float* outBoxes, uint8_t* outSlotsUsed);
 RAYLIB_API int32_t RaylibAMD_ScenePlain(SceneHandle scene);
 RAYLIB_API int32_t RaylibAMD_LastTracePlain(void);
 RAYLIB_API int32_t RaylibAMD_SceneLazyRefl(SceneHandle scene);
 RAYLIB_API int32_t RaylibAMD_LastTraceLazy(void);
 RAYLIB_API int32_t RaylibAMD_LastHitQueue(void);
 RAYLIB_API int32_t RaylibAMD_LastLitMask(void);
+RAYLIB_API int32_t RaylibAMD_LastCellLeaves(void);
 typedef struct RaylibAMDRenderPlan {
 	int32_t pathTrace;
 	int32_t stack, prims;
@@ -327,6 +331,8 @@
 	uint64_t jobs;
 	int32_t lazy;
 	int32_t hitQueue;
+	int32_t cellLeaves;
+	int32_t reserved;
 } RaylibAMDRenderPlan;
 RAYLIB_API int32_t RaylibAMD_PlanRender(SceneHandle scene, const RendererSettings* settings, int32_t hasSky, int32_t numCUs, int32_t workgroupsPerCU, RaylibAMDRenderPlan* out);
 #define RAYLIB_AMD_MAX_VIEWS 64
diff --git a/software-raytracing_amd/csrc/rl_abi.cc b/software-raytracing_amd/csrc/rl_abi.cc
--- a/software-raytracing_amd/csrc/rl_abi.cc
+++ b/software-raytracing_amd/csrc/rl_abi.cc
@@ -722,6 +722,15 @@
 	if (outEmpty) memcpy(outEmpty, r.empty.data(), (size_t)cellsX * cellsY);
 	if (outConstant) { outConstant[0] = r.L[0]; outConstant[1] = r.L[1]; outConstant[2] = r.L[2]; }
 	return (int32_t)(cellsX * cellsY - (uint32_t)r.active.size());
+}
+int32_t RaylibAMD_CellLeafMasks(SceneHandle sh, CameraHandle ch, const RendererSettings* settings, uint32_t cellFirst, uint32_t stride, uint32_t numLocalCells, uint32_t* out)
+{
+	Scene* s = (Scene*)sh; Camera* c = (Camera*)ch;
+	if (!s || !s->finalized || !c || !settings || !out || stride == 0 || numLocalCells == 0 || settings->viewportWidth == 0 || settings->viewportHeight == 0) return -1;
+	if (!DeviceSyncMovedScene(*s)) return -1;
+	const uint32_t W = settings->viewportWidth, H = settings->viewportHeight;
+	return CellLeafMasks(SceneCullScene(*s, false), s->bvh.leafList.data(), (uint32_t)s->bvh.leafList.size(), c->ToDevice(), settings->rayTMin, W, H, (W + 7) / 8,
+	                     cellFirst, stride, numLocalCells, out) ? 1 : 0;
 }
 int32_t RaylibAMD_EvalTexture(SceneHandle sh, int32_t texture, int32_t bSRGB, const float* uv, int32_t n, float* out)
 {
@@ -1720,6 +1729,17 @@
 	if (maxPerLeaf) *maxPerLeaf = most;
 	return leaves;
 }
+int32_t RaylibAMD_SceneLeafListBoxes(SceneHandle sh, float* outBoxes, uint8_t* outSlotsUsed)
+{
+	Scene* s = (Scene*)sh;
+	if (!s || !s->finalized || !DeviceSyncMovedScene(*s)) return 0;
+	const std::vector<DNode4>& L = s->bvh.leafList;
+	for (size_t g = 0; g < L.size(); ++g) for (int k = 0; k < 4; ++k) {
+		if (outBoxes) for (int a = 0; a < 3; ++a) { outBoxes[(4 * g + k) * 6 + a] = L[g].lo[a][k]; outBoxes[(4 * g + k) * 6 + 3 + a] = L[g].hi[a][k]; }
+		if (outSlotsUsed) outSlotsUsed[4 * g + k] = L[g].child[k] != DNODE_EMPTY ? 1 : 0;
+	}
+	return (int32_t)L.size();
+}
 int32_t RaylibAMD_ScenePlain(SceneHandle sh)
 {
 	Scene* s = (Scene*)sh;
@@ -1734,6 +1754,7 @@
 int32_t RaylibAMD_LastTraceLazy(void) { return DeviceLastTraceLazy(); }
 int32_t RaylibAMD_LastHitQueue(void) { return DeviceLastHitQueue(); }
 int32_t RaylibAMD_LastLitMask(void) { return DeviceLastLitMask(); }
+int32_t RaylibAMD_LastCellLeaves(void) { return DeviceLastCellLeaves(); }
 int32_t RaylibAMD_PlanRender(SceneHandle sh, const RendererSettings* settings, int32_t hasSky, int32_t numCUs, int32_t workgroupsPerCU, RaylibAMDRenderPlan* out)
 {
 	Scene* s = (Scene*)sh;
@@ -1742,7 +1763,7 @@
 	const RenderKnobs knobs = ReadRenderKnobs();
 	const TracePlan t = PlanTrace(*s, *settings, hasSky != 0, knobs);
 	if (!t.ok) return -1;
-	out->pathTrace = t.pathTrace; out->stack = t.stack; out->prims = t.prims; out->poolK = t.poolK; out->tree = t.tree; out->lstack = t.lstack; out->lds = t.lds; out->plain = t.plain; out->lazy = t.lazy ? 1 : 0; out->hitQueue = t.hitQueue ? 1 : 0;
+	out->pathTrace = t.pathTrace; out->stack = t.stack; out->prims = t.prims; out->poolK = t.poolK; out->tree = t.tree; out->lstack = t.lstack; out->lds = t.lds; out->plain = t.plain; out->lazy = t.lazy ? 1 : 0; out->hitQueue = t.hitQueue ? 1 : 0; out->cellLeaves = t.cellLeaves ? 1 : 0;
 	out->pathsPerWave = t.pathsPerWave; out->treeWidth = t.treeWidth; out->nodeBytes = t.nodeBytes;
 	out->keepNodes4 = t.keepNodes4; out->keepNodes4f = t.keepNodes4f; out->eagerTree = t.eagerTree;
 	const uint32_t cells = ((settings->viewportWidth + 7) / 8) * ((settings->viewportHeight + 7) / 8);
diff --git a/software-raytracing_amd/csrc/rl_cull.cc b/software-raytracing_amd/csrc/rl_cull.cc
--- a/software-raytracing_amd/csrc/rl_cull.cc
+++ b/software-raytracing_amd/csrc/rl_cull.cc
@@ -5,6 +5,48 @@
 #include <stdlib.h>
 
 namespace rl {
+
+namespace {
+
+struct CameraPlane { double O[3], TL[3], E[3], Hh[3], Vv[3], N[3]; double hh, vv, nn, planeDist; };
+struct BoxRect { double uLo, uHi, vLo, vHi, lensFac; };
+inline void sub3(const double* a, const double* b, double* r) { r[0] = a[0] - b[0]; r[1] = a[1] - b[1]; r[2] = a[2] - b[2]; }
+inline double dot3(const double* a, const double* b) { return a[0] * b[0] + a[1] * b[1] + a[2] * b[2]; }
+
+bool CameraPlaneOf(const DCamera& cam, CameraPlane& cp)
+{
+	for (int k = 0; k < 3; ++k) { cp.O[k] = cam.origin[k]; cp.TL[k] = cam.top_left[k]; cp.Hh[k] = cam.horizontal[k]; cp.Vv[k] = cam.vertical[k]; }
+	for (int k = 0; k < 3; ++k) if (!std::isfinite(cp.O[k]) || !std::isfinite(cp.TL[k]) || !std::isfinite(cp.Hh[k]) || !std::isfinite(cp.Vv[k])) return false;
+	sub3(cp.TL, cp.O, cp.E); for (int k = 0; k < 3; ++k) cp.E[k] += cp.Vv[k];
+	const double* Hh = cp.Hh; const double* Vv = cp.Vv;
+	cp.N[0] = Hh[1] * Vv[2] - Hh[2] * Vv[1]; cp.N[1] = Hh[2] * Vv[0] - Hh[0] * Vv[2]; cp.N[2] = Hh[0] * Vv[1] - Hh[1] * Vv[0];
+	cp.hh = dot3(Hh, Hh); cp.vv = dot3(Vv, Vv); cp.nn = dot3(cp.N, cp.N);
+	if (!(cp.hh > 0.0) || !(cp.vv > 0.0) || !(cp.nn > 0.0) || std::fabs(dot3(Hh, Vv)) > 1e-6 * std::sqrt(cp.hh * cp.vv)) return false;
+	cp.planeDist = dot3(cp.E, cp.N);
+	if (cp.planeDist < 0.0) { cp.planeDist = -cp.planeDist; for (int k = 0; k < 3; ++k) cp.N[k] = -cp.N[k]; }
+	return cp.planeDist > 1e-12 * std::sqrt(cp.nn) * std::sqrt(dot3(cp.E, cp.E));
+}
+
+bool ProjectBox(const CameraPlane& cp, const double corners[8][3], double ext, BoxRect& r)
+{
+	r.uLo = 1e300; r.uHi = -1e300; r.vLo = 1e300; r.vHi = -1e300; r.lensFac = 0.0;
+	for (int c = 0; c < 8; ++c) {
+		const double* X = corners[c];
+		double Q[3];
+		sub3(X, cp.O, Q);
+		const double depth = dot3(Q, cp.N);
+		if (!(depth > 1e-9 * std::sqrt(cp.nn) * (std::sqrt(dot3(Q, Q)) + ext))) return false;
+		const double sc = cp.planeDist / depth;
+		r.lensFac = std::max(r.lensFac, std::fabs(1.0 - sc));
+		double R3[3]; for (int k = 0; k < 3; ++k) R3[k] = Q[k] * sc - cp.E[k];
+		const double u = dot3(R3, cp.Hh) / cp.hh, v = -dot3(R3, cp.Vv) / cp.vv;
+		if (!std::isfinite(u) || !std::isfinite(v)) return false;
+		r.uLo = std::min(r.uLo, u); r.uHi = std::max(r.uHi, u); r.vLo = std::min(r.vLo, v); r.vHi = std::max(r.vHi, v);
+	}
+	return true;
+}
+
+}
 
 bool CullCells(const CullScene& DS, const DCamera& cam, int32_t maxPathLength, float rayTMin, uint32_t W, uint32_t H,
                uint32_t cellsX, uint32_t cellFirst, uint32_t stride, uint32_t numLocalCells, CullResult& out)
@@ -14,34 +56,15 @@
 	const double lensR = std::fabs((double)cam.lensRadius);
 	if (!std::isfinite(lensR)) return false;
 	if (!(rayTMin >= 0.0f)) return false;
-	auto sub3 = [](const double* a, const double* b, double* r) { r[0] = a[0] - b[0]; r[1] = a[1] - b[1]; r[2] = a[2] - b[2]; };
-	auto dot3 = [](const double* a, const double* b) { return a[0] * b[0] + a[1] * b[1] + a[2] * b[2]; };
-	const double O[3] = { cam.origin[0], cam.origin[1], cam.origin[2] }, TL[3] = { cam.top_left[0], cam.top_left[1], cam.top_left[2] };
-	const double Hh[3] = { cam.horizontal[0], cam.horizontal[1], cam.horizontal[2] }, Vv[3] = { cam.vertical[0], cam.vertical[1], cam.vertical[2] };
-	for (int k = 0; k < 3; ++k) if (!std::isfinite(O[k]) || !std::isfinite(TL[k]) || !std::isfinite(Hh[k]) || !std::isfinite(Vv[k])) return false;
-	double E[3]; sub3(TL, O, E); for (int k = 0; k < 3; ++k) E[k] += Vv[k];
-	double N[3] = { Hh[1] * Vv[2] - Hh[2] * Vv[1], Hh[2] * Vv[0] - Hh[0] * Vv[2], Hh[0] * Vv[1] - Hh[1] * Vv[0] };
-	const double hh = dot3(Hh, Hh), vv = dot3(Vv, Vv), nn = dot3(N, N);
-	if (!(hh > 0.0) || !(vv > 0.0) || !(nn > 0.0) || std::fabs(dot3(Hh, Vv)) > 1e-6 * std::sqrt(hh * vv)) return false;
-	double planeDist = dot3(E, N);
-	if (planeDist < 0.0) { planeDist = -planeDist; for (int k = 0; k < 3; ++k) N[k] = -N[k]; }
-	if (!(planeDist > 1e-12 * std::sqrt(nn) * std::sqrt(dot3(E, E)))) return false;
+	CameraPlane cp;
+	if (!CameraPlaneOf(cam, cp)) return false;
 	const double ext = std::max({ DS.boundsMax[0] - DS.boundsMin[0], DS.boundsMax[1] - DS.boundsMin[1], DS.boundsMax[2] - DS.boundsMin[2], 1e-30 });
-	double uLo = 1e300, uHi = -1e300, vLo = 1e300, vHi = -1e300;
-	double lensFac = 0.0;
-	for (int c = 0; c < 8; ++c) {
-		double X[3], Q[3];
-		for (int k = 0; k < 3; ++k) X[k] = (c >> k & 1) ? DS.boundsMax[k] + 1e-6 * ext : DS.boundsMin[k] - 1e-6 * ext;
-		sub3(X, O, Q);
-		const double depth = dot3(Q, N);
-		if (!(depth > 1e-9 * std::sqrt(nn) * (std::sqrt(dot3(Q, Q)) + ext))) return false;
-		const double sc = planeDist / depth;
-		lensFac = std::max(lensFac, std::fabs(1.0 - sc));
-		double R3[3]; for (int k = 0; k < 3; ++k) R3[k] = Q[k] * sc - E[k];
-		const double u = dot3(R3, Hh) / hh, v = -dot3(R3, Vv) / vv;
-		if (!std::isfinite(u) || !std::isfinite(v)) return false;
-		uLo = std::min(uLo, u); uHi = std::max(uHi, u); vLo = std::min(vLo, v); vHi = std::max(vHi, v);
-	}
+	double corners[8][3];
+	for (int c = 0; c < 8; ++c) for (int k = 0; k < 3; ++k) corners[c][k] = (c >> k & 1) ? DS.boundsMax[k] + 1e-6 * ext : DS.boundsMin[k] - 1e-6 * ext;
+	BoxRect br;
+	if (!ProjectBox(cp, corners, ext, br)) return false;
+	const double uLo = br.uLo, uHi = br.uHi, vLo = br.vLo, vHi = br.vHi, lensFac = br.lensFac, hh = cp.hh, vv = cp.vv;
+	const double* O = cp.O;
 	const double margin = 2.0;
 	const double cocU = lensR * lensFac / std::sqrt(hh) * 1.0001, cocV = lensR * lensFac / std::sqrt(vv) * 1.0001;
 	if (!std::isfinite(cocU) || !std::isfinite(cocV)) return false;
@@ -81,5 +104,87 @@
 	return out.active.size() < numLocalCells;
 }
 
+bool CellLeafMasks(const CullScene& DS, const DNode4* leafList, uint32_t numRecords, const DCamera& cam, float rayTMin, uint32_t W, uint32_t H,
+                   uint32_t cellsX, uint32_t cellFirst, uint32_t stride, uint32_t numLocalCells, uint32_t* out)
+{
+	if (const char* e = getenv("RAYLIB_CELL_LEAVES")) if (atoi(e) == 0) return false;
+	if (!leafList || numRecords == 0 || numRecords > 32u || !DS.boundsValid || numLocalCells == 0 || !out || W == 0 || H == 0 || cellsX == 0 || stride == 0) return false;
+	const double lensR = std::fabs((double)cam.lensRadius);
+	if (!std::isfinite(lensR)) return false;
+	if (!(rayTMin >= 0.0f)) return false;
+	CameraPlane cp;
+	if (!CameraPlaneOf(cam, cp)) return false;
+	double cu[3], cv[3];
+	for (int k = 0; k < 3; ++k) { cu[k] = cam.u[k]; cv[k] = cam.v[k]; if (!std::isfinite(cu[k]) || !std::isfinite(cv[k])) return false; }
+	const double ext = std::max({ DS.boundsMax[0] - DS.boundsMin[0], DS.boundsMax[1] - DS.boundsMin[1], DS.boundsMax[2] - DS.boundsMin[2], 1e-30 });
+	const double oMax = std::max({ std::fabs(cp.O[0]), std::fabs(cp.O[1]), std::fabs(cp.O[2]) }) + lensR;
+	const uint32_t cellsY = (H + 7) / 8, numCells = cellsX * cellsY;
+	const double margin = 2.0;
+	const uint32_t base = numRecords < 32u ? ~0u << numRecords : 0u;
+	struct Span { uint32_t bit; bool all; int64_t cx0, cx1, cy0, cy1; double xLo, xHi, yLo, yHi; };
+	std::vector<Span> spans; spans.reserve((size_t)numRecords * 4);
+	uint32_t everywhere = base;
+	for (uint32_t g = 0; g < numRecords; ++g) for (int s = 0; s < 4; ++s) {
+		const DNode4& n = leafList[g];
+		if (n.child[s] == DNODE_EMPTY) continue;
+		Span sp; sp.bit = 1u << g; sp.all = true;
+		double lo[3], hi[3], reach = 0.0;
+		bool finite = true;
+		for (int k = 0; k < 3; ++k) { lo[k] = n.lo[k][s]; hi[k] = n.hi[k][s]; if (!std::isfinite(lo[k]) || !std::isfinite(hi[k]) || lo[k] > hi[k]) finite = false; }
+		if (finite) {
+			for (int k = 0; k < 3; ++k) { const double f = std::max(std::fabs(lo[k] - cp.O[k]), std::fabs(hi[k] - cp.O[k])); reach += f * f; }
+			const double grow = 1e-6 * ext + 4e-5 * (std::sqrt(reach) + lensR) + 4.8e-7 * oMax;
+			double corners[8][3];
+			for (int c = 0; c < 8; ++c) for (int k = 0; k < 3; ++k) corners[c][k] = (c >> k & 1) ? hi[k] + grow : lo[k] - grow;
+			BoxRect br;
+			if (ProjectBox(cp, corners, ext, br)) {
+				const double cocU = lensR * br.lensFac / std::sqrt(cp.hh) * 1.0001, cocV = lensR * br.lensFac / std::sqrt(cp.vv) * 1.0001;
+				if (std::isfinite(cocU) && std::isfinite(cocV)) {
+					sp.xLo = (br.uLo - cocU) * W - margin; sp.xHi = (br.uHi + cocU) * W + margin; sp.yLo = (br.vLo - cocV) * H - margin; sp.yHi = (br.vHi + cocV) * H + margin;
+					const double big = 4.0e9;
+					sp.cx0 = (int64_t)std::floor(std::max(-big, std::min(big, (sp.xLo - 8.0) / 8.0))) - 1; sp.cx1 = (int64_t)std::ceil(std::max(-big, std::min(big, (sp.xHi + 1.0) / 8.0))) + 1;
+					sp.cy0 = (int64_t)std::floor(std::max(-big, std::min(big, (sp.yLo - 8.0) / 8.0))) - 1; sp.cy1 = (int64_t)std::ceil(std::max(-big, std::min(big, (sp.yHi + 1.0) / 8.0))) + 1;
+					sp.all = false;
+				}
+			}
+		}
+		if (sp.all) everywhere |= sp.bit; else spans.push_back(sp);
+	}
+	for (uint32_t k = 0; k < numLocalCells; ++k) out[k] = ((uint64_t)cellFirst + (uint64_t)k * stride >= numCells) ? ~0u : everywhere;
+	auto setBits = [&](int64_t cx, int64_t cy, uint32_t bits) {
+		const uint64_t cell = (uint64_t)cy * cellsX + (uint64_t)cx;
+		if (cell < cellFirst || (cell - cellFirst) % stride != 0) return;
+		const uint64_t k = (cell - cellFirst) / stride;
+		if (k < numLocalCells) out[k] |= bits;
+	};
+	for (const Span& sp : spans) {
+		if ((everywhere & sp.bit) != 0u) continue;
+		const int64_t x0 = std::max<int64_t>(0, sp.cx0), x1 = std::min<int64_t>((int64_t)cellsX - 1, sp.cx1), y0 = std::max<int64_t>(0, sp.cy0), y1 = std::min<int64_t>((int64_t)cellsY - 1, sp.cy1);
+		for (int64_t cy = y0; cy <= y1; ++cy) {
+			const double py0 = 8.0 * cy - 1.0, py1 = 8.0 * cy + 8.0;
+			if (py1 < sp.yLo || py0 > sp.yHi) continue;
+			for (int64_t cx = x0; cx <= x1; ++cx) {
+				const double px0 = 8.0 * cx - 1.0, px1 = 8.0 * cx + 8.0;
+				if (px1 < sp.xLo || px0 > sp.xHi) continue;
+				setBits(cx, cy, sp.bit);
+			}
+		}
+	}
+	for (int k = 0; k < 3; ++k) {
+		const double lens = lensR * (std::fabs(cu[k]) + std::fabs(cv[k]));
+		const double slack = lens + 1e-5 * (std::fabs(cp.TL[k]) + std::fabs(cp.Hh[k]) + std::fabs(cp.Vv[k]) + std::fabs(cp.O[k]) + lens) + 1e-30;
+		for (uint32_t cy = 0; cy < cellsY; ++cy) {
+			const double v0 = (8.0 * cy - 1.0) / H, v1 = (8.0 * cy + 8.0) / H;
+			const double bLo = std::min(-v0 * cp.Vv[k], -v1 * cp.Vv[k]), bHi = std::max(-v0 * cp.Vv[k], -v1 * cp.Vv[k]);
+			for (uint32_t cx = 0; cx < cellsX; ++cx) {
+				const double u0 = (8.0 * cx - 1.0) / W, u1 = (8.0 * cx + 8.0) / W;
+				const double fLo = cp.E[k] + std::min(u0 * cp.Hh[k], u1 * cp.Hh[k]) + bLo, fHi = cp.E[k] + std::max(u0 * cp.Hh[k], u1 * cp.Hh[k]) + bHi;
+				if (fLo - slack <= 0.0 && fHi + slack >= 0.0) setBits(cx, cy, ~0u);
+			}
+		}
+	}
+	return true;
+}
+
 
 }
diff --git a/software-raytracing_amd/csrc/rl_dev_jobs.h b/software-raytracing_amd/csrc/rl_dev_jobs.h
--- a/software-raytracing_amd/csrc/rl_dev_jobs.h
+++ b/software-raytracing_amd/csrc/rl_dev_jobs.h
@@ -82,6 +82,16 @@
 	j.sample = sLocal;
 	j.valid = (j.x < P.width) && (j.y < P.height);
 	return j;
+}
+
+__device__ __forceinline__ uint32_t BatchCellLocal(const DRenderParams& P, uint32_t base)
+{
+	const uint32_t rest = (uint32_t)__builtin_amdgcn_readfirstlane((int)base) >> 6;
+	uint32_t cellLocal = __umulhi(rest, P.magicSamples);
+	uint32_t sLocal = rest - cellLocal * P.sampleCount;
+	while (sLocal >= P.sampleCount) { sLocal -= P.sampleCount; ++cellLocal; }
+	if (P.activeCells) cellLocal = *(const __attribute__((address_space(4))) uint32_t*)(P.activeCells + cellLocal);
+	return cellLocal;
 }
 
 __device__ __forceinline__ uint32_t DecodeView(const DViews& V, uint32_t batchCell, uint32_t& cellInView)
@@ -231,6 +241,13 @@
 #define RL_LIT_ARGS() const DLitList& LL = LLk; (void)LL
 #endif
 
+struct KTraceHitqArgs { KTraceLazyArgs A; const uint32_t* cellLeaves; };
+#if RL_KARG_RELOAD
+#define RL_CELL_LEAVES_ARG() const uint32_t* const cellLeaves = KArg<const uint32_t*>((uint32_t)offsetof(KTraceHitqArgs, cellLeaves))
+#else
+#define RL_CELL_LEAVES_ARG() const uint32_t* const cellLeaves = cellLeavesK
+#endif
+
 template <class EACH>
 __device__ __forceinline__ float4 SumSlotBatch(const DRenderParams& P, const DSceneView& S, const SkyRot& R, const SampleRGB* samples,
                                                uint32_t numSlots, uint32_t slot, uint32_t cellLocal, uint32_t x, uint32_t y, float4 a, EACH&& each)
diff --git a/software-raytracing_amd/csrc/rl_dev_walk.h b/software-raytracing_amd/csrc/rl_dev_walk.h
--- a/software-raytracing_amd/csrc/rl_dev_walk.h
+++ b/software-raytracing_amd/csrc/rl_dev_walk.h
@@ -291,8 +291,8 @@
 	tn = fmaxf(tn, (nZ_.k - oL_.z) * invL_.z); tf = fminf(tf, (fZ_.k - oL_.z) * invL_.z); \
 	tk = (tf * widenL_ < tn) ? INFINITY : tn; }
 
-template <bool ANYHIT, bool PLAIN = false>
-__device__ __forceinline__ bool TraverseLeafList(const DSceneView& S, V3 o, V3 d, float tMin, HitRec& best, Counters& c, const float4* sm)
+template <bool ANYHIT, bool PLAIN = false, bool MASKED = false>
+__device__ __forceinline__ bool TraverseLeafList(const DSceneView& S, V3 o, V3 d, float tMin, HitRec& best, Counters& c, const float4* sm, const uint32_t recMask = 0xffffffffu)
 {
 	c.rays++;
 	const V3 invb = ExactInv(d);
@@ -304,11 +304,13 @@
 	const V3 cn = cc - ce, cf = cc + ce;
 	const char* recs = (const char*)(sm + LdsAt<2>::NODES);
 	const uint32_t oNX = nx ? 48u : 0u, oFX = 48u - oNX, oNY = ny ? 64u : 16u, oFY = 80u - oNY, oNZ = nz ? 80u : 32u, oFZ = 112u - oNZ;
+	const uint32_t live = MASKED ? recMask & ~(0xffffffffu << (uint32_t)S.numLeafRecords) : 0u;
+	if (MASKED) c.nodes += 2u * (uint32_t)S.numLeafRecords;
 	#pragma unroll
 	for (int g = 0; g < RL_LEAFLIST_RECORDS; ++g) {
 		key[4 * g] = key[4 * g + 1] = key[4 * g + 2] = key[4 * g + 3] = 0xffffffffu;
-		if (g < S.numLeafRecords) {
-			c.nodes += 2;
+		if (MASKED ? ((live >> g) & 1u) != 0u : g < S.numLeafRecords) {
+			if (!MASKED) c.nodes += 2;
 			RL_WSTEP(4);
 			const char* rec = recs + g * (RL_LDS_NSTRIDE * 16);
 			const float4 nX = *(const float4*)(rec + oNX), fX = *(const float4*)(rec + oFX);
@@ -377,11 +379,12 @@
 	return best.tri >= 0;
 }
 
-template <int STACK, bool ANYHIT, bool PRIMS, bool FULL, int LDS = 0, bool PLAIN = false>
+template <int STACK, bool ANYHIT, bool PRIMS, bool FULL, int LDS = 0, bool PLAIN = false, bool MASKED = false>
 __device__ __forceinline__ bool Traverse4(const DSceneView& S, V3 o, V3 d, float rayTime, float tMin, HitRec& best, int* stk, Counters& c, const float4* sm = nullptr,
-                                          const float tBound = INFINITY)
-{
-	if constexpr (LDS == 2) return TraverseLeafList<ANYHIT, PLAIN>(S, o, d, tMin, best, c, sm);
+                                          const float tBound = INFINITY, const uint32_t recMask = 0xffffffffu)
+{
+	static_assert(!MASKED || LDS == 2, "only the leaf-list walk takes a record mask");
+	if constexpr (LDS == 2) return TraverseLeafList<ANYHIT, PLAIN, MASKED>(S, o, d, tMin, best, c, sm, recMask);
 	c.rays++;
 	V3 invb = ExactInv(d);
 	if (!FULL) invb = ClampInv(invb);
diff --git a/software-raytracing_amd/csrc/rl_host.h b/software-raytracing_amd/csrc/rl_host.h
--- a/software-raytracing_amd/csrc/rl_host.h
+++ b/software-raytracing_amd/csrc/rl_host.h
@@ -205,6 +205,7 @@
 int32_t DeviceLastTraceLazy();
 int32_t DeviceLastHitQueue();
 int32_t DeviceLastLitMask();
+int32_t DeviceLastCellLeaves();
 int32_t DeviceLastTracePlain();
 bool DeviceDrain(RaylibAMDStats* outLastStats);
 void DeviceOwnStats();
@@ -252,6 +253,8 @@
 struct CullResult { std::vector<uint32_t> active; std::vector<unsigned char> empty; uint64_t emptyPixels = 0; float L[3] = { 0, 0, 0 }; uint32_t raysPerSample = 1; };
 bool CullCells(const CullScene& DS, const DCamera& cam, int32_t maxPathLength, float rayTMin, uint32_t W, uint32_t H,
                uint32_t cellsX, uint32_t cellFirst, uint32_t stride, uint32_t numLocalCells, CullResult& out);
+bool CellLeafMasks(const CullScene& DS, const DNode4* leafList, uint32_t numRecords, const DCamera& cam, float rayTMin, uint32_t W, uint32_t H,
+                   uint32_t cellsX, uint32_t cellFirst, uint32_t stride, uint32_t numLocalCells, uint32_t* out);
 bool DeviceEvalMath(int fn, const float* x, const float* y, int n, float* out);
 bool DeviceVerifyLazyRefl(uint32_t n, uint64_t seed, uint64_t out[3]);
 bool DeviceVerifyLazyPdf(uint32_t n, uint64_t seed, uint64_t out[3]);
diff --git a/software-raytracing_amd/csrc/rl_kernels.h b/software-raytracing_amd/csrc/rl_kernels.h
--- a/software-raytracing_amd/csrc/rl_kernels.h
+++ b/software-raytracing_amd/csrc/rl_kernels.h
@@ -30,8 +30,8 @@
 #define RL_K_TRACE_LAZY(a, b, c, d, e) template __global__ void k_trace_lazy<a, b, c, d, e>(RL_TRACE_ARGS, const DLitList);
 RL_TRACE_LAZY_INSTANCES(extern RL_K_TRACE_LAZY)
 template <int STACK, bool PRIMS, bool FULL, int LDS, bool PLAIN>
-__global__ void __launch_bounds__(RL_BLOCK, (STACK <= 32 ? RL_TRACE_MIN_WAVES : 2)) k_trace_lazy_hitq(RL_TRACE_ARGS, const DLitList);
-#define RL_K_TRACE_LAZY_HITQ(a, b, c, d, e) template __global__ void k_trace_lazy_hitq<a, b, c, d, e>(RL_TRACE_ARGS, const DLitList);
+__global__ void __launch_bounds__(RL_BLOCK, (STACK <= 32 ? RL_TRACE_MIN_WAVES : 2)) k_trace_lazy_hitq(RL_TRACE_ARGS, const DLitList, const uint32_t* __restrict__);
+#define RL_K_TRACE_LAZY_HITQ(a, b, c, d, e) template __global__ void k_trace_lazy_hitq<a, b, c, d, e>(RL_TRACE_ARGS, const DLitList, const uint32_t* __restrict__);
 RL_TRACE_LAZY_INSTANCES(extern RL_K_TRACE_LAZY_HITQ)
 __global__ void __launch_bounds__(RL_BLOCK) k_fold_lit(const DSceneView S, const DLitList LL, SampleRGB* __restrict__ samples, uint32_t numSlots);
 __global__ void __launch_bounds__(RL_BLOCK)
diff --git a/software-raytracing_amd/csrc/rl_plan.cc b/software-raytracing_amd/csrc/rl_plan.cc
--- a/software-raytracing_amd/csrc/rl_plan.cc
+++ b/software-raytracing_amd/csrc/rl_plan.cc
@@ -24,7 +24,7 @@
 	if (const char* e = getenv("RAYLIB_GUIDED")) k.guided = atoi(e);
 	if (const char* e = getenv("RAYLIB_BLOCKS_PER_CU")) k.blocksPerCU = std::max(0, atoi(e));
 	if (const char* e = getenv("RAYLIB_CULL_CELLS")) k.cullCells = atoi(e);
-	k.lazyRefl = flag("RAYLIB_LAZY_REFL"); k.hitQueue = flag("RAYLIB_HIT_QUEUE");
+	k.lazyRefl = flag("RAYLIB_LAZY_REFL"); k.hitQueue = flag("RAYLIB_HIT_QUEUE"); k.cellLeaves = flag("RAYLIB_CELL_LEAVES");
 	if (const char* e = getenv("RAYLIB_LIT_LIST")) k.litList = std::max(0ll, atoll(e));
 	k.litMask = flag("RAYLIB_LIT_MASK");
 	if (const char* e = getenv("RAYLIB_QUERY_TREE")) { const int v = atoi(e); k.queryTree = (v == 2 || v == 4 || v == 8) ? v : 0; }
@@ -92,6 +92,7 @@
 			p.plain = !hasSky && k.plainKernel != 0 && ScenePlain(sc);
 			p.lazy = p.plain && k.lazyRefl != 0 && st.maxPathLength <= RL_LAZY_MAX_PATH && SceneLazyRefl(sc);
 			p.hitQueue = p.lazy && st.maxPathLength >= 1 && (k.hitQueue >= 0 ? k.hitQueue != 0 : RL_HIT_QUEUE_DEFAULT != 0);
+			p.cellLeaves = p.lazy && st.maxPathLength >= 1 && (k.cellLeaves >= 0 ? k.cellLeaves != 0 : RL_CELL_LEAVES_DEFAULT != 0);
 		}
 	}
 	return p;
diff --git a/software-raytracing_amd/csrc/rl_plan.h b/software-raytracing_amd/csrc/rl_plan.h
--- a/software-raytracing_amd/csrc/rl_plan.h
+++ b/software-raytracing_amd/csrc/rl_plan.h
@@ -6,6 +6,7 @@
 
 #define RL_POOL_DEFAULT_MIN_TRIS 256u
 #define RL_HIT_QUEUE_DEFAULT 1
+#define RL_CELL_LEAVES_DEFAULT 1
 #define RL_FLOAT_BOX_MAX_TRIS 4096u
 
 struct RenderKnobs {
@@ -24,6 +25,7 @@
 	int gatherBatch = 0;
 	int lazyRefl = -1;
 	int hitQueue = -1;
+	int cellLeaves = -1;
 	long long litList = -1;
 	int litMask = -1;
 };
@@ -43,6 +45,7 @@
 	bool plain = false;
 	bool lazy = false;
 	bool hitQueue = false;
+	bool cellLeaves = false;
 	uint32_t pathsPerWave = 64, treeWidth = 2, nodeBytes = 64;
 	bool keepNodes4 = true, keepNodes4f = true;
 	int32_t eagerTree = TREE_NONE;
diff --git a/software-raytracing_amd/csrc/rl_rt.h b/software-raytracing_amd/csrc/rl_rt.h
--- a/software-raytracing_amd/csrc/rl_rt.h
+++ b/software-raytracing_amd/csrc/rl_rt.h
@@ -148,6 +148,8 @@
 	PinBuf<uint32_t> cellListHost[2]; DevBuf<uint32_t> cellList[2]; size_t cellListCells[2] = { 0, 0 };
 	std::vector<unsigned char> cullKey[2];
 	uint32_t cullActive[2] = { 0, 0 }; uint64_t cullEmptyPixels[2] = { 0, 0 }; float cullL[2][3] = { { 0, 0, 0 }, { 0, 0, 0 } }; uint32_t cullRays[2] = { 1, 1 };
+	PinBuf<uint32_t> leafMaskHost[2]; DevBuf<uint32_t> leafMask[2];
+	std::vector<unsigned char> leafMaskKey[2]; bool leafMaskHeld[2] = { false, false };
 	std::map<const void*, int> occupancy;
 	Worker* worker = nullptr;
 	DevBuf<float4> qRays;
@@ -221,6 +223,7 @@
 bool SyncMovedLocked(Scene& sc);
 bool ReadbackLocked(Image& img);
 bool EnqueueRender(RankCtx& R, Scene& sc, const RenderRequest& req, PendingRender& pend, ProgressiveSession* prog = nullptr);
+bool PrepareCellLeaves(Scene& sc, const RendererSettings& st);
 bool FinishRender(RankCtx& R, PendingRender& pend, RaylibAMDStats& stats);
 bool OnDevice(const void* p, int device);
 bool GatherLocked(Scene& sc, RankCtx& R, int32_t kind, const RaylibAMDRadianceParams& prm, uint64_t seed, const void* points, int32_t n, float* out, bool hostMem, void* stream,
diff --git a/software-raytracing_amd/csrc/rl_rt_frame.hip b/software-raytracing_amd/csrc/rl_rt_frame.hip
--- a/software-raytracing_amd/csrc/rl_rt_frame.hip
+++ b/software-raytracing_amd/csrc/rl_rt_frame.hip
@@ -7,6 +7,7 @@
 typedef void (*TraceKernel)(const DRenderParams, const DSceneView, const SkyRot, SampleRGB*, float*, unsigned long long*, unsigned int*);
 typedef void (*TraceViewsKernel)(const DRenderParams, const DSceneView, const SkyRot, SampleRGB*, float*, unsigned long long*, unsigned int*, const DViews);
 typedef void (*TraceLazyKernel)(const DRenderParams, const DSceneView, const SkyRot, SampleRGB*, float*, unsigned long long*, unsigned int*, const DLitList);
+typedef void (*TraceHitqKernel)(const DRenderParams, const DSceneView, const SkyRot, SampleRGB*, float*, unsigned long long*, unsigned int*, const DLitList, const uint32_t*);
 typedef void (*AovKernel)(const DRenderParams, const DSceneView, float4*, unsigned long long*);
 typedef void (*AovViewsKernel)(const DRenderParams, const DSceneView, float4*, unsigned long long*, const DViews);
 
@@ -29,7 +30,7 @@
 #undef RL_POOL_PICK
 		return nullptr;
 	}
-	if (p.lds == 2 && p.lazy && p.hitQueue && !views) return (const void*)(TraceLazyKernel)k_trace_lazy_hitq<16, false, true, 2, true>;
+	if (p.lds == 2 && p.lazy && p.hitQueue && !views) return (const void*)(TraceHitqKernel)k_trace_lazy_hitq<16, false, true, 2, true>;
 	if (p.lds == 2 && p.lazy && !views) return (const void*)(TraceLazyKernel)k_trace_lazy<16, false, true, 2, true>;
 	if (p.lds == 2) return p.plain ? Trace<16, false, true, 2, true>(views) : Trace<16, false, true, 2>(views);
 	if (p.lds == 1) return Trace<16, false, true, 1>(views);
@@ -52,6 +53,8 @@
 int32_t DeviceLastHitQueue() { return g_lastHitQueue.load(std::memory_order_relaxed); }
 static std::atomic<int32_t> g_lastLitMask{0};
 int32_t DeviceLastLitMask() { return g_lastLitMask.load(std::memory_order_relaxed); }
+static std::atomic<int32_t> g_lastCellLeaves{0};
+int32_t DeviceLastCellLeaves() { return g_lastCellLeaves.load(std::memory_order_relaxed); }
 
 struct Frame {
 	RenderKnobs knobs;
@@ -62,6 +65,7 @@
 	uint32_t sBegin = 0, sEnd = 1;
 	float4* out = nullptr;
 	const DViews* views = nullptr;
+	const uint32_t* cellLeaves = nullptr;
 	const void* resolve = nullptr;
 	void* resolveArgs[5] = {};
 	int firstBatch = 0, lastBatch = 0;
@@ -142,6 +146,7 @@
 		const bool lazy = plan.lazy && !F.views;
 		g_lastTraceLazy.store(lazy ? 1 : 0, std::memory_order_relaxed);
 		g_lastHitQueue.store(lazy && plan.hitQueue ? 1 : 0, std::memory_order_relaxed);
+		g_lastCellLeaves.store(lazy && plan.hitQueue && F.cellLeaves ? 1 : 0, std::memory_order_relaxed);
 		pend.lazy = lazy;
 		DLitList LL = {};
 		pend.pathsPerWave = plan.pathsPerWave; pend.treeWidth = plan.treeWidth; pend.nodeBytes = plan.nodeBytes;
@@ -154,7 +159,8 @@
 		g_lastLitMask.store(masked ? 1 : 0, std::memory_order_relaxed);
 		const void* resolveKernel = masked ? (const void*)k_resolve_lit : F.resolve;
 		const int depthSlots = P.maxPathLength > 1 ? P.maxPathLength : 1;
-		void* traceArgs[] = { &P, &F.view, &skyRot, &R.samples.ptr, &R.pathStack.ptr, &R.counters.ptr, &R.jobCounter.ptr, lazy ? (void*)&LL : (void*)F.views };
+		void* traceArgs[] = { &P, &F.view, &skyRot, &R.samples.ptr, &R.pathStack.ptr, &R.counters.ptr, &R.jobCounter.ptr, lazy ? (void*)&LL : (void*)F.views,
+		                      (void*)&F.cellLeaves };
 		void* foldArgs[] = { &F.view, &LL, &R.samples.ptr, (void*)&numSlots };
 		void* resolveArgs[] = { &P, &F.view, &skyRot, &R.samples.ptr, F.resolveArgs[0], F.resolveArgs[1], F.resolveArgs[2], F.resolveArgs[3], masked ? (void*)&LL : F.resolveArgs[4] };
 		for (uint32_t s0 = F.sBegin; s0 < F.sEnd; s0 += batch) {
@@ -280,6 +286,26 @@
 			prog->seeded = true;
 		}
 	}
+	if (F.plan.pathTrace && F.plan.hitQueue && F.plan.cellLeaves && numLocalCells && !sc.hostTreesStale) {
+		const std::vector<DNode4>& LLs = sc.bvh.leafList;
+		const CullScene cs = SceneCullScene(sc, false);
+		std::vector<unsigned char> key;
+		auto put = [&](const void* ptr, size_t n) { const unsigned char* b = (const unsigned char*)ptr; key.insert(key.end(), b, b + n); };
+		const uint32_t geo[6] = { W, H, req.cellFirst, stride, numLocalCells, __builtin_bit_cast(uint32_t, st.rayTMin) };
+		put(&req.camera, sizeof(req.camera)); put(geo, sizeof(geo)); put(&F.knobs.cellLeaves, sizeof(F.knobs.cellLeaves));
+		put(cs.boundsMin, sizeof(cs.boundsMin)); put(cs.boundsMax, sizeof(cs.boundsMax)); put(LLs.data(), LLs.size() * sizeof(DNode4));
+		if (key != R.leafMaskKey[q]) {
+			R.leafMaskKey[q].clear(); R.leafMaskHeld[q] = false;
+			const size_t bytes = (size_t)numLocalCells * sizeof(uint32_t);
+			if (!R.leafMaskHost[q].Grow(bytes) || !R.leafMask[q].Grow(bytes)) return false;
+			if (CellLeafMasks(cs, LLs.data(), (uint32_t)LLs.size(), req.camera, st.rayTMin, W, H, cellsX, req.cellFirst, stride, numLocalCells, R.leafMaskHost[q].ptr)) {
+				HIP_OK(hipMemcpyAsync(R.leafMask[q].ptr, R.leafMaskHost[q].ptr, bytes, hipMemcpyHostToDevice, R.stream));
+				R.leafMaskHeld[q] = true;
+			}
+			R.leafMaskKey[q] = key;
+		}
+		if (R.leafMaskHeld[q]) F.cellLeaves = R.leafMask[q].ptr;
+	}
 	if (prog) {
 		if (F.plan.pathTrace && numLocalCells) ListCells(F, pend, prog->trace.ptr, prog->empty.ptr, prog->numTrace, prog->numLive, prog->emptyL, prog->emptyLivePixels, prog->culledRays);
 		F.resolve = (const void*)k_progressive_resolve; F.resolveArgs[0] = &prog->st; F.resolveArgs[1] = &F.out; F.resolveArgs[2] = &F.lastBatch;
@@ -290,6 +316,14 @@
 	if (!EnqueueFrame(R, q, *sc.device, F, pend)) return false;
 	pend.pixels = CoveredPixels(W, H, req.cellFirst, stride, numLocalCells);
 	return true;
+}
+
+bool PrepareCellLeaves(Scene& sc, const RendererSettings& st)
+{
+	if (!sc.hostTreesStale || !sc.device) return true;
+	const TracePlan p = PlanTrace(sc, st, sc.device->copy[(size_t)Rank0().devSlot]->view.sky != nullptr, ReadRenderKnobs());
+	if (!p.ok || !p.pathTrace || !p.hitQueue || !p.cellLeaves) return true;
+	return SyncMovedLocked(sc);
 }
 
 static bool PrintStamps(RankCtx& R, const unsigned long long* cnt)
diff --git a/software-raytracing_amd/csrc/rl_rt_render.hip b/software-raytracing_amd/csrc/rl_rt_render.hip
--- a/software-raytracing_amd/csrc/rl_rt_render.hip
+++ b/software-raytracing_amd/csrc/rl_rt_render.hip
@@ -170,6 +170,7 @@
 	HIP_OK(hipSetDevice(Rank0().device));
 	if (!UploadScene(sc)) return false;
 	if (!SyncSky(sc)) return false;
+	if (!PrepareCellLeaves(sc, req.settings)) return false;
 	bool ok;
 	const bool whole = req.cellFirst == 0 && (req.cellStride == 0 || req.cellStride == 1);
 	if (whole && (RT.ranks.size() > 1 || RT.gatherSelf)) {
@@ -252,7 +253,7 @@
 	const uint32_t cnt = std::min(samples, S.cap - S.samples);
 	(void)DrainLocked();
 	Rt().deferredUnreported = false;
-	if (hipSetDevice(Rank0().device) != hipSuccess || !SyncSky(sc)) return -1;
+	if (hipSetDevice(Rank0().device) != hipSuccess || !SyncSky(sc) || !PrepareCellLeaves(sc, S.req.settings)) return -1;
 	S.passEnd = S.samples + cnt;
 	RenderRequest req = S.req;
 	req.outDevice = outDevice;
diff --git a/software-raytracing_amd/raylib_amd/binding.py b/software-raytracing_amd/raylib_amd/binding.py
--- a/software-raytracing_amd/raylib_amd/binding.py
+++ b/software-raytracing_amd/raylib_amd/binding.py
@@ -52,7 +52,7 @@
                [(k, C.c_uint32) for k in ("pathsPerWave", "treeWidth", "nodeBytes")] + \
                [(k, C.c_int32) for k in ("keepNodes4", "keepNodes4f", "eagerTree")] + \
                [(k, C.c_uint32) for k in ("batch", "sampleCount", "blocks", "stackStride", "jobChunk", "heads", "jobsPerHead", "guideShift")] + \
-               [("jobs", C.c_uint64), ("lazy", C.c_int32), ("hitQueue", C.c_int32)]
+               [("jobs", C.c_uint64), ("lazy", C.c_int32), ("hitQueue", C.c_int32), ("cellLeaves", C.c_int32), ("reserved", C.c_int32)]
     TREES = {0: "none", 1: "bvh2", 2: "box4", 3: "grid4", 4: "wide8"}
 
     def as_dict(self):
@@ -881,6 +881,9 @@
     "RaylibAMD_LastTraceLazy": (C.c_int32, []),
     "RaylibAMD_LastHitQueue": (C.c_int32, []),
     "RaylibAMD_LastLitMask": (C.c_int32, []),
+    "RaylibAMD_LastCellLeaves": (C.c_int32, []),
+    "RaylibAMD_CellLeafMasks": (C.c_int32, [C.c_void_p, C.c_void_p, C.POINTER(RendererSettings), C.c_uint32, C.c_uint32, C.c_uint32, C.POINTER(C.c_uint32)]),
+    "RaylibAMD_SceneLeafListBoxes": (C.c_int32, [C.c_void_p, C.POINTER(C.c_float), C.POINTER(C.c_uint8)]),
     "RaylibAMD_VerifyLazyRefl": (C.c_int32, [C.c_uint32, C.c_uint64, C.POINTER(C.c_uint64), C.POINTER(C.c_uint64), C.POINTER(C.c_uint64)]),
     "RaylibAMD_VerifyLazyPdf": (C.c_int32, [C.c_uint32, C.c_uint64, C.POINTER(C.c_uint64), C.POINTER(C.c_uint64), C.POINTER(C.c_uint64)]),
     "RaylibAMD_VerifySamplerRanged": (C.c_int32, [C.c_int32, C.POINTER(C.c_uint64), C.POINTER(C.c_uint64), C.POINTER(C.c_uint32), C.POINTER(C.c_uint64)]),
```

Result: faster. 23460, median of 5 (+1.3%).
